# neuraloperator/graph-pde

Hardware: AMD Instinct MI355X
Metric: M-edges/s through fused NNConv fwd (width=64) (higher is better)
Workload: dtype f32 (hidden layer + aggregation: 2-term f16-split MFMA, f32 accumulate); 1 GPU; GKN Darcy-2D 241x241 radius graph r=0.1 N=58081 E=95539625; NNConv_old fwd width=64; kernel MLP 6-1024-1024-4096; aggr=mean root+bias; one sample per GPU; graph=g241

## Files before the change

### graph-pde_amd/_lib.py

```python
from __future__ import annotations

import ctypes
import os
import re
import threading

_PKG = os.path.dirname(os.path.abspath(__file__))
LIB_PATH = os.environ.get("GPDE_LIB", os.path.join(_PKG, "libgpde.so"))

GPDE_OK = 0
GPDE_VERSION, GPDE_VERSION_ABLATION, GPDE_VERSION_INSTRUMENTED = 101, 0x10000, 0x20000
GPDE_ACC_EDGE_WEIGHTS, GPDE_ACC_ROOT, GPDE_ACC_BIAS = 1, 2, 4
GPDE_AGGR_ADD, GPDE_AGGR_MEAN, GPDE_AGGR_MAX = 0, 1, 2
GPDE_WECONV_MAX_GROUP = 16
GPDE_WECONV_ANY_MAX_WIDTH = 256
GPDE_REASSOC_ANY_MAX_HIDDEN = 4096
GPDE_RADIUS_BATCHED_REC_BYTES = 96
GPDE_FWD_DEFAULT, GPDE_FWD_F16SPLIT = 0, 1
GPDE_FWD_F16SPLIT_8WAVE, GPDE_FWD_STATIC_RANGES, GPDE_FWD_AGG_F16, GPDE_FWD_AGG_F32, GPDE_FWD_NO_EDGE_PATH = 2, 4, 16, 32, 64
GPDE_WIDTH = 64
GPDE_BWD_ACCUMULATE_GRAD_HIDDEN = 1

class GpdeWeConvDesc(ctypes.Structure):
    _fields_ = [("x", ctypes.c_void_p), ("edge_weights", ctypes.c_void_p), ("rowptr", ctypes.c_void_p),
                ("src", ctypes.c_void_p), ("root", ctypes.c_void_p), ("bias", ctypes.c_void_p),
                ("residual", ctypes.c_void_p), ("out", ctypes.c_void_p), ("n_nodes", ctypes.c_int32),
                ("aggr", ctypes.c_int32), ("relu", ctypes.c_int32), ("reserved", ctypes.c_int32)]


class GpdeNodeAttr(ctypes.Structure):
    _fields_ = [("table", ctypes.c_void_p), ("stride", ctypes.c_int32), ("n_slots", ctypes.c_int32), ("sel", ctypes.c_int32 * 8)]


HEADER_PATH = os.environ.get("GPDE_HEADER", os.path.join(os.path.dirname(_PKG), "include", "gpde.h"))
_SCALARS = {"int": ctypes.c_int, "int32_t": ctypes.c_int32, "int64_t": ctypes.c_int64, "uint32_t": ctypes.c_uint32,
            "size_t": ctypes.c_size_t, "double": ctypes.c_double}


def header_prototypes(path: str = None) -> dict:
    src = open(path or HEADER_PATH).read()
    src = re.sub(r"/\*.*?\*/", "", src, flags=re.S)
    out = {}
    for m in re.finditer(r"GPDE_API\s+([\w \*]+?)\s*\b(gpde_[a-z0-9_]+)\s*\(([^;]*?)\)\s*;", src, flags=re.S):
        ret, name, args = m.group(1).strip(), m.group(2), " ".join(m.group(3).split())
        types = []
        if args not in ("", "void"):
            for a in args.split(","):
                a = a.strip()
                t = re.sub(r"\b\w+$", "", a).strip() if not a.endswith("*") else a
                types.append(t.replace(" *", "*"))
        out[name] = (ret.replace(" *", "*"), types)
    return out


def _ctype(t: str, is_return: bool = False):
    if t.endswith("*"):
        return ctypes.c_char_p if is_return and t == "const char*" else ctypes.c_void_p
    base = t.replace("const ", "").strip()
    if base not in _SCALARS:
        raise GpdeError(f"{HEADER_PATH}: C type {t!r} has no binding rule (graph-pde_amd/_lib.py:_ctype)")
    return _SCALARS[base]


def _signatures_from_header() -> dict:
    if not os.path.exists(HEADER_PATH):
        raise GpdeError(f"{HEADER_PATH} not found: the binding is generated from the header (GPDE_HEADER overrides the path)")
    return {name: (_ctype(ret, True), [_ctype(a) for a in args]) for name, (ret, args) in header_prototypes().items()}


PROF_KINDS = ("fused", "gemm3", "epilogue", "prep", "other")


def profile_begin():
    lib().gpde_profile_begin()


def profile_end():
    ms = (ctypes.c_double * len(PROF_KINDS))()
    n = (ctypes.c_int32 * len(PROF_KINDS))()
    check(lib().gpde_profile_end_kinds(ms, n), "gpde_profile_end_kinds")
    return {k: (float(ms[i]), int(n[i])) for i, k in enumerate(PROF_KINDS)}


BWD_TRACE_FIELDS = ("phase", "na", "nb", "e0", "rows", "edge_kernel", "z", "hlast", "h1", "call_amax", "du1", "dw2", "dw1",
                    "du_pre", "ordered", "grad_attr", "from_h")
BWD_TRACE_CODES = {
    "phase": ("full", "conv", "mlp", "light", "deferred"),
    "z": ("none", "kept", "zagg32", "zagg16"),
    "hlast": ("none", "given", "store", "layers"),
    "h1": ("none", "gemm", "first_layer", "on_the_fly"),
    "du1": ("none", "f16s", "f32"),
    "dw2": ("none", "tn_split", "tn_acc"),
    "dw1": ("none", "epilogue", "dw_first", "tn_acc"),
}
BWD_TRACE_CAPACITY = 4096


def bwd_trace_begin():
    check(lib().gpde_bwd_trace_begin(), "gpde_bwd_trace_begin")


def bwd_trace_end() -> list:
    nf = len(BWD_TRACE_FIELDS)
    buf = (ctypes.c_int32 * (nf * BWD_TRACE_CAPACITY))()
    n = ctypes.c_int32()
    check(lib().gpde_bwd_trace_end(buf, BWD_TRACE_CAPACITY, ctypes.byref(n)), "gpde_bwd_trace_end")
    if n.value > BWD_TRACE_CAPACITY:
        raise GpdeError(f"gpde_bwd_trace_end: {n.value} records, more than the {BWD_TRACE_CAPACITY} this binding reads")
    out = []
    for r in range(n.value):
        rec = dict(zip(BWD_TRACE_FIELDS, buf[r * nf:(r + 1) * nf]))
        for k, names in BWD_TRACE_CODES.items():
            rec[k] = names[rec[k]]
        out.append(rec)
    return out

_lib = None
_lock = threading.Lock()
n_native_calls = 0


class GpdeError(RuntimeError):
    pass


SIGNATURES = _signatures_from_header()


def lib() -> ctypes.CDLL:
    global _lib
    if _lib is None:
        with _lock:
            if _lib is None:
                if not os.path.exists(LIB_PATH):
                    raise GpdeError(
                        f"{LIB_PATH} not found - build it with `python graph-pde_amd/build.py` "
                        "(or __graft_entry__.build()); the NNConv hot path has no non-HIP fallback")
                l = ctypes.CDLL(LIB_PATH)
                for name, (res, args) in SIGNATURES.items():
                    fn = getattr(l, name)
                    fn.restype, fn.argtypes = res, args
                ver = int(l.gpde_version())
                m = re.search(r"#define\s+GPDE_VERSION\s+(\d+)", open(HEADER_PATH).read())
                if m is None or int(m.group(1)) != (ver & 0xffff):
                    raise GpdeError(f"{LIB_PATH} reports ABI version {ver & 0xffff}, {HEADER_PATH} declares "
                                    f"{m.group(1) if m else '?'}: header and library do not belong together (GPDE_LIB / GPDE_HEADER)")
                if ver & GPDE_VERSION_ABLATION and os.environ.get("GPDE_ALLOW_ABLATION") != "1":
                    raise GpdeError(
                        f"{LIB_PATH} is an ABLATION build (gpde_version() = {ver:#x}: arithmetic compiled out, results are "
                        "wrong; timing experiments only) - refused.  GPDE_ALLOW_ABLATION=1 loads it for such an experiment")
                _lib = l
    return _lib


def reload_switches() -> None:
    if _lib is not None:
        _lib.gpde_reload_switches()


def check(rc: int, what: str) -> None:
    if rc != GPDE_OK:
        msg = lib().gpde_last_error().decode("utf-8", "replace")
        if rc == -2:
            raise NotImplementedError(f"{what}: {msg}")
        raise GpdeError(f"{what} failed (code {rc}): {msg}")


def dims_array(dims):
    return (ctypes.c_int32 * len(dims))(*[int(d) for d in dims])
```

### graph-pde_amd/csrc/gpde_api.hip

```cpp
#include "gpde_common.h"
#include <stdarg.h>
#include <stdio.h>
#include <stdlib.h>
#include <vector>

static thread_local char g_err[512] = "";

void gpde_set_error(const char* fmt, ...) {
    va_list ap;
    va_start(ap, fmt);
    vsnprintf(g_err, sizeof(g_err), fmt, ap);
    va_end(ap);
}

namespace {
__global__ void k_zero_words(unsigned* __restrict__ p, size_t n) {
    const size_t stride = (size_t)gridDim.x * blockDim.x;
    for (size_t i = (size_t)blockIdx.x * blockDim.x + threadIdx.x; i < n; i += stride) p[i] = 0u;
}
__global__ void k_zero_vec4(uint4* __restrict__ p, size_t n) {
    const size_t stride = (size_t)gridDim.x * blockDim.x;
    for (size_t i = (size_t)blockIdx.x * blockDim.x + threadIdx.x; i < n; i += stride) p[i] = uint4{0u, 0u, 0u, 0u};
}
__global__ void k_zero2d_words(unsigned* __restrict__ p, size_t pitch_words, size_t width_words, size_t rows) {
    const size_t n = width_words * rows, stride = (size_t)gridDim.x * blockDim.x;
    for (size_t i = (size_t)blockIdx.x * blockDim.x + threadIdx.x; i < n; i += stride) p[(i / width_words) * pitch_words + i % width_words] = 0u;
}
__global__ void k_copy_words(unsigned* __restrict__ d, const unsigned* __restrict__ s_, size_t n) {
    const size_t stride = (size_t)gridDim.x * blockDim.x;
    for (size_t i = (size_t)blockIdx.x * blockDim.x + threadIdx.x; i < n; i += stride) d[i] = s_[i];
}
unsigned fill_blocks(size_t items) {
    size_t b = (items + 255) / 256;
    return (unsigned)(b < 1 ? 1 : (b > 8192 ? 8192 : b));
}
}

hipError_t gpde_zero_async(void* p, size_t bytes, hipStream_t st) {
    if (bytes == 0) return hipSuccess;
    if (bytes % 4 != 0 || ((uintptr_t)p & 3)) return hipErrorInvalidValue;
    if (bytes % 16 == 0 && ((uintptr_t)p & 15) == 0) hipLaunchKernelGGL(k_zero_vec4, dim3(fill_blocks(bytes / 16)), dim3(256), 0, st, (uint4*)p, bytes / 16);
    else hipLaunchKernelGGL(k_zero_words, dim3(fill_blocks(bytes / 4)), dim3(256), 0, st, (unsigned*)p, bytes / 4);
    return hipGetLastError();
}
hipError_t gpde_zero2d_async(void* p, size_t pitch_bytes, size_t width_bytes, size_t rows, hipStream_t st) {
    if (width_bytes == 0 || rows == 0) return hipSuccess;
    if (pitch_bytes % 4 != 0 || width_bytes % 4 != 0 || ((uintptr_t)p & 3)) return hipErrorInvalidValue;
    hipLaunchKernelGGL(k_zero2d_words, dim3(fill_blocks(width_bytes / 4 * rows)), dim3(256), 0, st, (unsigned*)p, pitch_bytes / 4, width_bytes / 4, rows);
    return hipGetLastError();
}
hipError_t gpde_copy_async(void* dst, const void* src, size_t bytes, hipStream_t st) {
    if (bytes == 0) return hipSuccess;
    if (bytes % 4 != 0 || ((uintptr_t)dst & 3) || ((uintptr_t)src & 3)) return hipErrorInvalidValue;
    hipLaunchKernelGGL(k_copy_words, dim3(fill_blocks(bytes / 4)), dim3(256), 0, st, (unsigned*)dst, (const unsigned*)src, bytes / 4);
    return hipGetLastError();
}

namespace {
GpdeSwitches load_switches() {
    auto on = [](const char* n) { return getenv(n) != nullptr; };
    auto num = [](const char* n) { const char* e = getenv(n); return e ? atoi(e) : 0; };
    GpdeSwitches s{};
    s.bwd_gemm_f32 = on("GPDE_BWD_GEMM_F32");
    s.bwd_dw2_f32 = on("GPDE_BWD_DW2_F32");
    s.bwd_h1_materialize = on("GPDE_BWD_H1_MATERIALIZE");
    s.nt_no_prefetch = on("GPDE_NT_NO_PREFETCH");
    s.tn_no_ks_xcd = on("GPDE_TN_NO_KS_XCD");
    s.edge_bwd = num("GPDE_EDGE_BWD");
    const int v = num("GPDE_DEBUG_SKEW_US");
    s.debug_skew_us = v > 0 ? (v < 100000 ? v : 100000) : 0;
    return s;
}
GpdeSwitches& switches_storage() {
    static GpdeSwitches s = load_switches();
    return s;
}
}

const GpdeSwitches& gpde_switches() { return switches_storage(); }

extern "C" int gpde_reload_switches(void) {
    switches_storage() = load_switches();
    return GPDE_OK;
}

#if defined(GPDE_ABL_2MFMA) || defined(GPDE_ABL_NOSTAGE) || defined(GPDE_ABL_NOBARRIER) || defined(GPDE_ABL_NOGEMM2) || defined(GPDE_ABL_NOWAIT) || defined(GPDE_BWABL)
#define GPDE_BUILD_FLAGS_ GPDE_VERSION_ABLATION
#elif defined(GPDE_V6_TIMING) || defined(GPDE_NT_TIMING) || defined(GPDE_EB2_TIMING) || defined(GPDE_V3_TIMING)
#define GPDE_BUILD_FLAGS_ GPDE_VERSION_INSTRUMENTED
#else
#define GPDE_BUILD_FLAGS_ 0
#endif
extern "C" int gpde_version(void) { return GPDE_VERSION | GPDE_BUILD_FLAGS_; }
extern "C" const char* gpde_last_error(void) { return g_err; }

namespace {

struct EvPair { hipEvent_t a, b; int kind; };
thread_local bool g_prof_on = false;
thread_local std::vector<EvPair> g_prof;

struct ProfScope {
    bool on; EvPair p; hipStream_t s;
    ProfScope(int kind, hipStream_t stream) : on(g_prof_on), s(stream) {
        if (!on) return;
        p.kind = kind;
        if (hipEventCreate(&p.a) != hipSuccess || hipEventCreate(&p.b) != hipSuccess) { on = false; return; }
        (void)hipEventRecord(p.a, s);
    }
    ~ProfScope() {
        if (!on) return;
        (void)hipEventRecord(p.b, s);
        g_prof.push_back(p);
    }
};

constexpr size_t kAlign = 256;
size_t align_up(size_t v) { return (v + kAlign - 1) / kAlign * kAlign; }

int num_cus_impl() {
    static std::atomic<int> cus[32];
    int dev = 0;
    if (hipGetDevice(&dev) != hipSuccess || dev < 0 || dev > 31) dev = 0;
    int v = cus[dev].load(std::memory_order_relaxed);
    if (v == 0) {
        if (hipDeviceGetAttribute(&v, hipDeviceAttributeMultiprocessorCount, dev) != hipSuccess || v <= 0) v = 256;
        cus[dev].store(v, std::memory_order_relaxed);
    }
    return v;
}

struct Plan {
    GpdePackLayout L;
    int64_t nodes_per_chunk;
    int n_chunks;
    int n_groups;
    size_t off_part, off_z, off_ha, off_hb, off_xs, off_scal, off_blk;
    int nblk_max;
    size_t h_floats;
};

int pick_splits(int64_t nn) {
    const int64_t tiles = (nn + 63) / 64;
    int s = 1;
    while (s < 64 && tiles * s < 1024) s *= 2;
    return s;
}

int make_plan(int64_t N, int64_t E, int n_layers, const int32_t* dims, size_t ws_bytes, bool sizing,
              Plan* P, size_t* needed, bool hidden_given = false) {
    int rc = gpde_pack_layout(n_layers, dims, &P->L);
    if (rc != GPDE_OK) return rc;
    const GpdePackLayout& L = P->L;
    const size_t zrow = (size_t)GP_W * L.K2P * sizeof(float);
    const size_t prow = (size_t)64 * GP_W * sizeof(float);
    size_t fixed = 0;
    P->h_floats = 0;
    const size_t xs_bytes = (L.mode == 1 || hidden_given || sizing) ? align_up((size_t)(N > 0 ? N : 1) * GP_W * 4) + kAlign : 0;
    if (L.mode == 2 && !hidden_given) {
        int kmax = 0;
        for (int l = 1; l <= n_layers - 1; ++l) kmax = kmax > L.frontKP[l] ? kmax : L.frontKP[l];
        P->h_floats = (size_t)(E > 0 ? E : 1) * kmax;
        fixed = 2 * align_up(P->h_floats * sizeof(float));
    }
    fixed += xs_bytes;
    P->nblk_max = (L.mode == 1 && E < ((int64_t)1 << 31) - GP_QBLOCK) ? (int)(E / GP_QBLOCK + E / 8 / (GP_QBLOCK / 8)) + 10 : 0;
    const size_t blk_bytes = P->nblk_max ? align_up(((size_t)P->nblk_max + 2 + 64) * 4) : 0;
    fixed += blk_bytes;
    int64_t npc;
    if (sizing) {
        int64_t cap = (int64_t)(((size_t)4 << 30) / zrow);
        if (cap < 64) cap = 64;
        npc = N < cap ? N : cap;
        if (npc < 1) npc = 1;
    } else {
        if (ws_bytes < fixed + 2 * kAlign) {
            gpde_set_error("gpde_nnconv_fwd: workspace %zu bytes cannot hold the %zu-byte hidden "
                           "activation buffers", ws_bytes, fixed);
            return GPDE_EWORKSPACE;
        }
        npc = (int64_t)((ws_bytes - fixed - 2 * kAlign) / (zrow + prow));
        if (N > 0 && align_up((size_t)N * prow) + align_up((size_t)N * zrow) + fixed <= ws_bytes) npc = N;
        if (npc > N) npc = N;
        const int64_t min_nodes = N < 64 ? N : 64;
        if (npc < min_nodes || (N > 0 && npc < 1)) {
            gpde_set_error("gpde_nnconv_fwd: workspace %zu bytes holds %lld destination nodes, need >= %lld "
                           "(%zu bytes per node)", ws_bytes, (long long)npc, (long long)min_nodes, zrow + prow);
            return GPDE_EWORKSPACE;
        }
        if (npc < N && npc > 64) npc = npc / 64 * 64;
    }
    if (npc < 1) npc = 1;
    P->nodes_per_chunk = npc;
    P->n_chunks = (int)((N + npc - 1) / npc);
    if (P->n_chunks < 1) P->n_chunks = 1;
    size_t off = 0;
    P->off_part = off; off += align_up((size_t)npc * prow);
    P->off_z = off;    off += align_up((size_t)npc * zrow);
    P->off_ha = off;   off += (L.mode == 2 && !hidden_given) ? align_up(P->h_floats * sizeof(float)) : 0;
    P->off_hb = off;   off += (L.mode == 2 && !hidden_given) ? align_up(P->h_floats * sizeof(float)) : 0;
    P->off_xs = off;   off += xs_bytes ? xs_bytes - kAlign : 0;
    P->off_scal = off; off += xs_bytes ? kAlign : 0;
    P->off_blk = off;  off += blk_bytes;
    if (needed) *needed = off;
    const int ns = L.K2P / GP_TN;
    int groups = num_cus_impl() / ns;
    if (groups < 1) groups = 1;
    const int64_t tiles_chunk = ((E + GP_TE - 1) / GP_TE + P->n_chunks - 1) / P->n_chunks;
    int64_t gcap = (tiles_chunk + GP_WAVES - 1) / GP_WAVES;
    const int64_t gcap_nodes = (npc + GP_WAVES - 1) / GP_WAVES;
    if (gcap < gcap_nodes) gcap = gcap_nodes;
    if (groups > gcap) groups = (int)(gcap < 1 ? 1 : gcap);
    P->n_groups = groups;
    return GPDE_OK;
}

enum FusedKind { FK_GENERIC = 0, FK_V3 = 1, FK_V6 = 2 };
struct FusedChoice { FusedKind kind; bool g2f16; };
FusedChoice choose_fused(const GpdePackLayout& L, int mode, uint32_t flags, int64_t n_edges, int kt) {
    FusedChoice c{FK_GENERIC, false};
    if (mode != 1 || !(flags & GPDE_FWD_F16SPLIT)) return c;
    GpdeFusedArgs probe = gpde_fused_probe(L);
    probe.kt = kt;
    if (!gpde_fused_f16v3_supported(probe)) return c;
    c.kind = FK_V3;
    c.g2f16 = !(flags & GPDE_FWD_AGG_F32) && n_edges > 0 && ((flags & GPDE_FWD_AGG_F16) || n_edges >= 32768);
    probe.xs = c.g2f16 ? (const unsigned*)(uintptr_t)8 : nullptr;
    if (c.g2f16 && !(flags & GPDE_FWD_F16SPLIT_8WAVE) && gpde_fused_f16v6_supported(probe)) c.kind = FK_V6;
    return c;
}

bool takes_edge_path(const Plan& P, uint32_t flags, int64_t n_nodes, int64_t n_edges, bool hidden, bool hidden_absmax,
                     bool mixed, int kt) {
    const GpdePackLayout& L = P.L;
    bool store_ok = false;
    if (L.mode == 1 && L.k0 + 1 <= 8) store_ok = gpde_fused_store_supported(gpde_fused_probe(L));
    return ((flags & GPDE_FWD_F16SPLIT) || (hidden && hidden_absmax)) && !mixed && !kt && L.has_w3s && P.n_chunks == 1 &&
           n_edges >= 4096 && n_edges <= 4 * n_nodes && n_edges < ((int64_t)1 << 24) &&
           !(flags & GPDE_FWD_NO_EDGE_PATH) &&
           (hidden || (L.mode == 1 && store_ok)) &&
           (size_t)(n_edges) * L.K2P + gpde_edge_messages_ws_floats(n_edges, GP_W * GP_W) <=
               (size_t)n_nodes * GP_W * L.K2P;
}

}

int gpde_num_cus() { return num_cus_impl(); }

extern "C" const char* gpde_nnconv_fwd_kernel(int64_t n_edges, int n_layers, const int32_t* dims, uint32_t flags) {
    GpdePackLayout L;
    if (!dims || gpde_pack_layout(n_layers, dims, &L) != GPDE_OK) return "";
    switch (choose_fused(L, L.mode, flags, n_edges, 0).kind) {
        case FK_V6: return "gpde_fused_f16v6_kernel";
        case FK_V3: return "gpde_fused_f16v3_kernel";
        default: return "gpde_fused_kernel";
    }
}

extern "C" int gpde_nnconv_fwd_edge_path(int64_t n_nodes, int64_t n_edges, int n_layers, const int32_t* dims, uint32_t flags,
                                         size_t ws_bytes) {
    Plan P;
    if (!dims || n_nodes < 0 || n_edges < 0) { gpde_set_error("gpde_nnconv_fwd_edge_path: null/negative argument"); return GPDE_EINVAL; }
    int rc = make_plan(n_nodes, n_edges, n_layers, dims, ws_bytes, false, &P, nullptr);
    if (rc != GPDE_OK) return rc;
    return takes_edge_path(P, flags, n_nodes, n_edges, false, false, false, 0) ? 1 : 0;
}

extern "C" size_t gpde_nnconv_fwd_workspace_bytes(int64_t n_nodes, int64_t n_edges, int n_layers,
                                                  const int32_t* dims) {
    Plan P;
    size_t need = 0;
    if (!dims || n_nodes < 0 || n_edges < 0) return 0;
    if (make_plan(n_nodes, n_edges, n_layers, dims, 0, true, &P, &need) != GPDE_OK) return 0;
    return need + 2 * kAlign;
}

extern "C" int gpde_nnconv_fwd_plan(int64_t n_nodes, int64_t n_edges, int n_layers,
                                    const int32_t* dims, size_t ws_bytes, int32_t* n_chunks,
                                    int64_t* nodes_per_chunk, int32_t* fused_workgroups,
                                    int32_t* mode) {
    Plan P;
    if (!dims) { gpde_set_error("gpde_nnconv_fwd_plan: dims is null"); return GPDE_EINVAL; }
    int rc = make_plan(n_nodes, n_edges, n_layers, dims, ws_bytes, false, &P, nullptr);
    if (rc != GPDE_OK) return rc;
    if (n_chunks) *n_chunks = P.n_chunks;
    if (nodes_per_chunk) *nodes_per_chunk = P.nodes_per_chunk;
    if (fused_workgroups) *fused_workgroups = P.n_groups * (P.L.K2P / GP_TN);
    if (mode) *mode = P.L.mode;
    return GPDE_OK;
}

namespace {

struct FwdArgs {
    const float* x = nullptr;
    int64_t n_nodes = 0, n_edges = 0;
    const int32_t *rowptr = nullptr, *src = nullptr, *dst = nullptr;
    int n_layers = 0;
    const int32_t* dims = nullptr;
    const void* packed = nullptr;
    const float *root = nullptr, *bias = nullptr;
    int aggr = 0;
    float* out = nullptr;
    void* ws = nullptr;
    size_t ws_bytes = 0;
    hipStream_t stream = nullptr;
    const float* edge_attr = nullptr;
    const int32_t* perm = nullptr;
    uint32_t flags = 0;
    const float *hidden = nullptr, *hidden_absmax = nullptr;
    int64_t hidden_nodes = -1;
    int kt = 0;
    const int* sel = nullptr;
    const float* residual = nullptr;
    int relu_out = 0;
    float* z_keep = nullptr;
};

FwdArgs fwd_common(const float* x, int64_t n_nodes, int64_t n_edges, const int32_t* rowptr, const int32_t* src, const int32_t* dst,
                   int n_layers, const int32_t* dims, const void* packed, const float* root, const float* bias, int aggr,
                   float* out, void* ws, size_t ws_bytes, void* stream) {
    FwdArgs a;
    a.x = x; a.n_nodes = n_nodes; a.n_edges = n_edges; a.rowptr = rowptr; a.src = src; a.dst = dst;
    a.n_layers = n_layers; a.dims = dims; a.packed = packed; a.root = root; a.bias = bias; a.aggr = aggr;
    a.out = out; a.ws = ws; a.ws_bytes = ws_bytes; a.stream = (hipStream_t)stream;
    return a;
}

int fwd_impl(const FwdArgs& a) {
    const bool mixed = a.hidden && a.hidden_nodes >= 0 && a.hidden_nodes < a.n_nodes;
    if (a.aggr != GPDE_AGGR_ADD && a.aggr != GPDE_AGGR_MEAN) {
        gpde_set_error("gpde_nnconv_fwd: aggr %d not implemented (add=0, mean=1)", a.aggr);
        return GPDE_EUNSUPPORTED;
    }
    if (a.n_nodes == 0) return GPDE_OK;
    if (!a.ws) { gpde_set_error("gpde_nnconv_fwd: workspace is null"); return GPDE_EWORKSPACE; }
    Plan P;
    int rc = make_plan(a.n_nodes, a.n_edges, a.n_layers, a.dims, a.ws_bytes, false, &P, nullptr, a.hidden != nullptr && !mixed);
    if (rc != GPDE_OK) return rc;
    const GpdePackLayout& L = P.L;
    const int mode = (a.hidden && !mixed) ? 2 : L.mode;
    if (mixed && L.mode != 1) { gpde_set_error("gpde_nnconv_fwd_mixed_keepz: built for 3-Linear kernel MLPs"); return GPDE_EUNSUPPORTED; }
    const float* pk = (const float*)a.packed;
    char* w = (char*)a.ws;
    w = (char*)(((uintptr_t)w + kAlign - 1) / kAlign * kAlign);
    float* part = (float*)(w + P.off_part);
    float* zbuf = (float*)(w + P.off_z);
    float* ha = (float*)(w + P.off_ha);
    float* hb = (float*)(w + P.off_hb);

    const float* hfinal = a.hidden;
    if (!a.hidden && L.mode == 2 && a.n_edges > 0) {
        const float* in = a.edge_attr;
        int ldx = L.k0, kin = L.k0;
        const int32_t* gather = a.perm;
        float* bufs[2] = {ha, hb};
        for (int l = 0; l < a.n_layers - 1; ++l) {
            GpdeDenseArgs d;
            d.X = in; d.ldx = ldx; d.kin = kin; d.gather = gather; d.row0 = 0;
            d.W = pk + L.off_front_w[l]; d.ldw = L.frontKP[l];
            d.b = pk + L.off_front_b[l];
            d.Y = bufs[l & 1]; d.KoutP = L.frontKP[l + 1];
            d.rows = (int)a.n_edges; d.relu = 1;
            rc = gpde_launch_dense(d, a.stream);
            if (rc != GPDE_OK) return rc;
            in = d.Y; ldx = kin = d.KoutP; gather = nullptr;
        }
        hfinal = in;
    }

    const bool edge_path = !a.z_keep && takes_edge_path(P, a.flags, a.n_nodes, a.n_edges, a.hidden != nullptr,
                                                        a.hidden_absmax != nullptr, mixed, a.kt);
    if (edge_path) {
        float* Hbuf = zbuf;
        float* ews = zbuf + (a.hidden ? 0 : (size_t)a.n_edges * L.K2P);
        const float* Hrows = a.hidden;
        if (!a.hidden) {
            ProfScope ps(GPDE_PROF_FUSED, a.stream);
            GpdeFusedArgs f{};
            f.attr = a.edge_attr; f.rowptr = a.rowptr; f.perm = a.perm;
            gpde_fused_set_pack(f, pk, L);
            f.hout = Hbuf; f.hmax_out = nullptr;
            f.nc0 = 0; f.nc1 = (int)a.n_nodes; f.e_chunk0 = 0;
            f.n_groups = gpde_fused_groups(L.K2P, gpde_group_cap_fwd(a.n_edges));
            if ((rc = gpde_launch_fused_store(f, a.stream)) != GPDE_OK) return rc;
            Hrows = Hbuf;
        }
        {
            ProfScope ps(GPDE_PROF_GEMM3, a.stream);
            rc = gpde_launch_edge_messages(Hrows, L.K2P, a.n_edges, pk + L.off_w3s, pk + L.off_ucol3, a.x, a.src, a.rowptr, a.n_nodes,
                                           ews, part, a.stream);
            if (rc != GPDE_OK) return rc;
        }
        GpdeEpilogueArgs e;
        e.part = part; e.x = a.x; e.rowptr = a.rowptr; e.src = a.src;
        e.b3 = pk + L.off_b3; e.root = a.root; e.bias = a.bias; e.out = a.out;
        e.nc0 = 0; e.nn = (int)a.n_nodes; e.splits = 1; e.aggr = a.aggr;
        e.residual = a.residual; e.relu_out = a.relu_out;
        ProfScope ps2(GPDE_PROF_EPILOGUE, a.stream);
        return gpde_launch_epilogue(e, a.stream);
    }

    const unsigned* xs = nullptr;
    const unsigned* scal = nullptr;
    const FusedChoice fc = choose_fused(L, mode, a.flags, a.n_edges, a.kt);
    if (a.kt && fc.kind == FK_GENERIC) {
        gpde_set_error("gpde_nnconv_fwd_mixed_keepz (node_attr): built for 3-Linear kernel MLPs on the f16-split kernel only");
        return GPDE_EUNSUPPORTED;
    }
    if ((!a.hidden || mixed) && fc.g2f16) {
        ProfScope psp(GPDE_PROF_PREP, a.stream);
        rc = gpde_launch_g2_prep(a.x, a.n_nodes, a.edge_attr, a.n_edges, L.k0, pk + L.off_w1 + (size_t)L.K1P * 8,
                                 (unsigned*)(w + P.off_scal), (unsigned*)(w + P.off_xs), a.stream, a.kt, a.sel, a.src, a.dst);
        if (rc != GPDE_OK) return rc;
        xs = (const unsigned*)(w + P.off_xs);
        scal = (const unsigned*)(w + P.off_scal);
    }

    if (a.hidden && !mixed && a.hidden_absmax && a.n_edges >= 32768 && !(a.flags & GPDE_FWD_AGG_F32)) {
        rc = gpde_launch_g2_prep(a.x, a.n_nodes, nullptr, 0, 0, nullptr, (unsigned*)(w + P.off_scal),
                                 (unsigned*)(w + P.off_xs), a.stream);
        if (rc != GPDE_OK) return rc;
        xs = (const unsigned*)(w + P.off_xs);
        scal = (const unsigned*)(w + P.off_scal);
    }

    const int64_t hn = mixed ? a.hidden_nodes : (a.hidden ? a.n_nodes : 0);
    for (int64_t nc0 = 0, nc1 = 0; nc0 < a.n_nodes; nc0 = nc1) {
        const int64_t lim = nc0 < hn ? hn : a.n_nodes;
        nc1 = (nc0 + P.nodes_per_chunk < lim) ? nc0 + P.nodes_per_chunk : lim;
        const bool from_h = nc0 < hn;
        const int nn = (int)(nc1 - nc0);
        const int splits = pick_splits(nn);
        if (a.n_edges > 0) {
            GpdeFusedArgs f{};
            f.x = a.x; f.attr = a.edge_attr; f.rowptr = a.rowptr; f.src = a.src; f.dst = a.dst; f.perm = a.perm;
            gpde_fused_set_pack(f, pk, L);
            float* zc = a.z_keep ? a.z_keep + (size_t)nc0 * GP_W * L.K2P : zbuf;
            f.hbuf = hfinal; f.zbuf = zc; f.xs = xs; f.scal = scal;
            f.kt = a.kt; f.hmax = (from_h && xs) ? (const unsigned*)a.hidden_absmax : nullptr;
            for (int d = 0; d < 8; ++d) f.sel[d] = (a.kt && a.sel) ? a.sel[d < L.k0 ? d : L.k0 - 1] : 0;
            f.nc0 = (int)nc0; f.nc1 = (int)nc1; f.e_chunk0 = 0; f.n_groups = P.n_groups;
            {
                ProfScope ps(GPDE_PROF_FUSED, a.stream);
                if (!from_h && fc.kind == FK_V6 && P.nblk_max && L.K2P / GP_TN <= 64 && !(a.flags & GPDE_FWD_STATIC_RANGES)) {
                    int32_t* blk = (int32_t*)(w + P.off_blk);
                    f.blk = blk; f.qn = blk + P.nblk_max + 1; f.qctr = (unsigned*)(blk + P.nblk_max + 2);
                    rc = gpde_launch_block_bounds(a.rowptr, (int)nc0, (int)nc1, P.nblk_max, blk, blk + P.nblk_max + 1,
                                                  (unsigned*)(blk + P.nblk_max + 2), L.K2P / GP_TN, a.stream);
                    if (rc != GPDE_OK) return rc;
                }
                if (from_h) rc = gpde_launch_zagg(f, a.stream);
                else if (fc.kind == FK_V6) rc = gpde_launch_fused_f16v6(f, a.stream);
                else if (fc.kind == FK_V3) rc = gpde_launch_fused_f16v3(f, a.stream);
                else rc = gpde_launch_fused(mode, (a.flags & GPDE_FWD_F16SPLIT) != 0 && mode == 1, f, a.stream);
            }
            if (rc != GPDE_OK) return rc;
            ProfScope ps1(GPDE_PROF_GEMM3, a.stream);
            GpdeGemm3Args g;
            g.zbuf = zc; g.w3q = pk + L.off_w3q; g.part = part; g.nn = nn; g.K2P = L.K2P;
            g.splits = splits; g.rowptr = a.rowptr; g.nc0 = (int)nc0;
            rc = gpde_launch_gemm3(g, a.stream);
            if (rc != GPDE_OK) return rc;
        }
        GpdeEpilogueArgs e;
        e.part = part; e.x = a.x; e.rowptr = a.rowptr; e.src = a.src;
        e.b3 = pk + L.off_b3; e.root = a.root; e.bias = a.bias; e.out = a.out;
        e.nc0 = (int)nc0; e.nn = nn; e.splits = splits; e.aggr = a.aggr;
        e.residual = a.residual; e.relu_out = a.relu_out;
        ProfScope ps2(GPDE_PROF_EPILOGUE, a.stream);
        rc = gpde_launch_epilogue(e, a.stream);
        if (rc != GPDE_OK) return rc;
    }
    return GPDE_OK;
}

}

extern "C" int gpde_nnconv_fwd(const float* x, int64_t n_nodes, const float* edge_attr,
                               int64_t n_edges, const int32_t* rowptr, const int32_t* src,
                               const int32_t* dst, const int32_t* perm, int n_layers,
                               const int32_t* dims, const void* packed, const float* root,
                               const float* bias, int aggr, uint32_t flags, float* out, void* ws,
                               size_t ws_bytes, void* stream_) {
    if (n_nodes < 0 || n_edges < 0 || !dims || !packed || !rowptr || (n_nodes > 0 && (!x || !out)) ||
        (n_edges > 0 && (!edge_attr || !src || !dst || !perm))) {
        gpde_set_error("gpde_nnconv_fwd: null/negative argument");
        return GPDE_EINVAL;
    }
    FwdArgs a = fwd_common(x, n_nodes, n_edges, rowptr, src, dst, n_layers, dims, packed, root, bias, aggr, out, ws, ws_bytes, stream_);
    a.edge_attr = edge_attr; a.perm = perm; a.flags = flags;
    return fwd_impl(a);
}

extern "C" int gpde_nnconv_fwd_mixed_keepz(const float* x, int64_t n_nodes, const float* edge_attr, const GpdeNodeAttr* node_attr,
                                           const float* hidden, const float* hidden_absmax, int64_t hidden_nodes, int64_t n_edges,
                                           const int32_t* rowptr, const int32_t* src, const int32_t* dst,
                                           const int32_t* perm, int n_layers, const int32_t* dims, const void* packed,
                                           const float* root, const float* bias, int aggr, uint32_t flags, float* z_keep,
                                           float* out, void* ws, size_t ws_bytes, void* stream_) {
    if (n_nodes < 0 || n_edges < 0 || !dims || !packed || !rowptr || (n_nodes > 0 && (!x || !out)) ||
        (n_edges > 0 && (!src || !dst || (!node_attr && (!edge_attr || !perm)))) || hidden_nodes < 0 || hidden_nodes > n_nodes ||
        (hidden_nodes > 0 && !hidden)) {
        gpde_set_error("gpde_nnconv_fwd_mixed_keepz: null/negative argument");
        return GPDE_EINVAL;
    }
    int kt = 0;
    int sel[8] = {0, 0, 0, 0, 0, 0, 0, 0};
    const float* attr = edge_attr;
    if (node_attr) {
        const GpdeNodeAttr* na = node_attr;
        if (!na->table || na->stride < 1 || na->n_slots != dims[0] || dims[0] < 1 || dims[0] > 7) {
            gpde_set_error("gpde_nnconv_fwd_mixed_keepz: GpdeNodeAttr must describe dims[0] = 1..7 slots of a node table");
            return GPDE_EINVAL;
        }
        for (int d = 0; d < 8; ++d) {
            sel[d] = na->sel[d < dims[0] ? d : dims[0] - 1];
            if ((sel[d] >> 8) < 0 || (sel[d] >> 8) > 1 || (sel[d] & 255) >= na->stride) {
                gpde_set_error("gpde_nnconv_fwd_mixed_keepz: GpdeNodeAttr.sel[%d] = 0x%x (endpoint << 8 | column, column < %d)", d, sel[d], na->stride);
                return GPDE_EINVAL;
            }
        }
        kt = na->stride;
        attr = na->table;
        perm = nullptr;
    }
    FwdArgs a = fwd_common(x, n_nodes, n_edges, rowptr, src, dst, n_layers, dims, packed, root, bias, aggr, out, ws, ws_bytes, stream_);
    a.edge_attr = attr; a.perm = perm; a.flags = flags; a.kt = kt; a.sel = kt ? sel : nullptr; a.z_keep = z_keep;
    if (hidden_nodes != 0) { a.hidden = hidden; a.hidden_absmax = hidden_absmax; a.hidden_nodes = hidden_nodes; }
    return fwd_impl(a);
}

extern "C" int gpde_nnconv_fwd_hidden(const float* x, int64_t n_nodes, const float* hidden,
                                      const float* hidden_absmax, int64_t n_edges, const int32_t* rowptr, const int32_t* src,
                                      const int32_t* dst, int n_layers, const int32_t* dims,
                                      const void* packed, const float* root, const float* bias,
                                      int aggr, float* out, void* ws, size_t ws_bytes, void* stream_) {
    if (n_nodes < 0 || n_edges < 0 || !dims || !packed || !rowptr || (n_nodes > 0 && (!x || !out)) ||
        (n_edges > 0 && (!hidden || !src || !dst))) {
        gpde_set_error("gpde_nnconv_fwd_hidden: null/negative argument");
        return GPDE_EINVAL;
    }
    FwdArgs a = fwd_common(x, n_nodes, n_edges, rowptr, src, dst, n_layers, dims, packed, root, bias, aggr, out, ws, ws_bytes, stream_);
    a.hidden = hidden; a.hidden_absmax = hidden_absmax;
    return fwd_impl(a);
}

extern "C" int gpde_nnconv_fwd_act(const float* x, int64_t n_nodes, const float* edge_attr, int64_t n_edges,
                                   const int32_t* rowptr, const int32_t* src, const int32_t* dst, const int32_t* perm,
                                   int n_layers, const int32_t* dims, const void* packed, const float* root,
                                   const float* bias, int aggr, uint32_t flags, const float* residual, int relu_out,
                                   float* out, void* ws, size_t ws_bytes, void* stream_) {
    if (n_nodes < 0 || n_edges < 0 || !dims || !packed || !rowptr || (n_nodes > 0 && (!x || !out)) ||
        (n_edges > 0 && (!edge_attr || !src || !dst || !perm)) || (residual && residual == out)) {
        gpde_set_error("gpde_nnconv_fwd_act: null/negative argument (or residual aliases out)");
        return GPDE_EINVAL;
    }
    FwdArgs a = fwd_common(x, n_nodes, n_edges, rowptr, src, dst, n_layers, dims, packed, root, bias, aggr, out, ws, ws_bytes, stream_);
    a.edge_attr = edge_attr; a.perm = perm; a.flags = flags; a.residual = residual; a.relu_out = relu_out;
    return fwd_impl(a);
}

extern "C" int gpde_nnconv_fwd_hidden_act(const float* x, int64_t n_nodes, const float* hidden, const float* hidden_absmax,
                                          int64_t n_edges, const int32_t* rowptr, const int32_t* src, const int32_t* dst,
                                          int n_layers, const int32_t* dims, const void* packed, const float* root,
                                          const float* bias, int aggr, const float* residual, int relu_out, float* out,
                                          void* ws, size_t ws_bytes, void* stream_) {
    if (n_nodes < 0 || n_edges < 0 || !dims || !packed || !rowptr || (n_nodes > 0 && (!x || !out)) ||
        (n_edges > 0 && (!hidden || !src || !dst)) || (residual && residual == out)) {
        gpde_set_error("gpde_nnconv_fwd_hidden_act: null/negative argument (or residual aliases out)");
        return GPDE_EINVAL;
    }
    FwdArgs a = fwd_common(x, n_nodes, n_edges, rowptr, src, dst, n_layers, dims, packed, root, bias, aggr, out, ws, ws_bytes, stream_);
    a.hidden = hidden; a.hidden_absmax = hidden_absmax; a.residual = residual; a.relu_out = relu_out;
    return fwd_impl(a);
}

extern "C" int gpde_nnconv_fwd_keepz(const float* x, int64_t n_nodes, const float* edge_attr, const float* hidden,
                                     const float* hidden_absmax, int64_t n_edges, const int32_t* rowptr, const int32_t* src,
                                     const int32_t* dst, const int32_t* perm, int n_layers, const int32_t* dims,
                                     const void* packed, const float* root, const float* bias, int aggr, uint32_t flags,
                                     float* z_keep, float* out, void* ws, size_t ws_bytes, void* stream_) {
    if (n_nodes < 0 || n_edges < 0 || !dims || !packed || !rowptr || (n_nodes > 0 && (!x || !out || !z_keep)) ||
        (n_edges > 0 && (!src || !dst || (!hidden && (!edge_attr || !perm))))) {
        gpde_set_error("gpde_nnconv_fwd_keepz: null/negative argument");
        return GPDE_EINVAL;
    }
    FwdArgs a = fwd_common(x, n_nodes, n_edges, rowptr, src, dst, n_layers, dims, packed, root, bias, aggr, out, ws, ws_bytes, stream_);
    a.z_keep = z_keep;
    if (hidden) { a.hidden = hidden; a.hidden_absmax = hidden_absmax; }
    else { a.edge_attr = edge_attr; a.perm = perm; a.flags = flags; }
    return fwd_impl(a);
}

extern "C" int gpde_profile_begin(void) {
// ... 27 lines not shown
```

### graph-pde_amd/csrc/gpde_common.h

```cpp
#pragma once
#include <hip/hip_runtime.h>
#include <stdint.h>
#include <stddef.h>
#include "gpde.h"
#include <atomic>

typedef float f32x4 __attribute__((ext_vector_type(4)));
typedef float f32x16 __attribute__((ext_vector_type(16)));

constexpr int GP_W = GPDE_WIDTH;
constexpr int GP_TE = 32;
constexpr int GP_TN = 128;
constexpr int GP_BK = 32;
constexpr int GP_WAVES = 4;
constexpr int GP_BS_STRIDE = 36;

static inline int gp_round_up(int v, int m) { return (v + m - 1) / m * m; }

static inline bool gp_overlap(const void* a, size_t na, const void* b, size_t nb) {
    if (!a || !b || !na || !nb) return false;
    const uintptr_t a0 = (uintptr_t)a, b0 = (uintptr_t)b;
    return a0 < b0 + nb && b0 < a0 + na;
}

struct GpdePackLayout {
    int mode;
    int n_layers;
    int k0;
    int k1, K1P;
    int k2, K2P;
    size_t off_w1;
    size_t off_w2t;
    size_t off_b2;
    size_t off_w2h;
    size_t off_ucol;
    size_t off_w1h;
    size_t off_fcol;
    size_t off_w3q;
    size_t off_b3;
    size_t off_front;
    int frontKP[GPDE_MAX_LAYERS + 1];
    size_t off_front_w[GPDE_MAX_LAYERS];
    size_t off_front_b[GPDE_MAX_LAYERS];
    size_t off_w3s;
    size_t off_ucol3;
    int has_w3s;
    size_t total_floats;
    int has_b3;
};

int gpde_pack_layout(int n_layers, const int32_t* dims, GpdePackLayout* L);

void gpde_set_error(const char* fmt, ...);

hipError_t gpde_zero_async(void* p, size_t bytes, hipStream_t st);
hipError_t gpde_zero2d_async(void* p, size_t pitch_bytes, size_t width_bytes, size_t rows, hipStream_t st);
hipError_t gpde_copy_async(void* dst, const void* src, size_t bytes, hipStream_t st);

struct GpdeSwitches {
    bool bwd_gemm_f32;
    bool bwd_dw2_f32;
    bool bwd_h1_materialize;
    bool nt_no_prefetch;
    bool tn_no_ks_xcd;
    int edge_bwd;
    int debug_skew_us;
};
const GpdeSwitches& gpde_switches();

#define GP_HIP_CHECK(expr)                                                              \
    do {                                                                                \
        hipError_t _e = (expr);                                                         \
        if (_e != hipSuccess) {                                                         \
            gpde_set_error("%s failed: %s (%s:%d)", #expr, hipGetErrorString(_e),       \
                           __FILE__, __LINE__);                                         \
            return GPDE_EHIP;                                                           \
        }                                                                               \
    } while (0)

#define GP_LAUNCH_CHECK(name)                                                           \
    do {                                                                                \
        hipError_t _e = hipGetLastError();                                              \
        if (_e != hipSuccess) {                                                         \
            gpde_set_error("launch of %s failed: %s", name, hipGetErrorString(_e));     \
            return GPDE_EHIP;                                                           \
        }                                                                               \
    } while (0)

struct GpdeLdsOnce {
    std::atomic<unsigned> done{0};
    template <typename... Fn>
    int ensure(Fn... fns) {
        int dev = 0;
        if (hipGetDevice(&dev) != hipSuccess || dev < 0 || dev > 31) dev = 0;
        if (done.load(std::memory_order_acquire) & (1u << dev)) return GPDE_OK;
        const void* fl[] = {(const void*)fns...};
        for (const void* f : fl) {
            hipError_t e = hipFuncSetAttribute(f, hipFuncAttributeMaxDynamicSharedMemorySize, 160 * 1024);
            if (e != hipSuccess) {
                gpde_set_error("hipFuncSetAttribute(MaxDynamicSharedMemorySize) failed: %s", hipGetErrorString(e));
                return GPDE_EHIP;
            }
        }
        done.fetch_or(1u << dev, std::memory_order_release);
        return GPDE_OK;
    }
};

struct GpdeFusedArgs {
    const float* x;
    const float* attr;
    const int32_t* rowptr;
    const int32_t* src;
    const int32_t* dst;
    const int32_t* perm;
    const float* w1;
    const float* w2t;
    const float* b2;
    const void* w2h;
    const float* ucol;
    const void* w1h;
    const float* fcol;
    const float* hbuf;
    float* zbuf;
    float* hout;
    const unsigned* xs;
    const unsigned* scal;
    const unsigned* hmax;
    unsigned* hmax_out;
    const int32_t* blk;
    const int32_t* qn;
    unsigned* qctr;
    int kt;
    int sel[8];
    int k0, K1P, K2P;
    int nc0, nc1;
    int e_chunk0;
    int n_groups;
    int kernarg_pad_;
};
int gpde_launch_fused(int mode, bool f16split, const GpdeFusedArgs& a, hipStream_t stream);
int gpde_launch_g2_prep(const float* x, int64_t n_nodes, const float* attr, int64_t n_edges, int k0,
                        const float* wmax8, unsigned* scal, unsigned* xs, hipStream_t stream,
                        int kt = 0, const int* sel = nullptr, const int32_t* src = nullptr,
                        const int32_t* dst = nullptr);
constexpr int GP_QBLOCK = 4096;
int gpde_launch_block_bounds(const int32_t* rowptr, int nc0, int nc1, int nblk_max, int32_t* blk, int32_t* qn,
                             unsigned* qctr, int n_slices, hipStream_t stream);
__host__ __device__ static inline float gpde_pow2_to_2p13(float v) {
    union { float f; unsigned u; } a; a.f = v;
    const int eb = (int)((a.u >> 23) & 0xff);
    if (eb < 20 || eb > 230) return 1.f;
    a.u = (unsigned)(267 - eb) << 23;
    return a.f;
}
int gpde_launch_zagg(const GpdeFusedArgs& a, hipStream_t stream);
bool gpde_fused_f16v3_supported(const GpdeFusedArgs& a);
int gpde_launch_fused_f16v3(const GpdeFusedArgs& a, hipStream_t stream);
bool gpde_fused_store_supported(GpdeFusedArgs probe);
int gpde_launch_fused_store(const GpdeFusedArgs& a, hipStream_t stream);
bool gpde_fused_f16v6_supported(const GpdeFusedArgs& a);
int gpde_launch_fused_f16v6(const GpdeFusedArgs& a, hipStream_t stream);
int gpde_num_cus();
static inline void gpde_fused_set_pack(GpdeFusedArgs& f, const float* pk, const GpdePackLayout& L) {
    f.w1 = pk + L.off_w1; f.w2t = pk + L.off_w2t; f.b2 = pk + L.off_b2;
    f.w2h = pk + L.off_w2h; f.ucol = pk + L.off_ucol; f.w1h = pk + L.off_w1h; f.fcol = pk + L.off_fcol;
    f.k0 = L.k0; f.K1P = L.K1P; f.K2P = L.K2P;
}
static inline GpdeFusedArgs gpde_fused_probe(const GpdePackLayout& L) {
    GpdeFusedArgs probe{};
    probe.k0 = L.k0; probe.K1P = L.K1P; probe.K2P = L.K2P;
    return probe;
}
static inline int64_t gpde_group_cap_fwd(int64_t n_edges) { return ((n_edges + GP_TE - 1) / GP_TE + GP_WAVES - 1) / GP_WAVES; }
static inline int64_t gpde_group_cap_bwd_chunk(int rows) { return (rows / GP_TE + GP_WAVES) / GP_WAVES; }
static inline int gpde_fused_groups(int K2P, int64_t cap) {
    int groups = gpde_num_cus() / (K2P / GP_TN);
    if (groups < 1) groups = 1;
    return groups > cap ? (int)cap : groups;
}

struct GpdeGemm3Args {
    const float* zbuf;
    const float* w3q;
    float* part;
    int nn, K2P, splits;
    const int32_t* rowptr;
    int nc0;
};
int gpde_launch_gemm3(const GpdeGemm3Args& a, hipStream_t stream);

struct GpdeEpilogueArgs {
    const float* part;
    const float* x;
    const int32_t* rowptr;
    const int32_t* src;
    const float* b3;
    const float* root;
    const float* bias;
    float* out;
    int nc0, nn, splits, aggr;
    const float* residual;
    int relu_out;
};
int gpde_launch_epilogue(const GpdeEpilogueArgs& a, hipStream_t stream);

struct GpdeDenseArgs {
    const float* X; int ldx; int kin;
    const int32_t* gather;
    int row0;
    const float* W; int ldw;
    const float* b;
    float* Y; int KoutP;
    int rows; int relu;
};
int gpde_launch_dense(const GpdeDenseArgs& a, hipStream_t stream);

struct GpdeGemmArgs {
    const float* A; const float* B; float* C;
    int M, N, K;
    int lda, ldb, ldc;
    int a_kcontig, b_kcontig;
    const float* bias;
    int relu;
    const float* mask; int ldmask;
    int accumulate;
    int batches; size_t strideA, strideB, strideC;
    int splits; size_t strideSplit;
    int skew_us;
};
int gpde_debug_skew_us();
__device__ __forceinline__ void gp_debug_skew(int us) {
    if (us > 0) {
        const unsigned long long t0 = wall_clock64();
        while (wall_clock64() - t0 < (unsigned long long)us * 100ull) __builtin_amdgcn_s_sleep(64);
    }
}
int gpde_launch_gemm(const GpdeGemmArgs& g, hipStream_t stream);
int gpde_launch_reduce_splits(const float* P, size_t n, int splits, size_t stride, float* C,
                              int accumulate, hipStream_t stream);
struct GpdeGemmF16sArgs {
    const float* A; int lda; int M;
    const void* bsplit; const float* ucol;
    const float* mask; int ldmask;
    const uint32_t* maskbits; int ldmb;
    float* C; int ldc;
    int K, N;
    const float* sc; const float* isc;
    int n_groups;
    int ksplits; size_t cstride;
    const float* xc_x; const int32_t* xc_src;
    int skew_us;
    int no_tile_prefetch;
    int no_ks_xcd;
    const int32_t* g_src;
    const int32_t* g_tile;
    int g_ntiles;
    size_t g_layer_stride;
    size_t g_bnode_bytes;
    const float* g_unscale;
    int fl_mode;
    const float* fl_attr; int fl_ld0;
    int fl_rows;
    const void* fl_wimg;
    const float* fl_alpha;
    float* fl_dw_part; float* fl_dw_out; int fl_dw_ld; float* fl_db_out; int fl_skip_store;
};
size_t gpde_gemm_f16s_dw_part_floats(int M, int N);
bool gpde_gemm_f16s_supported(int M, int N, int K, int lda);

struct GpdeEdgeBwd3Args {
    const float* x; const int32_t* src; const int32_t* dst;
    const float* dZ;
    const float* dz_unscale;
    const float* dS;
    const float* H;
    float* dU;
    float* dx;
    float* dxe;
    int e0, e1, n0, K2P;
    float* dUt; int ldt;
    float* row_sc; float* row_isc;
    float* csum_part; unsigned* cmax_part;
    int du_accumulate;
};
int gpde_launch_dz_split(float* dZ, int nn, int K2P, float* unscale, hipStream_t stream);
int gpde_launch_edge_bwd3(const GpdeEdgeBwd3Args& a, hipStream_t stream);
int gpde_launch_gemm_f16s_nt(const GpdeGemmF16sArgs& a, float* row_scale_ws , hipStream_t stream);
size_t gpde_edge_messages_ws_floats(int64_t n_edges, int n_out);
int gpde_launch_edge_messages(const float* H, int K2P, int64_t n_edges, const void* w3s, const float* ucol3,
                              const float* x, const int32_t* src, const int32_t* rowptr, int64_t n_nodes, float* ws,
                              float* part, hipStream_t stream);
size_t gpde_gemm_f16s_tn_ws_floats(int rows_max, int n_out, int n_in, int ksplits);
struct GpdeFirstLayerSpec {
    const float* H0; int ld0;
    const float* Wp; int ldw;
    const float* bp;
    uint32_t* maskbits;
    int k0;
    const unsigned* amax_bits;
};
bool gpde_first_layer_in_kernel(const GpdeFirstLayerSpec& f, int rows, int ksplits);
struct GpdeDuStats {
    float* db_accumulate;
    float* row_sc; float* row_isc;
    const float* tile_csum; const unsigned* tile_cmax;
};
float* gpde_gemm_f16s_tn_at(float* ws, int rows, int ksplits, int* ld);
int gpde_launch_gemm_f16s_tn(const float* dU, int ldu, int n_out, const float* H, int ldh, int n_in, int rows,
                             int ksplits, float* ws, float* part, hipStream_t stream,
                             const unsigned* du_absmax_bits = nullptr ,
                             const GpdeFirstLayerSpec* first_layer = nullptr ,
                             const GpdeDuStats* du_stats = nullptr);
int gpde_launch_gemm_f16s_gather(const float* xstack, size_t layer_stride, int Lp, const float* sc_src, const float* isc_src,
                                 const int32_t* src_rows, int rows, const int32_t* tiles, int ntiles, const void* bimg,
// ... 16 lines not shown
```

### graph-pde_amd/csrc/gpde_fused_f16v6.hip

```cpp
#include "gpde_common.h"
#include <cstdlib>
#include <type_traits>

namespace {

typedef _Float16 h8 __attribute__((ext_vector_type(8)));
typedef unsigned u4 __attribute__((ext_vector_type(4)));

__device__ __forceinline__ f32x4 mfma32k(h8 a, h8 b, f32x4 c) {
    return __builtin_amdgcn_mfma_f32_16x16x32_f16(a, b, c, 0, 0, 0);
}
#define GPDE_GLDS(g, l, off)                                                                       \
    __builtin_amdgcn_global_load_lds((const __attribute__((address_space(1))) void*)(g),         \
                                     (__attribute__((address_space(3))) void*)(l), 16, off, 0)

__device__ __forceinline__ int lower_bound_node(const int32_t* __restrict__ rowptr, int lo, int hi, long target) {
    while (lo < hi) {
        int mid = (lo + hi) >> 1;
        if ((long)rowptr[mid] < target) lo = mid + 1; else hi = mid;
    }
    return lo;
}

#ifdef GPDE_V6_TIMING
__device__ unsigned long long gpde_v6_tm[8];
#define TM_MARK(acc) do { const long long tm1_ = clock64(); acc += tm1_ - tm0_; tm0_ = tm1_; } while (0)
#else
#define TM_MARK(acc) do { } while (0)
#endif

constexpr int NS = 3;
constexpr int TILE_B = GP_TN * 128;
constexpr int TE = 64;
constexpr int NW = 4;

template <int MODE, bool NODEATTR = false>
__global__ __launch_bounds__(256) __attribute__((amdgpu_waves_per_eu(1, 1)))
void gpde_fused_f16v6_kernel(GpdeFusedArgs a) {
    constexpr bool WRITE_H = MODE == 1;
    extern __shared__ __attribute__((aligned(16))) char smem[];
    char* ring = smem;
    char* w1s = smem + NS * TILE_B;
    unsigned* Xs_all = (unsigned*)(w1s + (size_t)a.K1P * 32);
    float* Es_all = (float*)(Xs_all + NW * TE * GP_W);
    int* red = (int*)(Es_all + NW * TE);
    float* colc = (float*)(red + 16);

    const int tid = threadIdx.x;
    const int lane = tid & 63;
    const int wave = __builtin_amdgcn_readfirstlane(tid >> 6);
    const int l15 = lane & 15;
    const int g = lane >> 4;
    float* Es = Es_all + wave * TE;
    unsigned* Xs = Xs_all + wave * TE * GP_W;

    const int ns = a.K2P / GP_TN;
    const int slice = blockIdx.x % ns;
    const int group = blockIdx.x / ns;
    const int NKC = a.K1P / GP_BK;

    for (int i = tid; i < a.K1P * 2; i += 256) ((f32x4*)w1s)[i] = ((const f32x4*)a.w1h)[i];

    const int e_lo = a.rowptr[a.nc0], e_hi = a.rowptr[a.nc1];
    const bool queue = a.blk != nullptr;
    int blk_a = 0, blk_b = 0;
    const int nblk = queue ? *a.qn : 0;
    bool have;
    auto draw_block = [&](int& ba, int& bb) {
        for (;;) {
            int b = 0;
            if (lane == 0) b = (int)atomicAdd(a.qctr + slice, 1u);
            b = __builtin_amdgcn_readfirstlane(b);
            if (b >= nblk) return false;
            ba = a.blk[b];
            bb = a.blk[b + 1];
            if (bb > ba) return true;
        }
    };
    if (queue) {
        have = draw_block(blk_a, blk_b);
    } else {
        const long tot = (long)e_hi - e_lo;
        const int nranges = a.n_groups * NW;
        const int wg = group * NW + wave;
        const int na = lower_bound_node(a.rowptr, a.nc0, a.nc1, e_lo + tot * wg / nranges);
        const int nb_ = (wg == nranges - 1) ? a.nc1
                                            : lower_bound_node(a.rowptr, a.nc0, a.nc1, e_lo + tot * (wg + 1) / nranges);
        blk_a = a.rowptr[na];
        blk_b = a.rowptr[nb_];
        have = blk_b > blk_a;
    }
    if (lane == 0) { red[wave] = have ? 0 : 1; red[4 + wave] = 0; }
    __syncthreads();
    if (red[0] + red[1] + red[2] + red[3] == 4) return;

    const unsigned long long w2base = (unsigned long long)a.w2h + (size_t)slice * NKC * TILE_B + wave * 4096;
    const unsigned lane16 = lane * 16;
    auto w2_src = [&](int chunk) {
        unsigned long long gb = w2base + (size_t)chunk * TILE_B;
        asm volatile("" : "+s"(gb));
        return (const char*)(gb + lane16);
    };

    float z_unscale = 1.f;
    if constexpr (WRITE_H) {
        if (tid < GP_TN) {
            colc[tid] = a.b2[slice * GP_TN + tid];
            colc[GP_TN + tid] = a.ucol[slice * GP_TN + tid];
        }
    } else {
        const float sx = gpde_pow2_to_2p13(__uint_as_float(a.scal[0]));
        const float hb = a.fcol[8] + a.fcol[9] * __uint_as_float(a.scal[1]);
        const float sh = gpde_pow2_to_2p13(hb);
        if (tid < GP_TN) {
            colc[tid] = a.b2[slice * GP_TN + tid] * sh;
            colc[GP_TN + tid] = a.ucol[slice * GP_TN + tid] * sh;
        }
        z_unscale = (1.f / sx) * (1.f / sh);
    }
    float wmx8[8], fcol8[8];
#pragma unroll
    for (int d = 0; d < 8; ++d) {
        wmx8[d] = a.w1[(size_t)a.K1P * 8 + (d & 1) * 4 + (d >> 1)];
        fcol8[d] = a.fcol[d];
    }
    const int bo = l15 * 128 + ((g ^ ((l15 >> 1) & 7)) << 4);
    const int w1o = (16 * (l15 >> 3) + 4 * ((l15 >> 2) & 1) + (l15 & 3)) * 32 + (g == 2 ? 16 : 0);

    const int e_clamp = max(e_hi - 1, 0);
    int perm_n = 0;
    [[maybe_unused]] int dst_n = 0;
    int src_l = 0;
    float attr_n[8];
    auto load_perm = [&](int e0n) {
        if constexpr (NODEATTR) {
            perm_n = a.src[min(e0n + lane, e_clamp)];
            dst_n = a.dst[min(e0n + lane, e_clamp)];
        } else perm_n = a.perm[min(e0n + lane, e_clamp)];
    };
    auto load_attr_d = [&](int d) {
        if constexpr (NODEATTR) {
            const int sd = a.sel[d];
            attr_n[d] = a.attr[(size_t)((sd >> 8) ? dst_n : perm_n) * a.kt + (sd & 255)];
        } else {
            attr_n[d] = a.attr[(size_t)perm_n * a.k0 + min(d, a.k0 - 1)];
        }
    };
    auto load_attr = [&]() {
#pragma unroll
        for (int d = 0; d < 8; ++d) load_attr_d(d);
    };
    int xsidx[4];
    auto x_addr1 = [&](int i0, int i) { xsidx[i] = __builtin_amdgcn_ds_bpermute((4 * (i0 + i) + (lane >> 4)) * 4, src_l); };
    auto x_issue1 = [&](int i0, int i) {
        int unit = lane & 15;
        GPDE_GLDS(a.xs + (size_t)xsidx[i] * GP_W + unit * 4, Xs + (i0 + i) * 4 * GP_W, 0);
    };

    auto conv_a = [&](float v0, float v1, unsigned& ph, unsigned& t0_, unsigned& t1_) {
        asm("v_max_i32 %1, 0, %3\n\t"
            "v_max_i32 %2, 0, %4\n\t"
            "v_cvt_pkrtz_f16_f32 %0, %1, %2"
            : "=&v"(ph), "=&v"(t0_), "=&v"(t1_) : "v"(v0), "v"(v1));
    };
    auto conv_b = [&](unsigned ph, unsigned t0_, unsigned t1_, unsigned& pl) {
        asm("v_fma_mixlo_f16 %0, %1, 1.0, -%3 op_sel:[0,0,0] op_sel_hi:[0,0,1]\n\t"
            "v_fma_mixhi_f16 %0, %2, 1.0, -%3 op_sel:[0,0,1] op_sel_hi:[0,0,1]"
            : "=&v"(pl) : "v"(t0_), "v"(t1_), "v"(ph));
    };
    auto conv_pair = [&](float v0, float v1, unsigned& ph, unsigned& pl) {
        unsigned t0_, t1_;
        conv_a(v0, v1, ph, t0_, t1_);
        conv_b(ph, t0_, t1_, pl);
    };
    auto conv_step = [&](int step, float v0, float v1, unsigned& ph, unsigned& t0_, unsigned& t1_, unsigned& pl) {
        if (step == 0) asm("v_max_i32 %0, 0, %1" : "=v"(t0_) : "v"(v0));
        if (step == 1) asm("v_max_i32 %0, 0, %1" : "=v"(t1_) : "v"(v1));
        if (step == 2) asm("v_cvt_pkrtz_f16_f32 %0, %1, %2" : "=v"(ph) : "v"(t0_), "v"(t1_));
        if (step == 3) asm("v_fma_mixlo_f16 %0, %1, 1.0, -%2 op_sel:[0,0,0] op_sel_hi:[0,0,1]" : "=v"(pl) : "v"(t0_), "v"(ph));
        if (step == 4) asm("v_fma_mixhi_f16 %0, %1, 1.0, -%2 op_sel:[0,0,1] op_sel_hi:[0,0,1]" : "+v"(pl) : "v"(t1_), "v"(ph));
    };
    auto h1gen_half = [&](f32x4 (&dd)[4][2], int e0, h8 w1r0, h8 w1r1, const h8 (&at)[4]) {
        asm volatile("s_nop 4");
#pragma unroll
        for (int e = e0; e < e0 + 2; ++e) {
            asm volatile("v_mfma_f32_16x16x32_f16 %0, %1, %2, 0" : "=&v"(dd[e][0]) : "v"(w1r0), "v"(at[e]));
            asm volatile("v_mfma_f32_16x16x32_f16 %0, %1, %2, 0" : "=&v"(dd[e][1]) : "v"(w1r1), "v"(at[e]));
        }
    };
    auto h1gen = [&](f32x4 (&dd)[4][2], h8 w1r0, h8 w1r1, const h8 (&at)[4]) {
        h1gen_half(dd, 0, w1r0, w1r1, at);
        h1gen_half(dd, 2, w1r0, w1r1, at);
    };

    {
        const char* g0 = w2_src(0);
        char* l0 = ring + wave * 4096;
        GPDE_GLDS(g0, l0, 0); GPDE_GLDS(g0, l0, 1024); GPDE_GLDS(g0, l0, 2048); GPDE_GLDS(g0, l0, 3072);
        const char* g1 = w2_src(1);
        char* l1 = ring + TILE_B + wave * 4096;
        GPDE_GLDS(g1, l1, 0); GPDE_GLDS(g1, l1, 1024); GPDE_GLDS(g1, l1, 2048); GPDE_GLDS(g1, l1, 3072);
    }
    load_perm(have ? blk_a : e_hi);
    load_attr();
    asm volatile("s_waitcnt vmcnt(0)" ::: "memory");
    __syncthreads();

    f32x4 acc[4][8], Z[4][8];
#pragma unroll
    for (int e = 0; e < 4; ++e)
#pragma unroll
        for (int nb = 0; nb < 8; ++nb)
#pragma unroll
            for (int r = 0; r < 4; ++r) { acc[e][nb][r] = 0.f; Z[e][nb][r] = 0.f; }
    int cur = -1;
    [[maybe_unused]] float hmax_run = 0.f;

    auto flush = [&](int node) {
        float* zb = a.zbuf + ((size_t)(node - a.nc0) * GP_W) * a.K2P + slice * GP_TN;
        int zl = lane;
        asm volatile("" : "+v"(zl));
        const int z_loff = 4 * (zl >> 4) * a.K2P + (zl & 15);
#pragma unroll
        for (int cb = 0; cb < 4; ++cb)
#pragma unroll
            for (int nb = 0; nb < 8; ++nb) asm volatile("" : "+a"(Z[cb][nb]));
#pragma unroll
        for (int cb = 0; cb < 4; ++cb) {
#pragma unroll
            for (int r = 0; r < 4; ++r) {
                float* rp = zb + (size_t)(cb * 16 + r) * a.K2P;
#pragma unroll
                for (int nb = 0; nb < 8; ++nb) {
                    rp[z_loff + nb * 16] = Z[cb][nb][r] * z_unscale;
                    Z[cb][nb][r] = 0.f;
                }
                if ((r & 1) == 1) __builtin_amdgcn_sched_barrier(0);
            }
        }
#pragma unroll
        for (int cb = 0; cb < 4; ++cb)
#pragma unroll
            for (int nb = 0; nb < 8; ++nb) asm volatile("" : "+a"(Z[cb][nb]));
    };

    int slot = 0;

#ifdef GPDE_V6_TIMING
    long long tm_pro = 0, tm_loop = 0, tm_post = 0, tm_peel = 0, tm0_ = clock64();
#endif
    int e0 = have ? blk_a : e_hi;
    int n_rounds = 0;
    for (int t = 0;; ++t) {
        const int eb = have ? blk_b : e0;
        const int e_end = min(e0 + TE, eb);
        const bool last_in_blk = have && (e0 + TE >= blk_b);
        int na_ = 0, nb_ = 0;
        bool have_n = have && !last_in_blk;
        if (last_in_blk && queue) have_n = draw_block(na_, nb_);
        const int e0n = !have ? e_hi : (last_in_blk ? (have_n ? na_ : e_hi) : e0 + TE);
        if (t > 0) {
            if (lane == 0) red[(t & 1) * 4 + wave] = have ? 0 : 1;
            __syncthreads();
            const int* rf = red + (t & 1) * 4;
            if (rf[0] + rf[1] + rf[2] + rf[3] == 4) break;
        }
        ++n_rounds;

        h8 B1[4];
        {
#pragma unroll
            for (int b = 0; b < 4; ++b) {
                float av[8];
#pragma unroll
                for (int d = 0; d < 8; ++d)
                    av[d] = __int_as_float(__builtin_amdgcn_ds_bpermute((16 * b + l15) * 4, __float_as_int(attr_n[d])));
                const bool valid = (e0 + 16 * b + l15) < eb;
                float v[8];
                float bnd = 0.f;
#pragma unroll
                for (int d = 0; d < 8; ++d) {
                    float q = (valid && d < a.k0) ? av[d] : 0.f;
                    if (valid && d == a.k0) q = 1.f;
                    v[d] = q;
                    bnd = fmaf(wmx8[d], fabsf(q), bnd);
                }
                const int ebits = (__float_as_int(bnd) >> 23) & 0xff;
                const bool okb = (ebits >= 20) && (ebits <= 230);
                const float sc = okb ? __int_as_float((267 - ebits) << 23) : 1.f;
                const float isc = okb ? __int_as_float((ebits - 13) << 23) : 1.f;
                if (g == 0) Es[16 * b + l15] = isc;
#pragma unroll
                for (int d = 0; d < 8; ++d) {
                    const float s_ = v[d] * fcol8[d] * sc;
                    const _Float16 hi = (_Float16)s_;
                    const _Float16 lo = (_Float16)(s_ - (float)hi);
                    B1[b][d] = g == 1 ? lo : (g == 3 ? (_Float16)0.f : hi);
                }
            }
        }
        h8 bhi[2][2], blo[2][2];
#pragma unroll
        for (int nb = 0; nb < 2; ++nb) {
            bhi[0][nb] = *(const h8*)(ring + slot * TILE_B + nb * 2048 + bo);
            blo[0][nb] = *(const h8*)(ring + slot * TILE_B + nb * 2048 + (bo ^ 64));
        }
        f32x4 d[4][2];
        u4 ahi[4], alo[4];
        {
            const char* wp = w1s + w1o;
            const h8 A1 = *(const h8*)wp, A2 = *(const h8*)(wp + 256);
            h1gen(d, A1, A2, B1);
            asm volatile("s_nop 15\n\ts_nop 15" ::: "memory");
#pragma unroll
            for (int e = 0; e < 4; ++e)
#pragma unroll
                for (int jp = 0; jp < 4; ++jp) {
                    unsigned ph, pl;
                    conv_pair(d[e][jp >> 1][2 * (jp & 1)], d[e][jp >> 1][2 * (jp & 1) + 1], ph, pl);
                    ahi[e][jp] = ph;
                    alo[e][jp] = pl;
                }
        }
        int nf_v[2] = {0, 0}, nl_v[2] = {0, 0};
        unsigned cph = 0, ct0 = 0, ct1 = 0, cpl = 0;
        h8 A1, A2;

        TM_MARK(tm_pro);
        auto chunk = [&](auto ph_tag, int c) {
            constexpr int PH = decltype(ph_tag)::value;
            asm volatile("" : "+s"(c));
            const int slot1 = slot + 1 == NS ? 0 : slot + 1;
            const int slot2 = slot1 + 1 == NS ? 0 : slot1 + 1;
            int c2 = c + 2;
            if (c2 >= NKC) c2 -= NKC;
            const char* gsrc = w2_src(c2);
            char* ldst = ring + slot2 * TILE_B + wave * 4096;
            const char* rb0 = ring + slot * TILE_B;
            const char* rb1 = ring + slot1 * TILE_B;
            int c1 = c + 1;
            if (c1 >= NKC) c1 -= NKC;
            const char* w1n = w1s + (size_t)c1 * GP_BK * 32 + w1o;
#pragma unroll
            for (int g8 = 0; g8 < 8; ++g8) {
                const int hf = g8 >> 2, bt = g8 & 3, fs = g8 & 1;
                const char* rn = (g8 < 7) ? rb0 + (2 * ((bt + 1) & 3)) * 2048 : rb1;
#pragma unroll
                for (int q = 0; q < 12; ++q) {
                    const int e = 2 * hf + q / 6, j = q % 6;
                    const int tt = j >> 1, nb = j & 1;
                    const int cb = 2 * bt + nb;
                    const int n = g8 * 12 + q;
#ifdef GPDE_ABL_2MFMA
                    if (tt != 2)
#endif
                    acc[e][cb] = mfma32k(__builtin_bit_cast(h8, tt == 2 ? alo[e] : ahi[e]),
                                         tt == 0 ? blo[fs][nb] : bhi[fs][nb], acc[e][cb]);
                    asm volatile("" : "+a"(acc[e][cb]));
                    if (q != 5 && q != 11) {
                        const int v = q < 5 ? q : q - 1, pr = 2 * bt + v / 5, step = v % 5;
                        const int ce = 2 * (1 - hf) + (pr >> 2), jp = pr & 3;
                        conv_step(step, d[ce][jp >> 1][2 * (jp & 1)], d[ce][jp >> 1][2 * (jp & 1) + 1], cph, ct0, ct1, cpl);
                        if (step == 4) {
                            ahi[ce][jp] = cph;
                            alo[ce][jp] = cpl;
                        }
                    } else {
                        const int ce = 2 * (1 - hf) + (bt >> 1);
                        asm volatile("" ::"v"(ahi[ce]), "v"(alo[ce]));
                    }
                    if (q == 0) blo[fs ^ 1][0] = *(const h8*)(rn + (bo ^ 64));
                    if (q == 3) blo[fs ^ 1][1] = *(const h8*)(rn + 2048 + (bo ^ 64));
                    if (q == 6) bhi[fs ^ 1][0] = *(const h8*)(rn + bo);
                    if (q == 9) bhi[fs ^ 1][1] = *(const h8*)(rn + 2048 + bo);
                    if (n == 5) GPDE_GLDS(gsrc, ldst, 0);
                    if (n == 11) GPDE_GLDS(gsrc, ldst, 1024);
                    if (n == 17) GPDE_GLDS(gsrc, ldst, 2048);
                    if (n == 23) GPDE_GLDS(gsrc, ldst, 3072);
                    if (n == 25) A1 = *(const h8*)w1n;
                    if (n == 31) A2 = *(const h8*)(w1n + 256);
                    if constexpr (MODE == 0 && PH == 0) {
                        if (n == 53) load_perm(e0n);
                        if (n == 59) src_l = a.src[min(e0 + lane, e_clamp)];
                        if (n == 65) nf_v[0] = a.dst[min(e0, e_clamp)];
                        if (n == 71) nl_v[0] = a.dst[min(max(min(e0 + 32, eb) - 1, e0), e_clamp)];
                        if (n == 77) nf_v[1] = a.dst[min(e0 + 32, e_clamp)];
                        if (n == 83) nl_v[1] = a.dst[min(max(min(e0 + 64, eb) - 1, e0 + 32), e_clamp)];
                    } else if constexpr (WRITE_H && PH == 0) {
                        if (n == 53) load_perm(e0n);
                    }
                    if constexpr (PH == 2) {
                        if (n >= 29 && n < 77 && (n - 29) % 6 == 0) load_attr_d((n - 29) / 6);
                    }
                    if constexpr (!WRITE_H && PH >= 2 && PH <= 5) {
                        if (n == 1 || n == 7 || n == 13 || n == 19) x_addr1(4 * (PH - 2), (n - 1) / 6);
                        if constexpr (PH == 2) {
                            if (n == 77 || n == 83 || n == 89 || n == 95) x_issue1(0, (n - 77) / 6);
                        } else {
                            if (n == 53 || n == 65 || n == 77 || n == 89) x_issue1(4 * (PH - 2), (n - 53) / 12);
                        }
                    }
                    __builtin_amdgcn_sched_barrier(0);
                    if (n == 45 || n == 93) {
                        h1gen_half(d, n == 45 ? 0 : 2, A1, A2, B1);
                        __builtin_amdgcn_sched_barrier(0);
                    }
                }
            }
            if constexpr (WRITE_H && PH == 0 && NODEATTR) asm volatile("s_waitcnt vmcnt(2)" ::: "memory");
            else if constexpr (WRITE_H && PH == 0) asm volatile("s_waitcnt vmcnt(1)" ::: "memory");
            else if constexpr (WRITE_H && PH == 2) asm volatile("s_waitcnt vmcnt(8)" ::: "memory");
            else if constexpr (WRITE_H) asm volatile("s_waitcnt vmcnt(0)" ::: "memory");
            else if constexpr (PH == 0 && NODEATTR) asm volatile("s_waitcnt vmcnt(7)" ::: "memory");
            else if constexpr (PH == 0) asm volatile("s_waitcnt vmcnt(6)" ::: "memory");
            else if constexpr (PH == 2) asm volatile("s_waitcnt vmcnt(12)" ::: "memory");
            else if constexpr (PH >= 3 && PH <= 5) asm volatile("s_waitcnt vmcnt(4)" ::: "memory");
            else asm volatile("s_waitcnt vmcnt(0)" ::: "memory");
            __builtin_amdgcn_s_barrier();
            __builtin_amdgcn_sched_barrier(0);
            slot = slot1;
        };
        chunk(std::integral_constant<int, 0>{}, 0);
        chunk(std::integral_constant<int, 1>{}, 1);
        chunk(std::integral_constant<int, 2>{}, 2);
        chunk(std::integral_constant<int, 3>{}, 3);
        chunk(std::integral_constant<int, 4>{}, 4);
        chunk(std::integral_constant<int, 5>{}, 5);
#ifdef GPDE_V6_TIMING
        tm_peel += clock64() - tm0_;
#endif
        for (int c = 6; c < NKC; ++c) chunk(std::integral_constant<int, 6>{}, c);


        TM_MARK(tm_loop);
        if constexpr (WRITE_H) {
#pragma unroll
            for (int b = 0; b < 4; ++b) {
                const f32x4 ie = *(const f32x4*)&Es[16 * b + 4 * g];
                auto store_rows = [&](auto full_tag) {
                    constexpr bool FULL = decltype(full_tag)::value;
#pragma unroll
                    for (int r = 0; r < 4; ++r) {
                        const int e = e0 + 16 * b + 4 * g + r;
                        float* hp = a.hout + (size_t)(e - a.e_chunk0) * a.K2P + slice * GP_TN + l15;
#pragma unroll
                        for (int nb = 0; nb < 8; ++nb) {
                            const float y = fmaxf(fmaf(acc[b][nb][r], ie[r] * colc[GP_TN + nb * 16 + l15], colc[nb * 16 + l15]), 0.f);
                            acc[b][nb][r] = 0.f;
                            if (FULL || e < eb) { hp[nb * 16] = y; hmax_run = fmaxf(hmax_run, y); }
                        }
                    }
                };
                if (e0 + TE <= eb) store_rows(std::true_type{});
                else store_rows(std::false_type{});
            }
        } else
#pragma unroll
        for (int b = 0; b < 2; ++b) {
            u4 g2hi[8], g2lo[8];
            float ie[8];
#pragma unroll
            for (int q4 = 0; q4 < 2; ++q4) {
                const f32x4 t4 = *(const f32x4*)&Es[32 * b + 16 * q4 + 4 * g];
#pragma unroll
                for (int j = 0; j < 4; ++j) ie[4 * q4 + j] = t4[j];
            }
#pragma unroll
            for (int nb = 0; nb < 8; ++nb) {
                float y[8];
                const float b2v = colc[nb * 16 + l15], ucv = colc[GP_TN + nb * 16 + l15];
#pragma unroll
                for (int r = 0; r < 8; ++r) {
                    y[r] = fmaf(acc[2 * b + (r >> 2)][nb][r & 3], ie[r] * ucv, b2v);
                    acc[2 * b + (r >> 2)][nb][r & 3] = 0.f;
                }
#pragma unroll
                for (int p_ = 0; p_ < 4; ++p_) {
                    unsigned ph, pl;
                    conv_pair(y[2 * p_], y[2 * p_ + 1], ph, pl);
                    g2hi[nb][p_] = ph;
                    g2lo[nb][p_] = pl;
                }
                if (nb & 1) __builtin_amdgcn_sched_barrier(0);
            }
            const int s0 = e0 + 32 * b;
            const int s_end = min(s0 + 32, e_end);
            int e_seg = s0;
            const int n_last_b = __builtin_amdgcn_readfirstlane(nl_v[b]);
            int node = __builtin_amdgcn_readfirstlane(nf_v[b]);
            while (e_seg < s_end) {
                const int seg_end = (node == n_last_b) ? s_end : min(a.rowptr[node + 1], s_end);
                if (node != cur) {
                    if (cur >= 0) flush(cur);
                    cur = node;
                }
                const int lo = e_seg - s0 - 4 * g, hi = seg_end - s0 - 4 * g;
                const bool full = (e_seg == s0) && (seg_end == s0 + 32);
                const unsigned* xu = Xs + 32 * b * GP_W;
                unsigned wq[2][8];
                auto ldx = [&](int cb, unsigned (&w)[8]) {
#pragma unroll
                    for (int tq = 0; tq < 8; ++tq) {
                        const int er = 16 * (tq >> 2) + (tq & 3);
                        w[tq] = xu[(er + 4 * g) * GP_W + cb * 16 + l15];
                    }
                };
                ldx(0, wq[0]);
#pragma unroll
                for (int cb = 0; cb < 4; ++cb) {
                    unsigned (&w)[8] = wq[cb & 1];
                    if (cb + 1 < 4) ldx(cb + 1, wq[(cb + 1) & 1]);
                    asm volatile("" : "+v"(w[0]), "+v"(w[1]), "+v"(w[2]), "+v"(w[3]), "+v"(w[4]), "+v"(w[5]), "+v"(w[6]), "+v"(w[7]));
                    if (!full) {
#pragma unroll
                        for (int tq = 0; tq < 8; ++tq) {
                            const int er = 16 * (tq >> 2) + (tq & 3);
                            const unsigned keep = (er >= lo && er < hi) ? 0xffffffffu : 0u;
                            w[tq] &= keep;
                        }
                    }
                    u4 ah, al;
#pragma unroll
                    for (int jp = 0; jp < 4; ++jp) {
                        ah[jp] = __builtin_amdgcn_perm(w[2 * jp + 1], w[2 * jp], 0x05040100u);
                        al[jp] = __builtin_amdgcn_perm(w[2 * jp + 1], w[2 * jp], 0x07060302u);
                    }
                    const h8 xhi = __builtin_bit_cast(h8, ah), xlo = __builtin_bit_cast(h8, al);
#pragma unroll
                    for (int nb = 0; nb < 8; ++nb) {
                        const h8 gh = __builtin_bit_cast(h8, g2hi[nb]), gl = __builtin_bit_cast(h8, g2lo[nb]);
                        Z[cb][nb] = mfma32k(xhi, gh, Z[cb][nb]);
                        Z[cb][nb] = mfma32k(xhi, gl, Z[cb][nb]);
                        Z[cb][nb] = mfma32k(xlo, gh, Z[cb][nb]);
                        asm volatile("" : "+a"(Z[cb][nb]));
                    }
                }
                e_seg = seg_end;
                if (e_seg < s_end) node = a.dst[e_seg];
            }
        }
        if constexpr (MODE == 0)
#pragma unroll
        for (int cb = 0; cb < 4; ++cb)
#pragma unroll
            for (int nb = 0; nb < 8; ++nb) asm volatile("" : "+a"(Z[cb][nb]));
        TM_MARK(tm_post);
        if (last_in_blk) {
            have = have_n;
            blk_a = na_;
            blk_b = nb_;
            e0 = have ? blk_a : e_hi;
        } else if (have) {
            e0 += TE;
        }
    }
    if constexpr (WRITE_H) {
        if (a.hmax_out) {
#pragma unroll
            for (int o = 32; o > 0; o >>= 1) hmax_run = fmaxf(hmax_run, __shfl_xor(hmax_run, o));
            if (lane == 0 && hmax_run > 0.f) atomicMax(a.hmax_out, __float_as_uint(hmax_run));
        }
    } else if constexpr (MODE == 0) {
        if (cur >= 0) flush(cur);
    }
    asm volatile("s_waitcnt vmcnt(0)" ::: "memory");
#ifdef GPDE_V6_TIMING
    if (lane == 0) {
        atomicAdd(&gpde_v6_tm[0], (unsigned long long)tm_pro);
        atomicAdd(&gpde_v6_tm[1], (unsigned long long)tm_loop);
        atomicAdd(&gpde_v6_tm[2], (unsigned long long)tm_post);
        atomicAdd(&gpde_v6_tm[3], (unsigned long long)n_rounds);
        atomicAdd(&gpde_v6_tm[4], (unsigned long long)tm_peel);
    }
#endif
}

size_t v6_lds_bytes(int K1P) {
    return (size_t)NS * TILE_B + (size_t)K1P * 32 + (size_t)NW * TE * GP_W * 4 + (size_t)NW * TE * 4 + 64 +
           2 * GP_TN * 4;
}

}

#ifdef GPDE_V6_TIMING
extern "C" GPDE_API int gpde_debug_v6_timing(unsigned long long* out8, int reset) {
    if (hipMemcpyFromSymbol(out8, HIP_SYMBOL(gpde_v6_tm), 64) != hipSuccess) return -1;
    if (reset) {
        unsigned long long z[8] = {0, 0, 0, 0, 0, 0, 0, 0};
        if (hipMemcpyToSymbol(HIP_SYMBOL(gpde_v6_tm), z, 64) != hipSuccess) return -1;
    }
    return 0;
}
#endif

bool gpde_fused_f16v6_supported(const GpdeFusedArgs& a) {
    return a.K1P / GP_BK >= 8 && a.k0 + 1 <= 8 && v6_lds_bytes(a.K1P) <= 160 * 1024 &&
           (a.hout != nullptr || a.xs != nullptr);
}

int gpde_launch_fused_f16v6(const GpdeFusedArgs& a, hipStream_t stream) {
    const int ns = a.K2P / GP_TN;
    const dim3 grid(a.n_groups * ns), block(256);
    const size_t lds = v6_lds_bytes(a.K1P);
    static GpdeLdsOnce once;
    if (int rc = once.ensure(gpde_fused_f16v6_kernel<0, false>, gpde_fused_f16v6_kernel<1, false>, gpde_fused_f16v6_kernel<0, true>,
                             gpde_fused_f16v6_kernel<1, true>)) return rc;
    if (a.hout) {
        GpdeFusedArgs b = a;
        b.blk = nullptr; b.qn = nullptr; b.qctr = nullptr;
        if (a.kt) hipLaunchKernelGGL((gpde_fused_f16v6_kernel<1, true>), grid, block, lds, stream, b);
        else hipLaunchKernelGGL((gpde_fused_f16v6_kernel<1, false>), grid, block, lds, stream, b);
    } else if (a.kt) hipLaunchKernelGGL((gpde_fused_f16v6_kernel<0, true>), grid, block, lds, stream, a);
    else hipLaunchKernelGGL((gpde_fused_f16v6_kernel<0, false>), grid, block, lds, stream, a);
    GP_LAUNCH_CHECK("gpde_fused_f16v6_kernel");
    return GPDE_OK;
}

bool gpde_fused_store_supported(GpdeFusedArgs probe) {
    if (!probe.hout) probe.hout = (float*)(uintptr_t)8;
    return gpde_fused_f16v6_supported(probe) || gpde_fused_f16v3_supported(probe);
}

int gpde_launch_fused_store(const GpdeFusedArgs& f, hipStream_t stream) {
    if (!f.hout) { gpde_set_error("gpde_launch_fused_store: hout is null"); return GPDE_EINVAL; }
    if (gpde_fused_f16v6_supported(f)) return gpde_launch_fused_f16v6(f, stream);
    if (gpde_fused_f16v3_supported(f)) return gpde_launch_fused_f16v3(f, stream);
    gpde_set_error("fused store kernel: unsupported kernel MLP (K1P = %d, k0 = %d)", f.K1P, f.k0);
    return GPDE_EUNSUPPORTED;
}
```

### graph-pde_amd/csrc/gpde_prep.hip

```cpp
#include "gpde_common.h"

namespace {

__global__ void k_absmax_x(const float* __restrict__ x, size_t n, unsigned* __restrict__ scal) {
    unsigned m = 0;
    for (size_t i = (size_t)blockIdx.x * blockDim.x + threadIdx.x; i < n; i += (size_t)gridDim.x * blockDim.x)
        m = max(m, __float_as_uint(x[i]) & 0x7fffffffu);
#pragma unroll
    for (int o = 32; o > 0; o >>= 1) m = max(m, (unsigned)__shfl_xor((int)m, o));
    if ((threadIdx.x & 63) == 0 && m) atomicMax(scal, m);
}

__global__ void k_attr_bound(const float* __restrict__ attr, int64_t E, int k0, const float* __restrict__ wmax8,
                             unsigned* __restrict__ scal) {
    float w[8];
#pragma unroll
    for (int d = 0; d < 8; ++d) w[d] = wmax8[(d & 1) * 4 + (d >> 1)];
    float m = 0.f;
    for (int64_t e = (int64_t)blockIdx.x * blockDim.x + threadIdx.x; e < E; e += (int64_t)gridDim.x * blockDim.x) {
        float bnd = w[k0 < 8 ? k0 : 7];
        for (int d = 0; d < k0 && d < 8; ++d) bnd = fmaf(w[d], fabsf(attr[(size_t)e * k0 + d]), bnd);
        m = fmaxf(m, bnd);
    }
#pragma unroll
    for (int o = 32; o > 0; o >>= 1) m = fmaxf(m, __shfl_xor(m, o));
    if ((threadIdx.x & 63) == 0 && m > 0.f) atomicMax(scal + 1, __float_as_uint(m));
}

struct SelArr { int v[8]; };
__global__ void k_attr_bound_nodes(const float* __restrict__ table, int kt, SelArr sel, const int32_t* __restrict__ src,
                                   const int32_t* __restrict__ dst, int64_t E, int k0,
                                   const float* __restrict__ wmax8, unsigned* __restrict__ scal) {
    float w[8];
#pragma unroll
    for (int d = 0; d < 8; ++d) w[d] = wmax8[(d & 1) * 4 + (d >> 1)];
    float m = 0.f;
    for (int64_t e = (int64_t)blockIdx.x * blockDim.x + threadIdx.x; e < E; e += (int64_t)gridDim.x * blockDim.x) {
        const int s_ = src[e], t_ = dst[e];
        float bnd = w[k0 < 8 ? k0 : 7];
        for (int d = 0; d < k0 && d < 8; ++d)
            bnd = fmaf(w[d], fabsf(table[(size_t)((sel.v[d] >> 8) ? t_ : s_) * kt + (sel.v[d] & 255)]), bnd);
        m = fmaxf(m, bnd);
    }
#pragma unroll
    for (int o = 32; o > 0; o >>= 1) m = fmaxf(m, __shfl_xor(m, o));
    if ((threadIdx.x & 63) == 0 && m > 0.f) atomicMax(scal + 1, __float_as_uint(m));
}

__global__ void k_split_x(const float* __restrict__ x, size_t n, const unsigned* __restrict__ scal,
                          unsigned* __restrict__ xs) {
    const float sc = gpde_pow2_to_2p13(__uint_as_float(scal[0]));
    for (size_t i = (size_t)blockIdx.x * blockDim.x + threadIdx.x; i < n; i += (size_t)gridDim.x * blockDim.x) {
        const float y = x[i] * sc;
        const _Float16 hi = (_Float16)__builtin_amdgcn_cvt_pkrtz(y, 0.f)[0];
        const _Float16 lo = (_Float16)(y - (float)hi);
        xs[i] = ((unsigned)__builtin_bit_cast(unsigned short, lo) << 16) | __builtin_bit_cast(unsigned short, hi);
    }
}

__global__ void k_block_bounds(const int32_t* __restrict__ rowptr, int nc0, int nc1, int nblk_max, int32_t* __restrict__ blk,
                               int32_t* __restrict__ qn, unsigned* __restrict__ qctr, int n_slices) {
    const int b = blockIdx.x * blockDim.x + threadIdx.x;
    const int e_lo = rowptr[nc0], e_hi = rowptr[nc1];
    const long tot = (long)e_hi - e_lo;
    const int nbig = (int)(tot / 8 * 7 / GP_QBLOCK);
    const long rest = tot - (long)nbig * GP_QBLOCK;
    constexpr int SMALL = GP_QBLOCK / 8;
    const int nblk = min(nbig + (int)((rest + SMALL - 1) / SMALL), nblk_max);
    if (b == 0) *qn = nblk;
    if (b < n_slices) qctr[b] = 0u;
    if (b > nblk) return;
    if (b == nblk) { blk[b] = e_hi; return; }
    const long target = (long)e_lo + (b <= nbig ? (long)b * GP_QBLOCK : (long)nbig * GP_QBLOCK + (long)(b - nbig) * SMALL);
    int lo = nc0, hi = nc1;
    while (lo < hi) {
        const int mid = (lo + hi) >> 1;
        if ((long)rowptr[mid] < target) lo = mid + 1; else hi = mid;
    }
    blk[b] = rowptr[lo];
}

}

int gpde_launch_block_bounds(const int32_t* rowptr, int nc0, int nc1, int nblk_max, int32_t* blk, int32_t* qn,
                             unsigned* qctr, int n_slices, hipStream_t stream) {
    const int threads = nblk_max + 1 > n_slices ? nblk_max + 1 : n_slices;
    hipLaunchKernelGGL(k_block_bounds, dim3((threads + 255) / 256), dim3(256), 0, stream, rowptr, nc0, nc1, nblk_max, blk, qn,
                       qctr, n_slices);
    GP_LAUNCH_CHECK("k_block_bounds");
    return GPDE_OK;
}

int gpde_launch_g2_prep(const float* x, int64_t n_nodes, const float* attr, int64_t n_edges, int k0,
                        const float* wmax8, unsigned* scal, unsigned* xs, hipStream_t stream, int kt,
                        const int* sel, const int32_t* src, const int32_t* dst) {
    GP_HIP_CHECK(gpde_zero_async(scal, 8, stream));
    const size_t n = (size_t)n_nodes * GP_W;
    const unsigned gx = (unsigned)((n + 1023) / 1024 < 1024 ? (n + 1023) / 1024 : 1024);
    const unsigned ge = (unsigned)((n_edges + 1023) / 1024 < 2048 ? (n_edges + 1023) / 1024 : 2048);
    hipLaunchKernelGGL(k_absmax_x, dim3(gx ? gx : 1), dim3(256), 0, stream, x, n, scal);
    if (n_edges == 0 || !wmax8) {
    } else if (kt) {
        SelArr sa;
        for (int d = 0; d < 8; ++d) sa.v[d] = sel[d];
        hipLaunchKernelGGL(k_attr_bound_nodes, dim3(ge ? ge : 1), dim3(256), 0, stream, attr, kt, sa, src, dst,
                           n_edges, k0, wmax8, scal);
    } else {
        hipLaunchKernelGGL(k_attr_bound, dim3(ge ? ge : 1), dim3(256), 0, stream, attr, n_edges, k0, wmax8, scal);
    }
    hipLaunchKernelGGL(k_split_x, dim3(gx ? gx : 1), dim3(256), 0, stream, x, n, scal, xs);
    GP_LAUNCH_CHECK("gpde_g2_prep kernels");
    return GPDE_OK;
}
```

### graph-pde_amd/ops.py

```python
from __future__ import annotations

import ctypes
import os
import weakref
from dataclasses import dataclass
from typing import List, Optional, Sequence, Tuple

import torch

from . import _lib

WIDTH = _lib.GPDE_WIDTH


cross_stream_hits: "dict[str, int]" = {}


def _current_stream(dev):
    return torch.cuda.current_stream(dev)


def _capturing() -> bool:
    return torch.cuda.is_current_stream_capturing()

# ... 401 lines not shown
           tuple(edge_index.shape), tuple(edge_index.stride()), _ver(edge_index), n_nodes)
    if n_src is not None or flip:
        key = key + (None if n_src is None else int(n_src), bool(flip))
    hit = _csr_cache.pop(key, None)
    if hit is not None:
        _csr_cache[key] = hit
        csr = hit[2]
        if hit[3] is not None:
            order_hit(hit[3], "csr", (csr.rowptr, csr.src, csr.dst, csr.perm))
        return csr
    csr = build_csr(edge_index, n_nodes, n_src, flip)
    _csr_cache[key] = (storage, storage.nbytes(), csr, stream_tag(edge_index.device, synced=int(edge_index.size(1)) > 0))
    while len(_csr_cache) > _CSR_CACHE_MAX_ENTRIES or \
            (len(_csr_cache) > 1 and sum(v[1] for v in _csr_cache.values()) > _CSR_CACHE_MAX_BYTES):
        _csr_cache.pop(next(iter(_csr_cache)))
    return csr


_capture_watch: "list | None" = None


def watch(*tensors):
    if _capture_watch is not None:
        for t in tensors:
            if isinstance(t, torch.Tensor) and not t.is_inference():
                _capture_watch.append((t, t._version))


def cache_snapshot() -> list:
    pins = [v for v in _csr_cache.values()] + [v[1] for v in _pack_cache.values()] + [v for v in _stage_cache.values()]
    for v in _gcn_norm_cache.values():
        pins.append((v[2].csr, v[2].coef, v[2].self_coef, v[2]._reversed))
    for v in _csr_cache.values():
        srt = v[2]._attr_sorted
        if srt:
            pins.extend(srt.values())
    return pins


def clear_param_caches():
    _pack_cache.clear()
    _pack_by_ptr.clear()


def clear_caches():
    _csr_cache.clear()
    _pack_cache.clear()
    _pack_by_ptr.clear()
    _stage_cache.clear()
    _gcn_norm_cache.clear()
    cross_stream_hits.clear()


def mlp_linears(mlp: torch.nn.Module) -> List[torch.nn.Linear]:
    if hasattr(mlp, "layers") and isinstance(mlp.layers, torch.nn.ModuleList):
        layers = list(mlp.layers)
    elif isinstance(mlp, torch.nn.Sequential):
        layers = list(mlp)
    elif isinstance(mlp, torch.nn.Linear):
        layers = [mlp]
    else:
        raise NotImplementedError(
            f"kernel network of type {type(mlp).__name__} is not a Linear/ReLU chain; the fused "
            "MI355X operator implements the DenseNet kernels used by the reference scripts")
    lin: List[torch.nn.Linear] = []
    expect_linear = True
    for l in layers:
        if isinstance(l, torch.nn.Linear):
            if not expect_linear:
                raise NotImplementedError("two Linear layers without ReLU between them")
            lin.append(l)
            expect_linear = False
        elif isinstance(l, torch.nn.ReLU):
            if expect_linear:
                raise NotImplementedError("ReLU without a preceding Linear layer")
            expect_linear = True
        else:
            raise NotImplementedError(f"kernel network layer {type(l).__name__} is not supported "
                                      "(Linear/ReLU chains only)")
    if expect_linear or len(lin) < 2:
        raise NotImplementedError("kernel network must be Linear,(ReLU,Linear)+ ending in Linear")
    return lin


@dataclass
class PackedMlp:
    dims: Tuple[int, ...]
    packed: torch.Tensor
    dims_c: object
    tag: Optional[StreamTag] = None


_pack_cache: "dict[tuple, tuple]" = {}
_pack_by_ptr: "dict[tuple, tuple]" = {}
_PACK_CACHE_MAX_BYTES = 1 << 30


def pack_mlp(weights: Sequence[torch.Tensor], biases: Sequence[Optional[torch.Tensor]]) -> PackedMlp:
    lib = _lib.lib()
    n = len(weights)
    for w in weights:
        _require_cuda(w, "kernel-network weight")
        if w.dtype != torch.float32:
            raise NotImplementedError(f"kernel-network weights must be float32, got {w.dtype}")
    dims = tuple([int(weights[0].size(1))] + [int(w.size(0)) for w in weights])
    watch(*weights, *biases)
    ptrs = tuple(w.data_ptr() for w in weights) + tuple(0 if b is None else b.data_ptr() for b in biases) + (dims,)
    key = tuple((w.data_ptr(), _ver(w)) for w in weights) + \
        tuple((0, 0) if b is None else (b.data_ptr(), _ver(b)) for b in biases) + (dims,)
    hit = _pack_cache.pop(key, None)
    if hit is not None:
        refs, pm = hit
        if all(r() is t for r, t in zip(refs, list(weights) + [b for b in biases if b is not None])):
            _pack_cache[key] = hit
            order_hit(pm.tag, "pack_mlp", (pm.packed,))
            return pm
    dims_c = _lib.dims_array(dims)
    nbytes = int(lib.gpde_mlp_pack_bytes(n, dims_c))
    if nbytes == 0:
        _lib.check(-2, "gpde_mlp_pack_bytes")
    dev = weights[0].device
    packed = torch.empty(nbytes // 4, dtype=torch.float32, device=dev)
    w_shapes, b_shapes = _mlp_shapes(dims)
    ws = _operands([w.detach() for w in weights], "kernel-network weight", w_shapes, dev)
    bs = _operands([None if b is None else b.detach() for b in biases], "kernel-network bias", b_shapes, dev)
    wp = (ctypes.c_void_p * n)(*[w.data_ptr() for w in ws])
    bp = (ctypes.c_void_p * n)(*[None if b is None else b.data_ptr() for b in bs])
    with torch.cuda.device(dev):
        rc = lib.gpde_mlp_pack(n, dims_c, wp, bp, packed.data_ptr(), nbytes, _stream_ptr(dev))
    _lib.check(rc, "gpde_mlp_pack")
    pm = PackedMlp(dims, packed, dims_c, stream_tag(dev))
    old_key = _pack_by_ptr.get(ptrs)
    if old_key is not None:
        _pack_cache.pop(old_key, None)
    refs = [weakref.ref(t) for t in list(weights) + [b for b in biases if b is not None]]
    _pack_cache[key] = (refs, pm)
    _pack_by_ptr[ptrs] = key
    while len(_pack_cache) > 1 and sum(v[1].packed.numel() * 4 for v in _pack_cache.values()) > _PACK_CACHE_MAX_BYTES:
        k0 = next(iter(_pack_cache))
        _pack_cache.pop(k0)
    if len(_pack_by_ptr) > 4096:
        live = set(_pack_cache)
        for k in [k for k, v in _pack_by_ptr.items() if v not in live]:
            _pack_by_ptr.pop(k)
    return pm


_AGGR = {"add": _lib.GPDE_AGGR_ADD, "mean": _lib.GPDE_AGGR_MEAN}
_PRECISION = {"f32": _lib.GPDE_FWD_DEFAULT, "f16split": _lib.GPDE_FWD_F16SPLIT,
              "f16split_8wave": _lib.GPDE_FWD_F16SPLIT | _lib.GPDE_FWD_F16SPLIT_8WAVE,
              "f16split_static": _lib.GPDE_FWD_F16SPLIT | _lib.GPDE_FWD_STATIC_RANGES,
              "f16split_agg16": _lib.GPDE_FWD_F16SPLIT | _lib.GPDE_FWD_AGG_F16,
              "f16split_agg32": _lib.GPDE_FWD_F16SPLIT | _lib.GPDE_FWD_AGG_F32,
              "f16split_noedge": _lib.GPDE_FWD_F16SPLIT | _lib.GPDE_FWD_NO_EDGE_PATH}
DEFAULT_PRECISION = os.environ.get("GPDE_PRECISION", "f16split")
EDGE_PATH_MAX_IN_DEGREE = 64


def _fwd_flags(csr: "Csr", precision: Optional[str]) -> int:
    name = DEFAULT_PRECISION if precision is None else precision
    if name not in _PRECISION:
        raise ValueError(f"precision must be one of {sorted(_PRECISION)}, got {name!r}")
    flags = _PRECISION[name]
    if precision is None and (flags & _lib.GPDE_FWD_F16SPLIT) and csr.n_edges > 0 and csr.max_in_degree > EDGE_PATH_MAX_IN_DEGREE:
        flags |= _lib.GPDE_FWD_NO_EDGE_PATH
    return flags


def workspace_bytes(n_nodes: int, n_edges: int, pm: PackedMlp) -> int:
    return int(_lib.lib().gpde_nnconv_fwd_workspace_bytes(n_nodes, n_edges, len(pm.dims) - 1, pm.dims_c))


SAVE_Z_BYTES = int(float(os.environ.get("GPDE_SAVE_Z_GB", "16")) * (1 << 30))
SAVE_Z_RESERVE_BYTES = int(float(os.environ.get("GPDE_SAVE_Z_RESERVE_GB", "48")) * (1 << 30))
SAVE_H_BYTES = int(float(os.environ.get("GPDE_SAVE_H_GB", "32")) * (1 << 30))
SAVE_H_MIN_EDGES = 262144


BWD_WS_FRACTION = float(os.environ.get("GPDE_BWD_WS_FRACTION", "0"))


def bwd_workspace_bytes(lib, n: int, e: int, nl: int, dims_c, dev, h_given_bytes: int = 0) -> int:
    nbytes = int(lib.gpde_nnconv_bwd_workspace_bytes(n, e, nl, dims_c))
    if nbytes == 0:
        _lib.check(-2, "gpde_nnconv_bwd_workspace_bytes")
    if BWD_WS_FRACTION > 0:
        one = int(lib.gpde_nnconv_bwd_workspace_bytes_one_chunk(n, e, nl, dims_c)) - int(h_given_bytes)
        free, _ = device_free_bytes(dev)
        if nbytes < one <= int(BWD_WS_FRACTION * free):
            nbytes = one
    return nbytes


def bwd_plan(n_nodes: int, n_edges: int, dims: Sequence[int], ws_bytes: int, n_defer: int = 0, h_given: bool = False) -> dict:
    ec, nc = ctypes.c_int64(), ctypes.c_int64()
    rc = _lib.lib().gpde_nnconv_bwd_plan(int(n_nodes), int(n_edges), len(dims) - 1, _lib.dims_array(dims), int(ws_bytes),
                                         int(n_defer), int(bool(h_given)), ctypes.byref(ec), ctypes.byref(nc))
    _lib.check(rc, "gpde_nnconv_bwd_plan")
    return {"edges_per_chunk": ec.value, "nodes_per_chunk": nc.value}


def device_free_bytes(dev):
    free, total = torch.cuda.mem_get_info(dev)
    cached = torch.cuda.memory_reserved(dev) - torch.cuda.memory_allocated(dev)
    return free + max(0, cached), total


def alloc_bwd_ws(lib, n: int, e: int, nl: int, dims_c, dev, h_given_bytes: int = 0) -> torch.Tensor:
    nbytes = bwd_workspace_bytes(lib, n, e, nl, dims_c, dev, h_given_bytes)
    default = int(lib.gpde_nnconv_bwd_workspace_bytes(n, e, nl, dims_c))
    if nbytes > default:
        try:
            return torch.empty(nbytes, dtype=torch.uint8, device=dev)
        except torch.OutOfMemoryError:
            global n_bwd_ws_fallbacks
            n_bwd_ws_fallbacks += 1
    return _alloc_ws(default, dev)


n_grad_hidden_accumulated = 0
n_kept_hidden = 0
n_bwd_ws_fallbacks = 0


def _alloc_ws(nbytes: int, dev) -> torch.Tensor:
    try:
        return torch.empty(max(int(nbytes), 1), dtype=torch.uint8, device=dev)
    except torch.OutOfMemoryError:
        from . import hidden_cache
        if not hidden_cache.release_all():
            raise
        torch.cuda.empty_cache()
        return torch.empty(max(int(nbytes), 1), dtype=torch.uint8, device=dev)


def z_buffer(csr: Csr, dims: Sequence[int], device) -> Optional[torch.Tensor]:
    nbytes = csr.n_nodes * WIDTH * hidden_width(dims) * 4
    if SAVE_Z_BYTES <= 0 or nbytes > SAVE_Z_BYTES or csr.n_edges < 32 * csr.n_nodes:
        return None
    if nbytes > (1 << 30):
        free, _ = device_free_bytes(device)
        if free - nbytes < SAVE_Z_RESERVE_BYTES:
            return None
    try:
        return torch.zeros(csr.n_nodes, WIDTH * hidden_width(dims), dtype=torch.float32, device=device)
    except torch.OutOfMemoryError:
        return None


def keep_hidden(csr: Csr, dims: Sequence[int], device) -> bool:
    nbytes = csr.n_edges * hidden_width(dims) * 4
    if SAVE_H_BYTES <= 0 or nbytes > SAVE_H_BYTES or len(dims) != 4 or csr.n_edges < SAVE_H_MIN_EDGES or \
            DEFAULT_PRECISION != "f16split" or not 1 <= dims[0] <= 8 or (int(dims[1]) + 31) // 32 < 8 or \
            csr.n_edges < 32 * csr.n_nodes:
        return False
    free, _ = device_free_bytes(device)
    return free - nbytes >= SAVE_Z_RESERVE_BYTES


def _check_residual(residual, x, n):
    if residual is None:
        return None
    _require_cuda(residual, "residual")
    if residual.dtype != torch.float32 or tuple(residual.shape) != (n, WIDTH):
        raise ValueError(f"residual must be float32 [{n},{WIDTH}], got {residual.dtype} {tuple(residual.shape)}")
    return _operand(residual, "residual", (n, WIDTH), x.device)


def _root_bias(root, bias, dev):
    return (_operand(None if root is None else root.detach(), "root", (WIDTH, WIDTH), dev),
            _operand(None if bias is None else bias.detach(), "bias", (WIDTH,), dev))


def _out_ws(out, ws, n, dev):
    return (_operand(out, "out", (n, WIDTH), dev, writable=True),
            _operand(ws, "ws", (None,), dev, writable=True, dtype=torch.uint8))


def _attr_source(csr: "Csr", edge_attr, keep_rows: bool = False):
    if edge_attr is None:
        return None, None, None, None
    if isinstance(edge_attr, NodeAttr):
        nas = edge_attr.c_struct()
        return None, ctypes.byref(nas), None, (edge_attr, nas)
    if keep_rows:
        attr, perm = _dense16(edge_attr), csr.perm
    else:
        attr, perm = attr_in_slot_order(csr, _dense16(edge_attr))
    return attr.data_ptr(), None, perm.data_ptr(), (attr, perm)


def _forward64(label: str, x: torch.Tensor, csr: Csr, pm: PackedMlp, root, bias, aggr: str, flags: int, attr=None,
               hidden: Optional[torch.Tensor] = None, hmax: Optional[torch.Tensor] = None, hidden_nodes: Optional[int] = None,
               residual: Optional[torch.Tensor] = None, relu: bool = False, z_keep: Optional[torch.Tensor] = None,
               out: Optional[torch.Tensor] = None, ws: Optional[torch.Tensor] = None) -> torch.Tensor:
    lib = _lib.lib()
    _require_cuda(x, "x")
    if aggr not in _AGGR:
        raise NotImplementedError(f"aggr={aggr!r}: 'add' and 'mean' only")
    n, e, dev, k2p = csr.n_nodes, csr.n_edges, x.device, hidden_width(pm.dims)
    x = _operand(x, "x", (n, WIDTH), dev)
    if isinstance(attr, NodeAttr):
        _require_cuda(attr.table, "node table")
        if attr.table.size(0) != n or attr.k0 != pm.dims[0]:
            raise ValueError(f"node table must have {n} rows and {pm.dims[0]} slots")
    elif attr is not None:
        _require_cuda(attr, "edge_attr")
        if attr.dim() != 2 or attr.size(0) != e or attr.size(1) != pm.dims[0]:
            raise ValueError(f"edge_attr must be [{e},{pm.dims[0]}], got {tuple(attr.shape)}")
        if attr.device != dev:
            raise ValueError(f"edge_attr is on {attr.device}, x on {dev}")
        if attr.dtype != torch.float32:
            raise NotImplementedError(f"float32 only (got x {x.dtype}, edge_attr {attr.dtype})")
    general = hidden_nodes is not None or isinstance(attr, NodeAttr)
    if hidden_nodes is not None:
# ... 12 lines not shown
        raise ValueError("z_keep cannot be combined with the fused glue")
    if general and glue:
        raise NotImplementedError("the fused glue with node-table attributes or a partial H is not built")
    if out is None:
        out = torch.empty(n, WIDTH, dtype=torch.float32, device=dev)
    if ws is None:
        ws = _alloc_ws(workspace_bytes(n, e, pm), dev)
    head = (x.data_ptr(), n)
    graph = (csr.rowptr.data_ptr(), csr.src.data_ptr(), csr.dst.data_ptr())
    mlp = (len(pm.dims) - 1, pm.dims_c, pm.packed.data_ptr(), _ptr(root_c), _ptr(bias_c), _AGGR[aggr])
    tail = (out.data_ptr(), ws.data_ptr(), ws.numel(), _stream_ptr(dev))
    act = (_ptr(residual), 1 if relu else 0)
    with torch.cuda.device(dev):
        if general:
            rc = lib.gpde_nnconv_fwd_mixed_keepz(*head, attr_p, na_ref, _ptr(hidden), _ptr(hmax), hidden_nodes or 0, e, *graph, perm_p,
                                                 *mlp, flags, _ptr(z_keep), *tail)
        elif z_keep is not None:
            rc = lib.gpde_nnconv_fwd_keepz(*head, attr_p, _ptr(hidden), _ptr(hmax), e, *graph, perm_p, *mlp, flags, z_keep.data_ptr(), *tail)
        elif hidden is not None:
            rc = lib.gpde_nnconv_fwd_hidden_act(*head, hidden.data_ptr(), _ptr(hmax), e, *graph, *mlp, *act, *tail)
        elif glue:
            rc = lib.gpde_nnconv_fwd_act(*head, attr_p, e, *graph, perm_p, *mlp, flags, *act, *tail)
        else:
            rc = lib.gpde_nnconv_fwd(*head, attr_p, e, *graph, perm_p, *mlp, flags, *tail)
    _lib.check(rc, label)
    _lib.n_native_calls += 1
    return out


def nnconv_forward_raw(x: torch.Tensor, csr: Csr, edge_attr: torch.Tensor, pm: PackedMlp,
                       root: Optional[torch.Tensor], bias: Optional[torch.Tensor], aggr: str,
                       out: Optional[torch.Tensor] = None, ws: Optional[torch.Tensor] = None,
                       precision: Optional[str] = None, residual: Optional[torch.Tensor] = None,
                       relu: bool = False, z_keep: Optional[torch.Tensor] = None) -> torch.Tensor:
    if isinstance(edge_attr, NodeAttr):
        if residual is not None or relu:
            raise NotImplementedError("the fused glue with node-table attributes is not built")
        return nnconv_forward_mixed_raw(x, csr, edge_attr, None, None, 0, pm, root, bias, aggr, precision=precision, z_keep=z_keep,
                                        out=out, ws=ws)
    if aggr not in _AGGR:
        raise NotImplementedError(
            f"aggr={aggr!r}: the fused MI355X operator implements 'add' and 'mean' (every reference "
            "script uses 'mean'); 'max' cannot use the re-associated contraction")
    flags = _fwd_flags(csr, precision)
    if x.dtype != torch.float32 or edge_attr.dtype != torch.float32:
        raise NotImplementedError(f"float32 only (got x {x.dtype}, edge_attr {edge_attr.dtype})")
    if x.dim() != 2 or x.size(1) != WIDTH:
        raise NotImplementedError(f"node features must be [N,{WIDTH}] (in_channels = out_channels = "
                                  f"{WIDTH}), got {tuple(x.shape)}")
    if x.size(0) != csr.n_nodes:
        raise ValueError(f"x has {x.size(0)} rows, CSR was built for {csr.n_nodes} nodes")
    return _forward64("gpde_nnconv_fwd", x, csr, pm, root, bias, aggr, flags, attr=edge_attr, residual=residual, relu=relu,
                      z_keep=z_keep, out=out, ws=ws)


class NodeAttr:

    def __init__(self, table: torch.Tensor, sel: Sequence[Tuple[int, int]]):
        if table.dim() != 2 or table.dtype != torch.float32:
            raise ValueError("node table must be float32 [N, columns]")
        if not 1 <= len(sel) <= 7:
            raise NotImplementedError("1..7 attribute slots")
        for ep, col in sel:
            if ep not in (0, 1) or not 0 <= col < table.size(1) or col > 255:
                raise ValueError(f"slot ({ep}, {col}): endpoint 0 = source / 1 = target, column < {table.size(1)}")
        if table.requires_grad and torch.is_grad_enabled():
            dense = table.is_contiguous() and table.data_ptr() % 16 == 0
            self.table = table if dense else table.clone(memory_format=torch.contiguous_format)
        else:
            self.table = _dense16(table)
        self.sel = [(int(ep), int(col)) for ep, col in sel]

    @staticmethod
    def darcy(pos: torch.Tensor, a: torch.Tensor) -> "NodeAttr":
        d = pos.size(1)
        table = torch.cat([pos.float(), a.float().reshape(-1, 1)], dim=1)
        sel = [(0, c) for c in range(d)] + [(1, c) for c in range(d)] + [(0, d), (1, d)]
        return NodeAttr(table, sel)

    @property
    def k0(self) -> int:
        return len(self.sel)

    dtype = torch.float32
    requires_grad = False

    def dim(self) -> int:
        return 2

    def detach(self) -> "NodeAttr":
        return self

    def contiguous(self) -> "NodeAttr":
        return self

    @property
    def is_cuda(self) -> bool:
        return self.table.is_cuda

    @property
    def device(self):
        return self.table.device

    def c_struct(self):
        na = _lib.GpdeNodeAttr()
        na.table, na.stride, na.n_slots = self.table.data_ptr(), int(self.table.size(1)), self.k0
        for d in range(8):
            ep, col = self.sel[min(d, self.k0 - 1)]
            na.sel[d] = (ep << 8) | col
        return na

    def materialize(self, edge_index: torch.Tensor) -> torch.Tensor:
        cols = [self.table[edge_index[ep].long(), col] for ep, col in self.sel]
        return torch.stack(cols, dim=1)


def nnconv_forward_nodeattr_raw(x: torch.Tensor, csr: Csr, na: NodeAttr, pm: PackedMlp,
                                root: Optional[torch.Tensor], bias: Optional[torch.Tensor], aggr: str,
                                out: Optional[torch.Tensor] = None, ws: Optional[torch.Tensor] = None,
                                precision: Optional[str] = None) -> torch.Tensor:
    if na.table.size(0) != csr.n_nodes or na.k0 != pm.dims[0]:
        raise ValueError(f"node table must have {csr.n_nodes} rows and {pm.dims[0]} slots, got {na.table.size(0)} / {na.k0}")
    return nnconv_forward_mixed_raw(x, csr, na, None, None, 0, pm, root, bias, aggr, precision=precision, out=out, ws=ws)


PER_EDGE_MAX_EDGES = 1 << 17


def per_edge_association(csr: Csr, dims: Sequence[int], aggr: str) -> bool:
    return aggr in ("add", "mean") and 0 < csr.n_edges <= PER_EDGE_MAX_EDGES and csr.max_in_degree > csr.n_nodes


def nnconv_forward_per_edge_raw(x: torch.Tensor, csr: Csr, edge_attr: torch.Tensor, pm: PackedMlp,
                                weights: Sequence[torch.Tensor], biases: Sequence[Optional[torch.Tensor]],
                                root: Optional[torch.Tensor], bias: Optional[torch.Tensor], aggr: str) -> torch.Tensor:
    hidden, _ = hidden_forward_raw(csr, edge_attr.detach().contiguous(), pm, list(weights[:-1]) + [None],
                                   list(biases[:-1]) + [None], "f32")
    we = edge_weights_raw(hidden, pm, weights[-1], biases[-1])
    del hidden
    return nnconv_forward_edgeweights_raw(x.detach().contiguous(), csr, we, root, bias, aggr)


def forward_route(csr: Csr, pm: PackedMlp, aggr: str = "mean", precision: Optional[str] = None,
                  ws_bytes: Optional[int] = None) -> dict:
    if per_edge_association(csr, pm.dims, aggr):
        return {"association": "per_edge"}
    flags = _fwd_flags(csr, precision)
    precision = DEFAULT_PRECISION if precision is None else precision
    n, e = csr.n_nodes, csr.n_edges
    ws_bytes = workspace_bytes(n, e, pm) if ws_bytes is None else int(ws_bytes)
    rc = _lib.lib().gpde_nnconv_fwd_edge_path(n, e, len(pm.dims) - 1, pm.dims_c, flags, ws_bytes)
    if rc < 0:
        _lib.check(rc, "gpde_nnconv_fwd_edge_path")
    return {"association": "node", "kernel": fused_kernel_name(n, e, pm, precision), "edge_path": rc == 1,
            "n_chunks": launch_plan(n, e, pm, ws_bytes)["n_chunks"]}


def launch_plan(n_nodes: int, n_edges: int, pm: PackedMlp, ws_bytes: int):
    lib = _lib.lib()
    nch, npc, wgs, mode = ctypes.c_int32(), ctypes.c_int64(), ctypes.c_int32(), ctypes.c_int32()
    rc = lib.gpde_nnconv_fwd_plan(n_nodes, n_edges, len(pm.dims) - 1, pm.dims_c, ws_bytes,
                                  ctypes.byref(nch), ctypes.byref(npc), ctypes.byref(wgs),
                                  ctypes.byref(mode))
    _lib.check(rc, "gpde_nnconv_fwd_plan")
    return {"n_chunks": nch.value, "nodes_per_chunk": npc.value, "fused_workgroups": wgs.value,
            "mode": mode.value}


def fused_kernel_name(n_nodes: int, n_edges: int, pm: PackedMlp, precision: Optional[str] = None) -> str:
    precision = DEFAULT_PRECISION if precision is None else precision
    return _lib.lib().gpde_nnconv_fwd_kernel(n_edges, len(pm.dims) - 1, pm.dims_c, _PRECISION[precision]).decode()


def nnconv_backward_raw(x: torch.Tensor, csr: Csr, edge_attr: torch.Tensor,
                        weights: Sequence[torch.Tensor], biases: Sequence[Optional[torch.Tensor]],
                        root: Optional[torch.Tensor], aggr: str, grad_out: torch.Tensor,
                        need_root: bool = True, need_bias: bool = True,
                        ws: Optional[torch.Tensor] = None, z_saved: Optional[torch.Tensor] = None, need_attr: bool = False,
                        hidden_saved: Optional[torch.Tensor] = None):
    lib = _lib.lib()
    for t, nm in ((x, "x"), (edge_attr, "edge_attr"), (grad_out, "grad_out")):
        _require_cuda(t, nm)
    if aggr not in _AGGR:
        raise NotImplementedError(f"aggr={aggr!r}")
    n, e, dev = csr.n_nodes, csr.n_edges, x.device
    x = _operand(x.detach(), "x", (n, WIDTH), dev)
    dims, dims_c, ws_, bs_ = _mlp_operands(weights, biases, dev)
    nl, k2p = len(ws_), hidden_width(dims)
    if need_attr and (isinstance(edge_attr, NodeAttr) or dims[0] > 8):
        raise NotImplementedError("the edge-attribute gradient is built for attribute tensors of <= 8 slots")
    attr_p, na_ref, perm_p, _alive = _attr_source(csr, edge_attr.detach(), keep_rows=need_attr)
    grad_out = _operand(grad_out.detach().float(), "grad_out", (n, WIDTH), dev)
    root_c, _ = _root_bias(root, None, dev)
    ws = _operand(ws, "ws", (None,), dev, writable=True, dtype=torch.uint8)
    z_saved = _operand(z_saved, "z_saved", (n, WIDTH * k2p), dev)
    gx = torch.empty(n, WIDTH, dtype=torch.float32, device=dev)
    gW = [torch.empty_like(w) for w in ws_]
    gb = [None if b is None else torch.empty_like(b) for b in bs_]
    groot, gbias = _update_grads(root, need_root, need_bias, dev)
    ga = torch.zeros(e, dims[0], dtype=torch.float32, device=dev) if need_attr else None
    if n == 0:
        for t in gW + gb + [groot, gbias]:
            if t is not None:
                t.zero_()
        return (gx, gW, gb, groot, gbias, ga) if need_attr else (gx, gW, gb, groot, gbias)
    if ws is None:
        ws = alloc_bwd_ws(lib, n, e, nl, dims_c, dev, 0 if hidden_saved is None else e * k2p * 4)
    srp, ssl = csr.src_order
    if hidden_saved is not None and (need_attr or hidden_saved.dtype != torch.float32 or tuple(hidden_saved.shape) != (e, k2p)):
        raise ValueError(f"hidden_saved must be float32 [{e},{k2p}] (and excludes need_attr)")
    hidden_saved = _operand(hidden_saved, "hidden_saved", (e, k2p), dev)
    with torch.cuda.device(dev):
        rc = lib.gpde_nnconv_bwd(x.data_ptr(), n, attr_p, na_ref, _ptr(hidden_saved), e, csr.rowptr.data_ptr(), csr.src.data_ptr(),
                                 csr.dst.data_ptr(), perm_p, csr.rowptr_host.data_ptr(), _ptr(srp), _ptr(ssl), nl, dims_c,
                                 _ptr_array(ws_), _ptr_array(bs_), _ptr(root_c), _AGGR[aggr], grad_out.data_ptr(), _ptr(z_saved),
                                 gx.data_ptr(), None, _ptr(ga), _ptr_array(gW), _ptr_array(gb), _ptr(groot), _ptr(gbias), 0,
                                 ws.data_ptr(), ws.numel(), _stream_ptr(dev))
    _lib.check(rc, "gpde_nnconv_bwd")
    _lib.n_native_calls += 1
    return (gx, gW, gb, groot, gbias, ga) if need_attr else (gx, gW, gb, groot, gbias)


def deferred_supported(dims: Sequence[int]) -> bool:
    return bool(_lib.lib().gpde_nnconv_bwd_deferred_supported(len(dims) - 1, _lib.dims_array(dims)))


def nodeattr_train_supported(dims: Sequence[int]) -> bool:
    return len(dims) == 4 and 1 <= dims[0] <= 7 and (int(dims[1]) + 31) // 32 >= 8 and deferred_supported(dims) and \
        DEFAULT_PRECISION == "f16split"


def deferred_layers_padded(n_defer: int) -> int:
    return max(4, (n_defer + 1) // 2 * 2)


def nnconv_backward_light_raw(x: torch.Tensor, csr: Csr, edge_attr: torch.Tensor,
                              weights: Sequence[torch.Tensor], biases: Sequence[Optional[torch.Tensor]],
                              root: Optional[torch.Tensor], aggr: str, grad_out: torch.Tensor,
                              need_root: bool = True, need_bias: bool = True, z_saved: Optional[torch.Tensor] = None,
                              hidden_part: Optional[torch.Tensor] = None, hidden_nodes: int = 0):
    lib = _lib.lib()
    for t, nm in ((x, "x"), (edge_attr, "edge_attr"), (grad_out, "grad_out")):
        _require_cuda(t, nm)
    if aggr not in _AGGR:
        raise NotImplementedError(f"aggr={aggr!r}")
    n, e, dev = csr.n_nodes, csr.n_edges, x.device
    x = _operand(x.detach(), "x", (n, WIDTH), dev)
    attr_p, na_ref, perm_p, _alive = _attr_source(csr, edge_attr.detach())
    grad_out = _operand(grad_out.detach().float(), "grad_out", (n, WIDTH), dev)
    dims, dims_c, ws_, bs_ = _mlp_operands(weights, biases, dev)
    nl, k2p = len(ws_), hidden_width(dims)
    root_c, _ = _root_bias(root, None, dev)
    z_saved = _operand(z_saved, "z_saved", (n, WIDTH * k2p), dev)
    hidden_part = _operand(hidden_part, "hidden_part", (None, k2p), dev)
    gx = torch.empty(n, WIDTH, dtype=torch.float32, device=dev)
    gw = torch.empty_like(ws_[-1])
    gb = None if bs_[-1] is None else torch.empty_like(bs_[-1])
    groot, gbias = _update_grads(root, need_root, need_bias, dev)
    ws = _queried_ws("gpde_nnconv_bwd_workspace_bytes", dev, n, e, nl, dims_c)
    srp, ssl = csr.src_order
    with torch.cuda.device(dev):
        rc = lib.gpde_nnconv_bwd_light(x.data_ptr(), n, attr_p, na_ref, e, csr.rowptr.data_ptr(), csr.src.data_ptr(), csr.dst.data_ptr(),
                                       perm_p, csr.rowptr_host.data_ptr(), _ptr(srp), _ptr(ssl), nl, dims_c,
                                       _ptr_array(ws_), _ptr_array(bs_), _ptr(root_c), _AGGR[aggr], grad_out.data_ptr(), _ptr(z_saved),
                                       _ptr(hidden_part) if hidden_nodes > 0 else None, int(hidden_nodes) if hidden_part is not None else 0,
                                       gx.data_ptr(), gw.data_ptr(), _ptr(gb), _ptr(groot), _ptr(gbias), ws.data_ptr(), ws.numel(),
                                       _stream_ptr(dev))
    _lib.check(rc, "gpde_nnconv_bwd_light")
    _lib.n_native_calls += 1
    return gx, gw, gb, groot, gbias


def nnconv_backward_deferred_raw(xs: Sequence[torch.Tensor], gs: Sequence[torch.Tensor], csr: Csr, edge_attr: torch.Tensor,
                                 weights: Sequence[torch.Tensor], biases: Sequence[Optional[torch.Tensor]], aggr: str,
                                 hidden_part: Optional[torch.Tensor] = None, hidden_nodes: int = 0):
    lib = _lib.lib()
    L = len(xs)
    if L < 1 or len(gs) != L:
        raise ValueError("one (input, output gradient) pair per deferred application")
    n, e, dev = csr.n_nodes, csr.n_edges, edge_attr.device
    Lp = deferred_layers_padded(L)
    x_stack = torch.zeros(Lp, n, WIDTH, dtype=torch.float32, device=dev)
    g_stack = torch.empty(L, n, WIDTH, dtype=torch.float32, device=dev)
    for l in range(L):
        x_stack[l].copy_(_operand(xs[l].detach(), f"xs[{l}]", (n, WIDTH), dev))
        g_stack[l].copy_(_operand(gs[l].detach().float(), f"gs[{l}]", (n, WIDTH), dev))
    attr_p, na_ref, perm_p, _alive = _attr_source(csr, edge_attr.detach())
    dims, dims_c, ws_, bs_ = _mlp_operands(weights, biases, dev)
    nl = len(ws_)
    hidden_part = _operand(hidden_part, "hidden_part", (None, hidden_width(dims)), dev)
    gW = [torch.empty_like(w) for w in ws_[:-1]] + [None]
    gb = [None if b is None else torch.empty_like(b) for b in bs_[:-1]] + [None]
    ws = _queried_ws("gpde_nnconv_bwd_deferred_workspace_bytes", dev, n, e, nl, dims_c, L)
    with torch.cuda.device(dev):
        rc = lib.gpde_nnconv_bwd_deferred(x_stack.data_ptr(), g_stack.data_ptr(), L, n, attr_p, na_ref, e, csr.rowptr.data_ptr(),
                                          csr.src.data_ptr(), csr.dst.data_ptr(), perm_p, csr.rowptr_host.data_ptr(), nl, dims_c,
                                          _ptr_array(ws_), _ptr_array(bs_), _AGGR[aggr],
                                          _ptr(hidden_part) if hidden_nodes > 0 else None,
                                          int(hidden_nodes) if hidden_part is not None else 0,
                                          _ptr_array(gW), _ptr_array(gb), ws.data_ptr(), ws.numel(), _stream_ptr(dev))
    _lib.check(rc, "gpde_nnconv_bwd_deferred")
    _lib.n_native_calls += 1
    return gW[:-1], gb[:-1]


def hidden_width(dims: Sequence[int]) -> int:
    return (int(dims[-2]) + 127) // 128 * 128


def hidden_forward_raw(csr: Csr, edge_attr: torch.Tensor, pm: PackedMlp,
                       weights: Sequence[torch.Tensor], biases: Sequence[Optional[torch.Tensor]],
                       precision: Optional[str] = None, n_nodes_limit: Optional[int] = None) -> torch.Tensor:
    lib = _lib.lib()
    _require_cuda(edge_attr, "edge_attr")
    precision = DEFAULT_PRECISION if precision is None else precision
    if precision not in _PRECISION:
        raise ValueError(f"precision must be one of {sorted(_PRECISION)}, got {precision!r}")
    e, dev, nl, flags = csr.n_edges, edge_attr.device, len(pm.dims) - 1, _PRECISION[precision]
    is_na = isinstance(edge_attr, NodeAttr)
    if not is_na and (edge_attr.dtype != torch.float32 or edge_attr.dim() != 2 or edge_attr.size(0) != e or
                      edge_attr.size(1) != pm.dims[0]):
        raise ValueError(f"edge_attr must be float32 [{e},{pm.dims[0]}], got {edge_attr.dtype} {tuple(edge_attr.shape)}")
    attr_p, na_ref, perm_p, _alive = _attr_source(csr, edge_attr.detach())
    n_lim = csr.n_nodes
    if n_nodes_limit is not None:
        n_lim = int(n_nodes_limit)
        e = int(csr.rowptr_host[n_lim])
    hidden = torch.empty(e, hidden_width(pm.dims), dtype=torch.float32, device=dev)
    if is_na:
        fast, ends, wa, ba, ws = True, (csr.src.data_ptr(), csr.dst.data_ptr()), None, None, None
    else:
        _, _, ws_, bs_ = _mlp_operands(weights, biases, dev, pm.dims)
        ends, wa, ba = (None, None), _ptr_array(ws_), _ptr_array(bs_)
        nbytes = int(lib.gpde_hidden_workspace_bytes(e, nl, pm.dims_c))
        fast = (flags & _lib.GPDE_FWD_F16SPLIT) and nl == 3
        ws = torch.empty(1 if fast else max(nbytes, 1), dtype=torch.uint8, device=dev)
    hmax = torch.zeros(1, dtype=torch.float32, device=dev) if fast else None

    def call(hmax, ws):
        return lib.gpde_hidden_fwd(attr_p, na_ref, e, csr.rowptr.data_ptr(), n_lim, perm_p, *ends, nl, pm.dims_c, pm.packed.data_ptr(),
                                   wa, ba, flags, hidden.data_ptr(), _ptr(hmax), _ptr(ws), 0 if ws is None else ws.numel(),
                                   _stream_ptr(dev))
    with torch.cuda.device(dev):
        rc = call(hmax, ws)
        if rc in (-1, -3) and fast and not is_na:
            hmax = None
            rc = call(hmax, _alloc_ws(nbytes, dev))
    _lib.check(rc, "gpde_hidden_fwd (node table)" if is_na else "gpde_hidden_fwd")
    _lib.n_native_calls += 1
    return hidden, hmax


def nnconv_forward_hidden_raw(x: torch.Tensor, csr: Csr, hidden: torch.Tensor, pm: PackedMlp,
                              root: Optional[torch.Tensor], bias: Optional[torch.Tensor], aggr: str,
                              out: Optional[torch.Tensor] = None, ws: Optional[torch.Tensor] = None,
                              hmax: Optional[torch.Tensor] = None, residual: Optional[torch.Tensor] = None,
                              relu: bool = False, z_keep: Optional[torch.Tensor] = None) -> torch.Tensor:
    n = csr.n_nodes
    if x.dtype != torch.float32 or x.dim() != 2 or x.size(1) != WIDTH or x.size(0) != n:
        raise ValueError(f"x must be float32 [{n},{WIDTH}], got {x.dtype} {tuple(x.shape)}")
    return _forward64("gpde_nnconv_fwd_hidden" if z_keep is None else "gpde_nnconv_fwd_keepz", x, csr, pm, root, bias, aggr, 0,
                      hidden=hidden, hmax=hmax, residual=residual, relu=relu, z_keep=z_keep, out=out, ws=ws)


EDGE_WEIGHT_BYTES = WIDTH * WIDTH * 4


def edge_weights_raw(hidden: torch.Tensor, pm: PackedMlp, w_last: torch.Tensor, b_last: Optional[torch.Tensor]) -> torch.Tensor:
    lib = _lib.lib()
    _require_cuda(hidden, "hidden")
    e, dev = int(hidden.size(0)), hidden.device
    if hidden.dim() != 2:
        raise ValueError(f"hidden must be float32 [E,{hidden_width(pm.dims)}]")
    hidden = _operand(hidden.detach(), "hidden", (e, hidden_width(pm.dims)), dev)
    w_c = _operand(w_last.detach(), "w_last", (WIDTH * WIDTH, pm.dims[-2]), dev)
    b_c = _operand(None if b_last is None else b_last.detach(), "b_last", (WIDTH * WIDTH,), dev)
    we = torch.empty(e, WIDTH * WIDTH, dtype=torch.float32, device=dev)
    nl = len(pm.dims) - 1
    ws = torch.empty(max(int(lib.gpde_edge_weights_workspace_bytes(e, nl, pm.dims_c)), 1), dtype=torch.uint8, device=dev)
    with torch.cuda.device(dev):
        rc = lib.gpde_edge_weights_fwd(hidden.data_ptr(), e, nl, pm.dims_c, pm.packed.data_ptr(), w_c.data_ptr(),
                                       None if b_c is None else b_c.data_ptr(), we.data_ptr(), ws.data_ptr(), ws.numel(),
                                       _stream_ptr(dev))
    _lib.check(rc, "gpde_edge_weights_fwd")
    _lib.n_native_calls += 1
    return we


_AGGR_WE = {"add": _lib.GPDE_AGGR_ADD, "mean": _lib.GPDE_AGGR_MEAN, "max": _lib.GPDE_AGGR_MAX}


def nnconv_forward_edgeweights_group(calls: Sequence[dict]) -> List[torch.Tensor]:
    lib = _lib.lib()
    if not calls:
        return []
    dev = calls[0]["x"].device
    descs = (_lib.GpdeWeConvDesc * len(calls))()
    outs, keep = [], []
    for k, c in enumerate(calls):
        x, csr, we = c["x"], c["csr"], c["edge_weights"]
        _require_cuda(x, "x")
        n, e = csr.n_nodes, csr.n_edges
        if x.device != dev:
            raise ValueError("all calls of a group must live on one device")
        if x.dtype != torch.float32 or x.dim() != 2 or tuple(x.shape) != (n, WIDTH):
            raise ValueError(f"x must be float32 [{n},{WIDTH}], got {x.dtype} {tuple(x.shape)}")
        we = _operand(we.detach(), "edge_weights", (e, WIDTH * WIDTH), dev)
        aggr = c.get("aggr", "mean")
        if aggr not in _AGGR_WE:
            raise NotImplementedError(f"aggr={aggr!r}")
        x_c = _operand(x.detach(), "x", (n, WIDTH), dev)
        root_c, bias_c = _root_bias(c.get("root"), c.get("bias"), dev)
        res = _check_residual(c.get("residual"), x_c, n)
        out = _operand(c.get("out"), "out", (n, WIDTH), dev, writable=True)
        if out is None:
            out = torch.empty(n, WIDTH, dtype=torch.float32, device=dev)
        keep.append((x_c, root_c, bias_c, res, we, csr))
        outs.append(out)
        d = descs[k]
        d.x, d.edge_weights, d.rowptr, d.src = x_c.data_ptr(), we.data_ptr(), csr.rowptr.data_ptr(), csr.src.data_ptr()
        d.root = None if root_c is None else root_c.data_ptr()
        d.bias = None if bias_c is None else bias_c.data_ptr()
        d.residual = None if res is None else res.data_ptr()
        d.out, d.n_nodes, d.aggr, d.relu, d.reserved = out.data_ptr(), n, _AGGR_WE[aggr], 1 if c.get("relu") else 0, 0
    with torch.cuda.device(dev):
        rc = lib.gpde_nnconv_fwd_edgeweights_group(descs, len(calls), _stream_ptr(dev))
    _lib.check(rc, "gpde_nnconv_fwd_edgeweights_group")
    _lib.n_native_calls += len(calls)
    return outs


def nnconv_forward_edgeweights_raw(x, csr, edge_weights, root, bias, aggr, residual=None, relu=False, out=None):
    return nnconv_forward_edgeweights_group([dict(x=x, csr=csr, edge_weights=edge_weights, root=root, bias=bias, aggr=aggr,
                                                  residual=residual, relu=relu, out=out)])[0]


def nnconv_backward_edgeweights_raw(x: torch.Tensor, csr: Csr, edge_weights: torch.Tensor, root: Optional[torch.Tensor], aggr: str,
                                    grad_out: torch.Tensor, need_root: bool = True, need_bias: bool = True, acc=None):
    lib = _lib.lib()
    for t, nm in ((x, "x"), (edge_weights, "edge_weights"), (grad_out, "grad_out")):
        _require_cuda(t, nm)
    if aggr not in _AGGR:
        raise NotImplementedError(f"aggr={aggr!r}: the gradient of the per-edge weight operator is built for 'add' and 'mean'")
    n, e, dev = csr.n_nodes, csr.n_edges, x.device
    x = _operand(x.detach(), "x", (n, WIDTH), dev)
    grad_out = _operand(grad_out.detach().float(), "grad_out", (n, WIDTH), dev)
    we = _operand(edge_weights.detach(), "edge_weights", (e, WIDTH * WIDTH), dev)
    root_c, _ = _root_bias(root, None, dev)
    gx = torch.empty(n, WIDTH, dtype=torch.float32, device=dev)
    want_root = need_root and root is not None
    bits = 0
    if acc is not None:
        gwe, groot, gbias = acc
        if (groot is not None) != want_root or (gbias is not None) != bool(need_bias):
            raise ValueError("acc: (grad_edge_weights [E,4096], grad_root, grad_bias) of an application of the same module expected")
        gwe = _operand(gwe, "acc[0] (grad_edge_weights)", (e, WIDTH * WIDTH), dev, writable=True)
        groot = _operand(groot, "acc[1] (grad_root)", (WIDTH, WIDTH), dev, writable=True)
        gbias = _operand(gbias, "acc[2] (grad_bias)", (WIDTH,), dev, writable=True)
        bits = _lib.GPDE_ACC_EDGE_WEIGHTS | (_lib.GPDE_ACC_ROOT if want_root else 0) | (_lib.GPDE_ACC_BIAS if need_bias else 0)
    else:
        gwe = torch.empty(e, WIDTH * WIDTH, dtype=torch.float32, device=dev)
        groot = torch.empty(WIDTH, WIDTH, dtype=torch.float32, device=dev) if want_root else None
        gbias = torch.empty(WIDTH, dtype=torch.float32, device=dev) if need_bias else None
    ws = _alloc_ws(int(lib.gpde_nnconv_bwd_edgeweights_workspace_bytes(n, e)), dev)
    srp, ssl = csr.src_order
    with torch.cuda.device(dev):
        rc = lib.gpde_nnconv_bwd_edgeweights_acc(x.data_ptr(), n, we.data_ptr(), e, csr.rowptr.data_ptr(), csr.src.data_ptr(), _ptr(srp), _ptr(ssl),
                                                 _ptr(root_c), _AGGR[aggr], grad_out.data_ptr(), gx.data_ptr(), gwe.data_ptr(), _ptr(groot), _ptr(gbias),
                                                 bits, ws.data_ptr(), ws.numel(), _stream_ptr(dev))
    _lib.check(rc, "gpde_nnconv_bwd_edgeweights_acc")
# ... 1170 lines not shown
```

### include/gpde.h

```cpp
#ifndef GPDE_H
#define GPDE_H

#include <stddef.h>
#include <stdint.h>

#ifdef __cplusplus
extern "C" {
#endif

#define GPDE_VERSION 101
#define GPDE_VERSION_ABLATION 0x10000
#define GPDE_VERSION_INSTRUMENTED 0x20000

#define GPDE_API __attribute__((visibility("default")))

enum {
    GPDE_OK = 0,
    GPDE_EINVAL = -1,
    GPDE_EUNSUPPORTED = -2,
    GPDE_EWORKSPACE = -3,
    GPDE_EHIP = -4
};

enum { GPDE_AGGR_ADD = 0, GPDE_AGGR_MEAN = 1,
       GPDE_AGGR_MAX = 2  };

enum {
    GPDE_FWD_DEFAULT = 0,
    GPDE_FWD_F16SPLIT = 1,
    GPDE_FWD_F16SPLIT_8WAVE = 2,
    GPDE_FWD_STATIC_RANGES = 4,
    GPDE_FWD_AGG_F16 = 16,
    GPDE_FWD_AGG_F32 = 32,
    GPDE_FWD_NO_EDGE_PATH = 64
};

#define GPDE_MAX_LAYERS 8
#define GPDE_WIDTH 64

typedef struct GpdeNodeAttr {
    const float* table;
    int32_t stride;
    int32_t n_slots;
    int32_t sel[8];
} GpdeNodeAttr;

GPDE_API int gpde_version(void);
GPDE_API const char* gpde_last_error(void);
GPDE_API int gpde_reload_switches(void);

GPDE_API size_t gpde_csr_workspace_bytes(int64_t n_edges, int64_t n_nodes);
GPDE_API int gpde_csr_from_coo(const int64_t* edge_index, int64_t stride_row, int64_t stride_col,
                      int64_t n_edges, int64_t n_nodes, int32_t* rowptr, int32_t* src,
                      int32_t* dst, int32_t* perm, int32_t* n_bad, void* ws, size_t ws_bytes,
                      void* stream);
GPDE_API int gpde_csr_from_coo2(const int64_t* edge_index, int64_t stride_row, int64_t stride_col, int64_t n_edges,
                       int64_t n_src, int64_t n_dst, int32_t* rowptr, int32_t* src, int32_t* dst, int32_t* perm,
                       int32_t* n_bad, void* ws, size_t ws_bytes, void* stream);
GPDE_API int gpde_gather_rows(const float* rows, int k, const int32_t* perm, int64_t n, float* out, void* stream);

GPDE_API size_t gpde_mlp_pack_bytes(int n_layers, const int32_t* dims);
GPDE_API int gpde_mlp_pack(int n_layers, const int32_t* dims, const float* const* W,
                  const float* const* b, void* packed, size_t packed_bytes, void* stream);

GPDE_API size_t gpde_nnconv_fwd_workspace_bytes(int64_t n_nodes, int64_t n_edges, int n_layers,
                                       const int32_t* dims);
GPDE_API int gpde_nnconv_fwd(const float* x, int64_t n_nodes, const float* edge_attr, int64_t n_edges,
                    const int32_t* rowptr, const int32_t* src, const int32_t* dst,
                    const int32_t* perm, int n_layers, const int32_t* dims, const void* packed,
                    const float* root, const float* bias, int aggr, uint32_t flags, float* out,
                    void* ws, size_t ws_bytes, void* stream);

GPDE_API int gpde_nnconv_fwd_act(const float* x, int64_t n_nodes, const float* edge_attr, int64_t n_edges,
                        const int32_t* rowptr, const int32_t* src, const int32_t* dst, const int32_t* perm,
                        int n_layers, const int32_t* dims, const void* packed, const float* root,
                        const float* bias, int aggr, uint32_t flags, const float* residual, int relu_out,
                        float* out, void* ws, size_t ws_bytes, void* stream);
GPDE_API int gpde_nnconv_fwd_hidden_act(const float* x, int64_t n_nodes, const float* hidden, const float* hidden_absmax,
                               int64_t n_edges, const int32_t* rowptr, const int32_t* src, const int32_t* dst,
                               int n_layers, const int32_t* dims, const void* packed, const float* root,
                               const float* bias, int aggr, const float* residual, int relu_out, float* out,
                               void* ws, size_t ws_bytes, void* stream);

GPDE_API int gpde_nnconv_fwd_plan(int64_t n_nodes, int64_t n_edges, int n_layers, const int32_t* dims,
                         size_t ws_bytes, int32_t* n_chunks, int64_t* nodes_per_chunk,
                         int32_t* fused_workgroups, int32_t* mode);

GPDE_API const char* gpde_nnconv_fwd_kernel(int64_t n_edges, int n_layers, const int32_t* dims, uint32_t flags);

GPDE_API int gpde_nnconv_fwd_edge_path(int64_t n_nodes, int64_t n_edges, int n_layers, const int32_t* dims, uint32_t flags,
                                       size_t ws_bytes);

GPDE_API size_t gpde_nnconv_bwd_workspace_bytes(int64_t n_nodes, int64_t n_edges, int n_layers,
                                       const int32_t* dims);
GPDE_API size_t gpde_nnconv_bwd_workspace_bytes_one_chunk(int64_t n_nodes, int64_t n_edges, int n_layers,
                                                 const int32_t* dims);
GPDE_API int gpde_nnconv_bwd_plan(int64_t n_nodes, int64_t n_edges, int n_layers, const int32_t* dims, size_t ws_bytes,
                                  int n_defer, int h_given, int64_t* edges_per_chunk, int64_t* nodes_per_chunk);
enum { GPDE_BWD_ACCUMULATE_GRAD_HIDDEN = 1  };
GPDE_API int gpde_nnconv_bwd(const float* x, int64_t n_nodes, const float* edge_attr, const GpdeNodeAttr* node_attr,
                    const float* hidden, int64_t n_edges, const int32_t* rowptr, const int32_t* src, const int32_t* dst,
                    const int32_t* perm, const int32_t* rowptr_host, const int32_t* src_rowptr, const int32_t* src_slots,
                    int n_layers, const int32_t* dims, const float* const* W, const float* const* b, const float* root,
                    int aggr, const float* grad_out, const float* z_saved, float* grad_x, float* grad_hidden,
                    float* grad_edge_attr, float* const* grad_W, float* const* grad_b, float* grad_root,
                    float* grad_bias, uint32_t flags, void* ws, size_t ws_bytes, void* stream);
GPDE_API int gpde_csr_source_order(const int32_t* src, int64_t n_edges, int64_t n_nodes, int32_t* src_rowptr,
                          int32_t* src_slots, void* ws, size_t ws_bytes, void* stream);

GPDE_API size_t gpde_hidden_workspace_bytes(int64_t n_edges, int n_layers, const int32_t* dims);
GPDE_API int gpde_hidden_fwd(const float* edge_attr, const GpdeNodeAttr* node_attr, int64_t n_edges, const int32_t* rowptr,
                    int64_t n_nodes, const int32_t* perm, const int32_t* src, const int32_t* dst, int n_layers,
                    const int32_t* dims, const void* packed, const float* const* W, const float* const* b, uint32_t flags,
                    float* hidden, float* hidden_absmax, void* ws, size_t ws_bytes, void* stream);
GPDE_API int gpde_nnconv_fwd_hidden(const float* x, int64_t n_nodes, const float* hidden,
                           const float* hidden_absmax, int64_t n_edges,
                           const int32_t* rowptr, const int32_t* src, const int32_t* dst,
                           int n_layers, const int32_t* dims, const void* packed, const float* root,
                           const float* bias, int aggr, float* out, void* ws, size_t ws_bytes,
                           void* stream);
GPDE_API int gpde_hidden_bwd(const float* edge_attr, const GpdeNodeAttr* node_attr, int64_t n_edges, const int32_t* perm,
                    const int32_t* src, const int32_t* dst, int n_layers,
                    const int32_t* dims, const float* const* W, const float* const* b,
                    const float* grad_hidden, float* const* grad_W, float* const* grad_b, void* ws,
                    size_t ws_bytes, void* stream);

GPDE_API int gpde_nnconv_fwd_keepz(const float* x, int64_t n_nodes, const float* edge_attr, const float* hidden,
                          const float* hidden_absmax, int64_t n_edges, const int32_t* rowptr, const int32_t* src,
                          const int32_t* dst, const int32_t* perm, int n_layers, const int32_t* dims, const void* packed,
                          const float* root, const float* bias, int aggr, uint32_t flags, float* z_keep, float* out,
                          void* ws, size_t ws_bytes, void* stream);

GPDE_API int gpde_nnconv_bwd_deferred_supported(int n_layers, const int32_t* dims);
GPDE_API size_t gpde_nnconv_bwd_deferred_workspace_bytes(int64_t n_nodes, int64_t n_edges, int n_layers, const int32_t* dims,
                                                int n_defer);
GPDE_API int gpde_nnconv_bwd_light(const float* x, int64_t n_nodes, const float* edge_attr, const GpdeNodeAttr* node_attr,
                          int64_t n_edges, const int32_t* rowptr,
                          const int32_t* src, const int32_t* dst, const int32_t* perm, const int32_t* rowptr_host,
                          const int32_t* src_rowptr, const int32_t* src_slots, int n_layers, const int32_t* dims,
                          const float* const* W, const float* const* b, const float* root, int aggr, const float* grad_out,
                          const float* z_saved, const float* hidden_part, int64_t hidden_nodes, float* grad_x,
                          float* grad_w_last, float* grad_b_last, float* grad_root,
                          float* grad_bias, void* ws, size_t ws_bytes, void* stream);
GPDE_API int gpde_nnconv_bwd_deferred(const float* x_stack, const float* grad_out_stack, int n_defer, int64_t n_nodes,
                             const float* edge_attr, const GpdeNodeAttr* node_attr, int64_t n_edges, const int32_t* rowptr,
                             const int32_t* src, const int32_t* dst, const int32_t* perm, const int32_t* rowptr_host,
                             int n_layers, const int32_t* dims, const float* const* W, const float* const* b, int aggr,
                             const float* hidden_part, int64_t hidden_nodes,
                             float* const* grad_W, float* const* grad_b, void* ws, size_t ws_bytes, void* stream);
GPDE_API int gpde_nnconv_fwd_mixed_keepz(const float* x, int64_t n_nodes, const float* edge_attr, const GpdeNodeAttr* node_attr,
                                const float* hidden, const float* hidden_absmax, int64_t hidden_nodes, int64_t n_edges,
                                const int32_t* rowptr, const int32_t* src, const int32_t* dst,
                                const int32_t* perm, int n_layers, const int32_t* dims, const void* packed,
                                const float* root, const float* bias, int aggr, uint32_t flags, float* z_keep, float* out,
                                void* ws, size_t ws_bytes, void* stream);

GPDE_API size_t gpde_edge_weights_workspace_bytes(int64_t n_edges, int n_layers, const int32_t* dims);
GPDE_API int gpde_edge_weights_fwd(const float* hidden , int64_t n_edges, int n_layers,
                          const int32_t* dims, const void* packed ,
                          const float* w_last , const float* b_last ,
                          float* edge_weights , void* ws, size_t ws_bytes, void* stream);
#define GPDE_WECONV_MAX_GROUP 16
typedef struct GpdeWeConvDesc {
    const float* x;
    const float* edge_weights;
    const int32_t* rowptr;
    const int32_t* src;
    const float* root;
    const float* bias;
    const float* residual;
    float* out;
    int32_t n_nodes;
    int32_t aggr;
    int32_t relu;
    int32_t reserved;
} GpdeWeConvDesc;
GPDE_API int gpde_nnconv_fwd_edgeweights_group(const GpdeWeConvDesc* descs , int n_descs, void* stream);

GPDE_API size_t gpde_nnconv_bwd_edgeweights_workspace_bytes(int64_t n_nodes, int64_t n_edges);
GPDE_API int gpde_nnconv_bwd_edgeweights(const float* x, int64_t n_nodes, const float* edge_weights, int64_t n_edges,
                                const int32_t* rowptr, const int32_t* src, const int32_t* src_rowptr,
                                const int32_t* src_slots, const float* root, int aggr, const float* grad_out,
                                float* grad_x, float* grad_edge_weights, float* grad_root, float* grad_bias, void* ws,
                                size_t ws_bytes, void* stream);
enum {
    GPDE_ACC_EDGE_WEIGHTS = 1,
    GPDE_ACC_ROOT = 2,
    GPDE_ACC_BIAS = 4
};
GPDE_API int gpde_nnconv_bwd_edgeweights_acc(const float* x, int64_t n_nodes, const float* edge_weights, int64_t n_edges,
                                    const int32_t* rowptr, const int32_t* src, const int32_t* src_rowptr,
                                    const int32_t* src_slots, const float* root, int aggr, const float* grad_out,
                                    float* grad_x, float* grad_edge_weights, float* grad_root, float* grad_bias,
                                    int accumulate, void* ws, size_t ws_bytes, void* stream);
GPDE_API size_t gpde_edge_weights_bwd_workspace_bytes(int64_t n_edges, int n_layers, const int32_t* dims);
GPDE_API int gpde_edge_weights_bwd(const float* grad_edge_weights, const float* hidden, int64_t n_edges, int n_layers,
                          const int32_t* dims, const float* w_last, float* grad_hidden, float* grad_w_last,
                          float* grad_b_last, void* ws, size_t ws_bytes, void* stream);

#define GPDE_WECONV_ANY_MAX_WIDTH 256
GPDE_API int gpde_nnconv_fwd_edgeweights_any(const float* x, int64_t n_nodes, const float* edge_weights, int64_t n_edges,
                                    const int32_t* rowptr, const int32_t* src, const float* root, const float* bias,
                                    const float* residual, int relu, int aggr, int in_channels, int out_channels,
                                    float* out, void* stream);
GPDE_API size_t gpde_nnconv_bwd_edgeweights_any_workspace_bytes(int64_t n_nodes, int64_t n_edges, int in_channels,
                                                       int out_channels);
GPDE_API int gpde_nnconv_edgeweights_any_plan(int in_channels, int out_channels, int vec4, int aggr, int32_t* out);
GPDE_API int gpde_nnconv_bwd_edgeweights_any(const float* x, int64_t n_nodes, const float* edge_weights, int64_t n_edges,
                                    const int32_t* rowptr, const int32_t* src, const int32_t* src_rowptr,
                                    const int32_t* src_slots, const float* root, int aggr, int in_channels,
                                    int out_channels, const float* grad_out, float* grad_x, float* grad_edge_weights,
                                    float* grad_root, float* grad_bias, void* ws, size_t ws_bytes, void* stream);

#define GPDE_REASSOC_ANY_MAX_HIDDEN 4096
GPDE_API size_t gpde_nnconv_fwd_hidden_any_workspace_bytes(int64_t n_nodes, int64_t n_edges, int in_channels, int out_channels,
                                                  int k_hidden);
GPDE_API int gpde_nnconv_fwd_hidden_any(const float* x, int64_t n_nodes, const float* hidden, int64_t n_edges, int k_hidden,
                               const int32_t* rowptr, const int32_t* src, const float* w_last, const float* b_last,
                               const float* root, const float* bias, int aggr, int in_channels, int out_channels, float* out,
                               void* ws, size_t ws_bytes, void* stream);
GPDE_API size_t gpde_nnconv_bwd_hidden_any_workspace_bytes(int64_t n_nodes, int64_t n_edges, int in_channels, int out_channels,
                                                  int k_hidden);
GPDE_API int gpde_nnconv_bwd_hidden_any(const float* x, int64_t n_nodes, const float* hidden, int64_t n_edges, int k_hidden,
                               const int32_t* rowptr, const int32_t* src, const float* w_last, const float* b_last,
                               const float* root, int aggr, int in_channels, int out_channels, const float* grad_out,
                               float* grad_x, float* grad_hidden, float* grad_w_last, float* grad_b_last, float* grad_root,
                               float* grad_bias, const int32_t* src_rowptr, const int32_t* src_slots, void* ws, size_t ws_bytes,
                               void* stream);

GPDE_API int gpde_nnconv_fwd_edgeweights_bip(const float* x_src, int64_t n_src, const float* x_dst, int64_t n_dst,
                                    const float* edge_weights, int64_t n_edges, const int32_t* rowptr, const int32_t* src,
                                    const float* root, const float* bias, const float* residual, int relu, int aggr,
                                    int in_src, int in_dst, int out_channels, float* out, void* stream);
GPDE_API size_t gpde_nnconv_bwd_edgeweights_bip_workspace_bytes(int64_t n_src, int64_t n_dst, int64_t n_edges, int in_src,
                                                       int in_dst, int out_channels);
GPDE_API int gpde_nnconv_bwd_edgeweights_bip(const float* x_src, int64_t n_src, const float* x_dst, int64_t n_dst,
                                    const float* edge_weights, int64_t n_edges, const int32_t* rowptr, const int32_t* src,
                                    const int32_t* src_rowptr, const int32_t* src_slots, const float* root, int aggr,
                                    int in_src, int in_dst, int out_channels, const float* grad_out, float* grad_x_src,
                                    float* grad_x_dst, float* grad_edge_weights, float* grad_root, float* grad_bias,
                                    void* ws, size_t ws_bytes, void* stream);
GPDE_API size_t gpde_nnconv_fwd_hidden_bip_workspace_bytes(int64_t n_dst, int64_t n_edges, int in_src, int out_channels,
                                                  int k_hidden);
GPDE_API int gpde_nnconv_fwd_hidden_bip(const float* x_src, int64_t n_src, const float* x_dst, int64_t n_dst,
// ... 139 lines not shown
```

Before: 204.7 M-edges/s.

## Precompute per-edge f16-split attribute image before fused NNConv kernel

Adds a pre-pass kernel that gathers edge attributes through the permutation, computes the per-edge scale, and writes f16 hi/lo planes plus an inverse scale in sorted edge order. The fused f16v6 kernel then streams these with contiguous global-to-LDS loads instead of permuted gathers and in-loop conversion, and its first-layer operands are formed ahead of the loop. This costs an extra kernel pass and about 36 bytes per edge of workspace, which can shrink the node chunk size. A flag is added to turn the path off.

```diff
diff --git a/graph-pde_amd/_lib.py b/graph-pde_amd/_lib.py
--- a/graph-pde_amd/_lib.py
+++ b/graph-pde_amd/_lib.py
@@ -18,6 +18,7 @@
 GPDE_RADIUS_BATCHED_REC_BYTES = 96
 GPDE_FWD_DEFAULT, GPDE_FWD_F16SPLIT = 0, 1
 GPDE_FWD_F16SPLIT_8WAVE, GPDE_FWD_STATIC_RANGES, GPDE_FWD_AGG_F16, GPDE_FWD_AGG_F32, GPDE_FWD_NO_EDGE_PATH = 2, 4, 16, 32, 64
+GPDE_FWD_NO_ATTR_IMAGE = 128
 GPDE_WIDTH = 64
 GPDE_BWD_ACCUMULATE_GRAD_HIDDEN = 1
 
diff --git a/graph-pde_amd/csrc/gpde_api.hip b/graph-pde_amd/csrc/gpde_api.hip
--- a/graph-pde_amd/csrc/gpde_api.hip
+++ b/graph-pde_amd/csrc/gpde_api.hip
@@ -135,7 +135,8 @@
     int64_t nodes_per_chunk;
     int n_chunks;
     int n_groups;
-    size_t off_part, off_z, off_ha, off_hb, off_xs, off_scal, off_blk;
+    size_t off_part, off_z, off_ha, off_hb, off_xs, off_scal, off_blk, off_img;
+    bool attr_image;
     int nblk_max;
     size_t h_floats;
 };
@@ -147,8 +148,11 @@
     return s;
 }
 
+bool attr_image_eligible(const GpdePackLayout& L, uint32_t flags, int64_t n_edges, int kt);
+
 int make_plan(int64_t N, int64_t E, int n_layers, const int32_t* dims, size_t ws_bytes, bool sizing,
-              Plan* P, size_t* needed, bool hidden_given = false) {
+              Plan* P, size_t* needed, bool hidden_given = false, uint32_t flags = GPDE_FWD_F16SPLIT, int kt = 0,
+              bool attr_given = true) {
     int rc = gpde_pack_layout(n_layers, dims, &P->L);
     if (rc != GPDE_OK) return rc;
     const GpdePackLayout& L = P->L;
@@ -167,28 +171,43 @@
     P->nblk_max = (L.mode == 1 && E < ((int64_t)1 << 31) - GP_QBLOCK) ? (int)(E / GP_QBLOCK + E / 8 / (GP_QBLOCK / 8)) + 10 : 0;
     const size_t blk_bytes = P->nblk_max ? align_up(((size_t)P->nblk_max + 2 + 64) * 4) : 0;
     fixed += blk_bytes;
+    const size_t img_bytes = (attr_given && !hidden_given && attr_image_eligible(L, flags, E, kt)) ? gpde_attr_image_bytes(E) : 0;
+    int64_t npc_rec = (int64_t)(((size_t)4 << 30) / zrow);
+    if (npc_rec < 64) npc_rec = 64;
+    if (npc_rec > N) npc_rec = N;
+    if (npc_rec < 1) npc_rec = 1;
+    auto nodes_for = [&](size_t fx, bool quiet, int64_t* out) {
+        if (ws_bytes < fx + 2 * kAlign) {
+            if (!quiet) gpde_set_error("gpde_nnconv_fwd: workspace %zu bytes cannot hold the %zu-byte hidden "
+                                       "activation buffers", ws_bytes, fx);
+            return GPDE_EWORKSPACE;
+        }
+        int64_t n_ = (int64_t)((ws_bytes - fx - 2 * kAlign) / (zrow + prow));
+        if (N > 0 && align_up((size_t)N * prow) + align_up((size_t)N * zrow) + fx <= ws_bytes) n_ = N;
+        if (n_ > N) n_ = N;
+        const int64_t min_nodes = N < 64 ? N : 64;
+        if (n_ < min_nodes || (N > 0 && n_ < 1)) {
+            if (!quiet) gpde_set_error("gpde_nnconv_fwd: workspace %zu bytes holds %lld destination nodes, need >= %lld "
+                                       "(%zu bytes per node)", ws_bytes, (long long)n_, (long long)min_nodes, zrow + prow);
+            return GPDE_EWORKSPACE;
+        }
+        if (n_ < N && n_ > 64) n_ = n_ / 64 * 64;
+        *out = n_;
+        return GPDE_OK;
+    };
     int64_t npc;
+    P->attr_image = false;
     if (sizing) {
-        int64_t cap = (int64_t)(((size_t)4 << 30) / zrow);
-        if (cap < 64) cap = 64;
-        npc = N < cap ? N : cap;
-        if (npc < 1) npc = 1;
+        npc = npc_rec;
+        P->attr_image = img_bytes != 0;
     } else {
-        if (ws_bytes < fixed + 2 * kAlign) {
-            gpde_set_error("gpde_nnconv_fwd: workspace %zu bytes cannot hold the %zu-byte hidden "
-                           "activation buffers", ws_bytes, fixed);
-            return GPDE_EWORKSPACE;
-        }
-        npc = (int64_t)((ws_bytes - fixed - 2 * kAlign) / (zrow + prow));
-        if (N > 0 && align_up((size_t)N * prow) + align_up((size_t)N * zrow) + fixed <= ws_bytes) npc = N;
-        if (npc > N) npc = N;
-        const int64_t min_nodes = N < 64 ? N : 64;
-        if (npc < min_nodes || (N > 0 && npc < 1)) {
-            gpde_set_error("gpde_nnconv_fwd: workspace %zu bytes holds %lld destination nodes, need >= %lld "
-                           "(%zu bytes per node)", ws_bytes, (long long)npc, (long long)min_nodes, zrow + prow);
-            return GPDE_EWORKSPACE;
-        }
-        if (npc < N && npc > 64) npc = npc / 64 * 64;
+        int64_t npc_img = 0;
+        if (img_bytes && nodes_for(fixed + img_bytes, true, &npc_img) == GPDE_OK && npc_img >= npc_rec) {
+            npc = npc_img;
+            P->attr_image = true;
+        } else if ((rc = nodes_for(fixed, false, &npc)) != GPDE_OK) {
+            return rc;
+        }
     }
     if (npc < 1) npc = 1;
     P->nodes_per_chunk = npc;
@@ -202,6 +221,7 @@
     P->off_xs = off;   off += xs_bytes ? xs_bytes - kAlign : 0;
     P->off_scal = off; off += xs_bytes ? kAlign : 0;
     P->off_blk = off;  off += blk_bytes;
+    P->off_img = off;  off += P->attr_image ? img_bytes : 0;
     if (needed) *needed = off;
     const int ns = L.K2P / GP_TN;
     int groups = num_cus_impl() / ns;
@@ -230,6 +250,12 @@
     return c;
 }
 
+bool attr_image_eligible(const GpdePackLayout& L, uint32_t flags, int64_t n_edges, int kt) {
+    if ((flags & GPDE_FWD_NO_ATTR_IMAGE) || n_edges >= ((int64_t)1 << 31) - GP_QBLOCK) return false;
+    if (choose_fused(L, L.mode, flags, n_edges, kt).kind != FK_V6) return false;
+    return gpde_fused_f16v6_image_supported(gpde_fused_probe(L));
+}
+
 bool takes_edge_path(const Plan& P, uint32_t flags, int64_t n_nodes, int64_t n_edges, bool hidden, bool hidden_absmax,
                      bool mixed, int kt) {
     const GpdePackLayout& L = P.L;
@@ -261,9 +287,19 @@
                                          size_t ws_bytes) {
     Plan P;
     if (!dims || n_nodes < 0 || n_edges < 0) { gpde_set_error("gpde_nnconv_fwd_edge_path: null/negative argument"); return GPDE_EINVAL; }
-    int rc = make_plan(n_nodes, n_edges, n_layers, dims, ws_bytes, false, &P, nullptr);
+    int rc = make_plan(n_nodes, n_edges, n_layers, dims, ws_bytes, false, &P, nullptr, false, flags);
     if (rc != GPDE_OK) return rc;
     return takes_edge_path(P, flags, n_nodes, n_edges, false, false, false, 0) ? 1 : 0;
+}
+
+extern "C" int gpde_nnconv_fwd_attr_image(int64_t n_nodes, int64_t n_edges, int n_layers, const int32_t* dims, uint32_t flags,
+                                          size_t ws_bytes, int32_t* n_chunks) {
+    Plan P;
+    if (!dims || n_nodes < 0 || n_edges < 0) { gpde_set_error("gpde_nnconv_fwd_attr_image: null/negative argument"); return GPDE_EINVAL; }
+    int rc = make_plan(n_nodes, n_edges, n_layers, dims, ws_bytes, false, &P, nullptr, false, flags);
+    if (rc != GPDE_OK) return rc;
+    if (n_chunks) *n_chunks = P.n_chunks;
+    return (P.attr_image && !takes_edge_path(P, flags, n_nodes, n_edges, false, false, false, 0)) ? 1 : 0;
 }
 
 extern "C" size_t gpde_nnconv_fwd_workspace_bytes(int64_t n_nodes, int64_t n_edges, int n_layers,
@@ -336,7 +372,8 @@
     if (a.n_nodes == 0) return GPDE_OK;
     if (!a.ws) { gpde_set_error("gpde_nnconv_fwd: workspace is null"); return GPDE_EWORKSPACE; }
     Plan P;
-    int rc = make_plan(a.n_nodes, a.n_edges, a.n_layers, a.dims, a.ws_bytes, false, &P, nullptr, a.hidden != nullptr && !mixed);
+    int rc = make_plan(a.n_nodes, a.n_edges, a.n_layers, a.dims, a.ws_bytes, false, &P, nullptr, a.hidden != nullptr && !mixed,
+                       a.flags, a.kt, a.hidden == nullptr);
     if (rc != GPDE_OK) return rc;
     const GpdePackLayout& L = P.L;
     const int mode = (a.hidden && !mixed) ? 2 : L.mode;
@@ -403,6 +440,7 @@
 
     const unsigned* xs = nullptr;
     const unsigned* scal = nullptr;
+    GpdeAttrImage img{nullptr, nullptr, nullptr, nullptr};
     const FusedChoice fc = choose_fused(L, mode, a.flags, a.n_edges, a.kt);
     if (a.kt && fc.kind == FK_GENERIC) {
         gpde_set_error("gpde_nnconv_fwd_mixed_keepz (node_attr): built for 3-Linear kernel MLPs on the f16-split kernel only");
@@ -415,6 +453,12 @@
         if (rc != GPDE_OK) return rc;
         xs = (const unsigned*)(w + P.off_xs);
         scal = (const unsigned*)(w + P.off_scal);
+        if (P.attr_image && fc.kind == FK_V6) {
+            img = gpde_attr_image_at(w + P.off_img, a.n_edges);
+            rc = gpde_launch_attr_image(a.edge_attr, a.perm, a.n_edges, L.k0, pk + L.off_w1 + (size_t)L.K1P * 8, pk + L.off_fcol,
+                                        img, a.stream, a.kt, a.sel, a.src, a.dst);
+            if (rc != GPDE_OK) return rc;
+        }
     }
 
     if (a.hidden && !mixed && a.hidden_absmax && a.n_edges >= 32768 && !(a.flags & GPDE_FWD_AGG_F32)) {
@@ -441,6 +485,7 @@
             f.kt = a.kt; f.hmax = (from_h && xs) ? (const unsigned*)a.hidden_absmax : nullptr;
             for (int d = 0; d < 8; ++d) f.sel[d] = (a.kt && a.sel) ? a.sel[d < L.k0 ? d : L.k0 - 1] : 0;
             f.nc0 = (int)nc0; f.nc1 = (int)nc1; f.e_chunk0 = 0; f.n_groups = P.n_groups;
+            f.img_rec = img.rec; f.img_hi = img.hi; f.img_lo = img.lo; f.img_isc = img.isc;
             {
                 ProfScope ps(GPDE_PROF_FUSED, a.stream);
                 if (!from_h && fc.kind == FK_V6 && P.nblk_max && L.K2P / GP_TN <= 64 && !(a.flags & GPDE_FWD_STATIC_RANGES)) {
diff --git a/graph-pde_amd/csrc/gpde_common.h b/graph-pde_amd/csrc/gpde_common.h
--- a/graph-pde_amd/csrc/gpde_common.h
+++ b/graph-pde_amd/csrc/gpde_common.h
@@ -138,12 +138,29 @@
     int e_chunk0;
     int n_groups;
     int kernarg_pad_;
+    const void* img_hi;
+    const void* img_lo;
+    const float* img_isc;
+    const void* img_rec;
 };
 int gpde_launch_fused(int mode, bool f16split, const GpdeFusedArgs& a, hipStream_t stream);
 int gpde_launch_g2_prep(const float* x, int64_t n_nodes, const float* attr, int64_t n_edges, int k0,
                         const float* wmax8, unsigned* scal, unsigned* xs, hipStream_t stream,
                         int kt = 0, const int* sel = nullptr, const int32_t* src = nullptr,
                         const int32_t* dst = nullptr);
+struct GpdeAttrImage { void* rec; void* hi; void* lo; float* isc; };
+static inline size_t gpde_attr_image_bytes(int64_t n_edges) {
+    const size_t e = (size_t)(n_edges > 0 ? n_edges : 0);
+    return 256 + 2 * ((e * 16 + 255) / 256 * 256) + (e * 4 + 255) / 256 * 256;
+}
+static inline GpdeAttrImage gpde_attr_image_at(void* base, int64_t n_edges) {
+    const size_t e = (size_t)(n_edges > 0 ? n_edges : 0), plane = (e * 16 + 255) / 256 * 256;
+    char* b = (char*)base;
+    return GpdeAttrImage{b, b + 256, b + 256 + plane, (float*)(b + 256 + 2 * plane)};
+}
+int gpde_launch_attr_image(const float* attr, const int32_t* perm, int64_t n_edges, int k0, const float* wmax8,
+                           const float* fcol, const GpdeAttrImage& img, hipStream_t stream, int kt = 0,
+                           const int* sel = nullptr, const int32_t* src = nullptr, const int32_t* dst = nullptr);
 constexpr int GP_QBLOCK = 4096;
 int gpde_launch_block_bounds(const int32_t* rowptr, int nc0, int nc1, int nblk_max, int32_t* blk, int32_t* qn,
                              unsigned* qctr, int n_slices, hipStream_t stream);
@@ -161,6 +178,7 @@
 int gpde_launch_fused_store(const GpdeFusedArgs& a, hipStream_t stream);
 bool gpde_fused_f16v6_supported(const GpdeFusedArgs& a);
 int gpde_launch_fused_f16v6(const GpdeFusedArgs& a, hipStream_t stream);
+bool gpde_fused_f16v6_image_supported(const GpdeFusedArgs& a);
 int gpde_num_cus();
 static inline void gpde_fused_set_pack(GpdeFusedArgs& f, const float* pk, const GpdePackLayout& L) {
     f.w1 = pk + L.off_w1; f.w2t = pk + L.off_w2t; f.b2 = pk + L.off_b2;
diff --git a/graph-pde_amd/csrc/gpde_fused_f16v6.hip b/graph-pde_amd/csrc/gpde_fused_f16v6.hip
--- a/graph-pde_amd/csrc/gpde_fused_f16v6.hip
+++ b/graph-pde_amd/csrc/gpde_fused_f16v6.hip
@@ -34,10 +34,13 @@
 constexpr int TE = 64;
 constexpr int NW = 4;
 
-template <int MODE, bool NODEATTR = false>
+enum { ASRC_TENSOR = 0, ASRC_NODES = 1, ASRC_IMAGE = 2 };
+template <int MODE, int ASRC = ASRC_TENSOR>
 __global__ __launch_bounds__(256) __attribute__((amdgpu_waves_per_eu(1, 1)))
 void gpde_fused_f16v6_kernel(GpdeFusedArgs a) {
     constexpr bool WRITE_H = MODE == 1;
+    constexpr bool NODEATTR = ASRC == ASRC_NODES, IMAGE = ASRC == ASRC_IMAGE;
+    static_assert(!(IMAGE && WRITE_H), "the store variant forms its attribute operands itself");
     extern __shared__ __attribute__((aligned(16))) char smem[];
     char* ring = smem;
     char* w1s = smem + NS * TILE_B;
@@ -53,6 +56,12 @@
     const int g = lane >> 4;
     float* Es = Es_all + wave * TE;
     unsigned* Xs = Xs_all + wave * TE * GP_W;
+    char* stage = nullptr;
+    float* Es_n = nullptr;
+    if constexpr (IMAGE) {
+        stage = (char*)(colc + 2 * GP_TN) + wave * 2048;
+        Es_n = (float*)((char*)(colc + 2 * GP_TN) + NW * 2048) + wave * TE;
+    }
 
     const int ns = a.K2P / GP_TN;
     const int slice = blockIdx.x % ns;
@@ -91,6 +100,9 @@
         have = blk_b > blk_a;
     }
     if (lane == 0) { red[wave] = have ? 0 : 1; red[4 + wave] = 0; }
+    if constexpr (IMAGE) {
+        if (tid < 4) red[8 + tid] = 0;
+    }
     __syncthreads();
     if (red[0] + red[1] + red[2] + red[3] == 4) return;
 
@@ -150,6 +162,27 @@
 #pragma unroll
         for (int d = 0; d < 8; ++d) load_attr_d(d);
     };
+    [[maybe_unused]] auto img_issue = [&](int which, int e0t, int ebt, float* es_to) {
+        const int e = e0t + lane;
+        const bool ok = e < ebt;
+        if (which == 0) {
+            const char* p = ok ? (const char*)a.img_hi + (size_t)e * 16 : (const char*)a.img_rec;
+            GPDE_GLDS(p, stage, 0);
+        } else if (which == 1) {
+            const char* p = ok ? (const char*)a.img_lo + (size_t)e * 16 : (const char*)a.img_rec;
+            GPDE_GLDS(p, stage + 1024, 0);
+        } else {
+            const char* p = ok ? (const char*)(a.img_isc + e) : (const char*)a.img_rec + 16;
+            __builtin_amdgcn_global_load_lds((const __attribute__((address_space(1))) void*)p,
+                                             (__attribute__((address_space(3))) void*)es_to, 4, 0, 0);
+        }
+    };
+    const char* b1p = nullptr;
+    int b1s = 0;
+    if constexpr (IMAGE) {
+        b1p = g == 3 ? (const char*)(red + 8) : stage + l15 * 16 + (g == 1 ? 1024 : 0);
+        b1s = g == 3 ? 0 : 256;
+    }
     int xsidx[4];
     auto x_addr1 = [&](int i0, int i) { xsidx[i] = __builtin_amdgcn_ds_bpermute((4 * (i0 + i) + (lane >> 4)) * 4, src_l); };
     auto x_issue1 = [&](int i0, int i) {
@@ -201,8 +234,13 @@
         char* l1 = ring + TILE_B + wave * 4096;
         GPDE_GLDS(g1, l1, 0); GPDE_GLDS(g1, l1, 1024); GPDE_GLDS(g1, l1, 2048); GPDE_GLDS(g1, l1, 3072);
     }
-    load_perm(have ? blk_a : e_hi);
-    load_attr();
+    if constexpr (IMAGE) {
+#pragma unroll
+        for (int i = 0; i < 3; ++i) img_issue(i, have ? blk_a : e_hi, have ? blk_b : 0, Es);
+    } else {
+        load_perm(have ? blk_a : e_hi);
+        load_attr();
+    }
     asm volatile("s_waitcnt vmcnt(0)" ::: "memory");
     __syncthreads();
 
@@ -251,6 +289,26 @@
 #endif
     int e0 = have ? blk_a : e_hi;
     int n_rounds = 0;
+    h8 B1[4];
+    f32x4 d[4][2];
+    u4 ahi[4], alo[4];
+    if constexpr (IMAGE) {
+#pragma unroll
+        for (int b = 0; b < 4; ++b) B1[b] = *(const h8*)(b1p + b * b1s);
+        const char* wp = w1s + w1o;
+        const h8 A1 = *(const h8*)wp, A2 = *(const h8*)(wp + 256);
+        h1gen(d, A1, A2, B1);
+        asm volatile("s_nop 15\n\ts_nop 15" ::: "memory");
+#pragma unroll
+        for (int e = 0; e < 2; ++e)
+#pragma unroll
+            for (int jp = 0; jp < 4; ++jp) {
+                unsigned ph, pl;
+                conv_pair(d[e][jp >> 1][2 * (jp & 1)], d[e][jp >> 1][2 * (jp & 1) + 1], ph, pl);
+                ahi[e][jp] = ph;
+                alo[e][jp] = pl;
+            }
+    }
     for (int t = 0;; ++t) {
         const int eb = have ? blk_b : e0;
         const int e_end = min(e0 + TE, eb);
@@ -259,6 +317,7 @@
         bool have_n = have && !last_in_blk;
         if (last_in_blk && queue) have_n = draw_block(na_, nb_);
         const int e0n = !have ? e_hi : (last_in_blk ? (have_n ? na_ : e_hi) : e0 + TE);
+        [[maybe_unused]] const int ebn = !have ? 0 : (last_in_blk ? (have_n ? nb_ : 0) : blk_b);
         if (t > 0) {
             if (lane == 0) red[(t & 1) * 4 + wave] = have ? 0 : 1;
             __syncthreads();
@@ -267,8 +326,7 @@
         }
         ++n_rounds;
 
-        h8 B1[4];
-        {
+        if constexpr (!IMAGE) {
 #pragma unroll
             for (int b = 0; b < 4; ++b) {
                 float av[8];
@@ -305,9 +363,7 @@
             bhi[0][nb] = *(const h8*)(ring + slot * TILE_B + nb * 2048 + bo);
             blo[0][nb] = *(const h8*)(ring + slot * TILE_B + nb * 2048 + (bo ^ 64));
         }
-        f32x4 d[4][2];
-        u4 ahi[4], alo[4];
-        {
+        if constexpr (!IMAGE) {
             const char* wp = w1s + w1o;
             const h8 A1 = *(const h8*)wp, A2 = *(const h8*)(wp + 256);
             h1gen(d, A1, A2, B1);
@@ -380,7 +436,9 @@
                     if (n == 25) A1 = *(const h8*)w1n;
                     if (n == 31) A2 = *(const h8*)(w1n + 256);
                     if constexpr (MODE == 0 && PH == 0) {
-                        if (n == 53) load_perm(e0n);
+                        if constexpr (!IMAGE) {
+                            if (n == 53) load_perm(e0n);
+                        }
                         if (n == 59) src_l = a.src[min(e0 + lane, e_clamp)];
                         if (n == 65) nf_v[0] = a.dst[min(e0, e_clamp)];
                         if (n == 71) nl_v[0] = a.dst[min(max(min(e0 + 32, eb) - 1, e0), e_clamp)];
@@ -389,8 +447,16 @@
                     } else if constexpr (WRITE_H && PH == 0) {
                         if (n == 53) load_perm(e0n);
                     }
-                    if constexpr (PH == 2) {
+                    if constexpr (PH == 2 && IMAGE) {
+                        if (n == 29 || n == 35 || n == 41) img_issue((n - 29) / 6, e0n, ebn, Es_n);
+                    } else if constexpr (PH == 2) {
                         if (n >= 29 && n < 77 && (n - 29) % 6 == 0) load_attr_d((n - 29) / 6);
+                    }
+                    if constexpr (PH == 7) {
+                        if (n == 1) B1[0] = *(const h8*)b1p;
+                        if (n == 2) B1[1] = *(const h8*)(b1p + b1s);
+                        if (n == 4) B1[2] = *(const h8*)(b1p + 2 * b1s);
+                        if (n == 7) B1[3] = *(const h8*)(b1p + 3 * b1s);
                     }
                     if constexpr (!WRITE_H && PH >= 2 && PH <= 5) {
                         if (n == 1 || n == 7 || n == 13 || n == 19) x_addr1(4 * (PH - 2), (n - 1) / 6);
@@ -412,7 +478,9 @@
             else if constexpr (WRITE_H && PH == 2) asm volatile("s_waitcnt vmcnt(8)" ::: "memory");
             else if constexpr (WRITE_H) asm volatile("s_waitcnt vmcnt(0)" ::: "memory");
             else if constexpr (PH == 0 && NODEATTR) asm volatile("s_waitcnt vmcnt(7)" ::: "memory");
+            else if constexpr (PH == 0 && IMAGE) asm volatile("s_waitcnt vmcnt(5)" ::: "memory");
             else if constexpr (PH == 0) asm volatile("s_waitcnt vmcnt(6)" ::: "memory");
+            else if constexpr (PH == 2 && IMAGE) asm volatile("s_waitcnt vmcnt(7)" ::: "memory");
             else if constexpr (PH == 2) asm volatile("s_waitcnt vmcnt(12)" ::: "memory");
             else if constexpr (PH >= 3 && PH <= 5) asm volatile("s_waitcnt vmcnt(4)" ::: "memory");
             else asm volatile("s_waitcnt vmcnt(0)" ::: "memory");
@@ -429,8 +497,8 @@
 #ifdef GPDE_V6_TIMING
         tm_peel += clock64() - tm0_;
 #endif
-        for (int c = 6; c < NKC; ++c) chunk(std::integral_constant<int, 6>{}, c);
-
+        for (int c = 6; c < (IMAGE ? NKC - 1 : NKC); ++c) chunk(std::integral_constant<int, 6>{}, c);
+        if constexpr (IMAGE) chunk(std::integral_constant<int, 7>{}, NKC - 1);
 
         TM_MARK(tm_loop);
         if constexpr (WRITE_H) {
@@ -545,6 +613,11 @@
 #pragma unroll
             for (int nb = 0; nb < 8; ++nb) asm volatile("" : "+a"(Z[cb][nb]));
         TM_MARK(tm_post);
+        if constexpr (IMAGE) {
+            float* es_t = Es;
+            Es = Es_n;
+            Es_n = es_t;
+        }
         if (last_in_blk) {
             have = have_n;
             blk_a = na_;
@@ -579,6 +652,7 @@
     return (size_t)NS * TILE_B + (size_t)K1P * 32 + (size_t)NW * TE * GP_W * 4 + (size_t)NW * TE * 4 + 64 +
            2 * GP_TN * 4;
 }
+size_t v6_image_lds_bytes(int K1P) { return v6_lds_bytes(K1P) + (size_t)NW * 2048 + (size_t)NW * TE * 4; }
 
 }
 
@@ -598,20 +672,34 @@
            (a.hout != nullptr || a.xs != nullptr);
 }
 
+bool gpde_fused_f16v6_image_supported(const GpdeFusedArgs& a) {
+    GpdeFusedArgs p = a;
+    if (!p.xs) p.xs = (const unsigned*)(uintptr_t)8;
+    p.hout = nullptr;
+    return gpde_fused_f16v6_supported(p) && v6_image_lds_bytes(a.K1P) <= 160 * 1024;
+}
+
 int gpde_launch_fused_f16v6(const GpdeFusedArgs& a, hipStream_t stream) {
     const int ns = a.K2P / GP_TN;
     const dim3 grid(a.n_groups * ns), block(256);
     const size_t lds = v6_lds_bytes(a.K1P);
     static GpdeLdsOnce once;
-    if (int rc = once.ensure(gpde_fused_f16v6_kernel<0, false>, gpde_fused_f16v6_kernel<1, false>, gpde_fused_f16v6_kernel<0, true>,
-                             gpde_fused_f16v6_kernel<1, true>)) return rc;
+    if (int rc = once.ensure(gpde_fused_f16v6_kernel<0, ASRC_TENSOR>, gpde_fused_f16v6_kernel<1, ASRC_TENSOR>,
+                             gpde_fused_f16v6_kernel<0, ASRC_NODES>, gpde_fused_f16v6_kernel<1, ASRC_NODES>,
+                             gpde_fused_f16v6_kernel<0, ASRC_IMAGE>)) return rc;
     if (a.hout) {
         GpdeFusedArgs b = a;
         b.blk = nullptr; b.qn = nullptr; b.qctr = nullptr;
-        if (a.kt) hipLaunchKernelGGL((gpde_fused_f16v6_kernel<1, true>), grid, block, lds, stream, b);
-        else hipLaunchKernelGGL((gpde_fused_f16v6_kernel<1, false>), grid, block, lds, stream, b);
-    } else if (a.kt) hipLaunchKernelGGL((gpde_fused_f16v6_kernel<0, true>), grid, block, lds, stream, a);
-    else hipLaunchKernelGGL((gpde_fused_f16v6_kernel<0, false>), grid, block, lds, stream, a);
+        if (a.kt) hipLaunchKernelGGL((gpde_fused_f16v6_kernel<1, ASRC_NODES>), grid, block, lds, stream, b);
+        else hipLaunchKernelGGL((gpde_fused_f16v6_kernel<1, ASRC_TENSOR>), grid, block, lds, stream, b);
+    } else if (a.img_hi) {
+        if (!a.img_lo || !a.img_isc || !a.img_rec || !gpde_fused_f16v6_image_supported(a)) {
+            gpde_set_error("gpde_fused_f16v6_kernel: attribute image incomplete or K1P = %d beyond the image variant", a.K1P);
+            return GPDE_EINVAL;
+        }
+        hipLaunchKernelGGL((gpde_fused_f16v6_kernel<0, ASRC_IMAGE>), grid, block, v6_image_lds_bytes(a.K1P), stream, a);
+    } else if (a.kt) hipLaunchKernelGGL((gpde_fused_f16v6_kernel<0, ASRC_NODES>), grid, block, lds, stream, a);
+    else hipLaunchKernelGGL((gpde_fused_f16v6_kernel<0, ASRC_TENSOR>), grid, block, lds, stream, a);
     GP_LAUNCH_CHECK("gpde_fused_f16v6_kernel");
     return GPDE_OK;
 }
diff --git a/graph-pde_amd/csrc/gpde_prep.hip b/graph-pde_amd/csrc/gpde_prep.hip
--- a/graph-pde_amd/csrc/gpde_prep.hip
+++ b/graph-pde_amd/csrc/gpde_prep.hip
@@ -47,6 +47,55 @@
     if ((threadIdx.x & 63) == 0 && m > 0.f) atomicMax(scal + 1, __float_as_uint(m));
 }
 
+typedef _Float16 h8v __attribute__((ext_vector_type(8)));
+template <bool NODES>
+__global__ void k_attr_image(const float* __restrict__ attr, const int32_t* __restrict__ perm, int kt, SelArr sel,
+                             const int32_t* __restrict__ src, const int32_t* __restrict__ dst, int64_t E, int k0,
+                             const float* __restrict__ wmax8, const float* __restrict__ fcol, h8v* __restrict__ hi8,
+                             h8v* __restrict__ lo8, float* __restrict__ isc_out, unsigned* __restrict__ rec) {
+    float wmx8[8], fcol8[8];
+#pragma unroll
+    for (int d = 0; d < 8; ++d) {
+        wmx8[d] = wmax8[(d & 1) * 4 + (d >> 1)];
+        fcol8[d] = fcol[d];
+    }
+    if (blockIdx.x == 0 && threadIdx.x < 5) rec[threadIdx.x] = threadIdx.x == 4 ? __float_as_uint(1.f) : 0u;
+    for (int64_t e = (int64_t)blockIdx.x * blockDim.x + threadIdx.x; e < E; e += (int64_t)gridDim.x * blockDim.x) {
+        float v[8];
+        if constexpr (NODES) {
+            const int s_ = src[e], t_ = dst[e];
+#pragma unroll
+            for (int d = 0; d < 8; ++d)
+                v[d] = d < k0 ? attr[(size_t)((sel.v[d] >> 8) ? t_ : s_) * kt + (sel.v[d] & 255)] : 0.f;
+        } else {
+            const size_t row = (size_t)perm[e] * k0;
+#pragma unroll
+            for (int d = 0; d < 8; ++d) v[d] = d < k0 ? attr[row + d] : 0.f;
+        }
+        float bnd = 0.f;
+#pragma unroll
+        for (int d = 0; d < 8; ++d) {
+            if (d == k0) v[d] = 1.f;
+            bnd = fmaf(wmx8[d], fabsf(v[d]), bnd);
+        }
+        const int ebits = (__float_as_int(bnd) >> 23) & 0xff;
+        const bool okb = (ebits >= 20) && (ebits <= 230);
+        const float sc = okb ? __int_as_float((267 - ebits) << 23) : 1.f;
+        const float isc = okb ? __int_as_float((ebits - 13) << 23) : 1.f;
+        h8v hi, lo;
+#pragma unroll
+        for (int d = 0; d < 8; ++d) {
+            const float s_ = v[d] * fcol8[d] * sc;
+            const _Float16 h = (_Float16)s_;
+            hi[d] = h;
+            lo[d] = (_Float16)(s_ - (float)h);
+        }
+        hi8[e] = hi;
+        lo8[e] = lo;
+        isc_out[e] = isc;
+    }
+}
+
 __global__ void k_split_x(const float* __restrict__ x, size_t n, const unsigned* __restrict__ scal,
                           unsigned* __restrict__ xs) {
     const float sc = gpde_pow2_to_2p13(__uint_as_float(scal[0]));
@@ -91,6 +140,24 @@
     return GPDE_OK;
 }
 
+int gpde_launch_attr_image(const float* attr, const int32_t* perm, int64_t n_edges, int k0, const float* wmax8,
+                           const float* fcol, const GpdeAttrImage& img, hipStream_t stream, int kt, const int* sel,
+                           const int32_t* src, const int32_t* dst) {
+    if (k0 < 1 || k0 > 7 || (kt ? (!sel || !src || !dst) : !perm)) {
+        gpde_set_error("gpde_launch_attr_image: k0 = %d (1..7) or a missing attribute source", k0);
+        return GPDE_EINVAL;
+    }
+    const unsigned ge = (unsigned)((n_edges + 255) / 256 < 8192 ? (n_edges + 255) / 256 : 8192);
+    SelArr sa;
+    for (int d = 0; d < 8; ++d) sa.v[d] = kt ? sel[d] : 0;
+    if (kt) hipLaunchKernelGGL(k_attr_image<true>, dim3(ge ? ge : 1), dim3(256), 0, stream, attr, perm, kt, sa, src, dst, n_edges,
+                               k0, wmax8, fcol, (h8v*)img.hi, (h8v*)img.lo, img.isc, (unsigned*)img.rec);
+    else hipLaunchKernelGGL(k_attr_image<false>, dim3(ge ? ge : 1), dim3(256), 0, stream, attr, perm, kt, sa, src, dst, n_edges,
+                            k0, wmax8, fcol, (h8v*)img.hi, (h8v*)img.lo, img.isc, (unsigned*)img.rec);
+    GP_LAUNCH_CHECK("k_attr_image");
+    return GPDE_OK;
+}
+
 int gpde_launch_g2_prep(const float* x, int64_t n_nodes, const float* attr, int64_t n_edges, int k0,
                         const float* wmax8, unsigned* scal, unsigned* xs, hipStream_t stream, int kt,
                         const int* sel, const int32_t* src, const int32_t* dst) {
diff --git a/graph-pde_amd/ops.py b/graph-pde_amd/ops.py
--- a/graph-pde_amd/ops.py
+++ b/graph-pde_amd/ops.py
@@ -577,15 +577,21 @@
               "f16split_static": _lib.GPDE_FWD_F16SPLIT | _lib.GPDE_FWD_STATIC_RANGES,
               "f16split_agg16": _lib.GPDE_FWD_F16SPLIT | _lib.GPDE_FWD_AGG_F16,
               "f16split_agg32": _lib.GPDE_FWD_F16SPLIT | _lib.GPDE_FWD_AGG_F32,
-              "f16split_noedge": _lib.GPDE_FWD_F16SPLIT | _lib.GPDE_FWD_NO_EDGE_PATH}
+              "f16split_noedge": _lib.GPDE_FWD_F16SPLIT | _lib.GPDE_FWD_NO_EDGE_PATH,
+              "f16split_noimage": _lib.GPDE_FWD_F16SPLIT | _lib.GPDE_FWD_NO_ATTR_IMAGE}
+_SAME_BYTES_SWITCHES = ("f16split_noimage",)
 DEFAULT_PRECISION = os.environ.get("GPDE_PRECISION", "f16split")
+
+
+def _precision_choices() -> list:
+    return sorted(k for k in _PRECISION if k not in _SAME_BYTES_SWITCHES)
 EDGE_PATH_MAX_IN_DEGREE = 64
 
 
 def _fwd_flags(csr: "Csr", precision: Optional[str]) -> int:
     name = DEFAULT_PRECISION if precision is None else precision
     if name not in _PRECISION:
-        raise ValueError(f"precision must be one of {sorted(_PRECISION)}, got {name!r}")
+        raise ValueError(f"precision must be one of {_precision_choices()}, got {name!r}")
     flags = _PRECISION[name]
     if precision is None and (flags & _lib.GPDE_FWD_F16SPLIT) and csr.n_edges > 0 and csr.max_in_degree > EDGE_PATH_MAX_IN_DEGREE:
         flags |= _lib.GPDE_FWD_NO_EDGE_PATH
@@ -904,8 +910,12 @@
     rc = _lib.lib().gpde_nnconv_fwd_edge_path(n, e, len(pm.dims) - 1, pm.dims_c, flags, ws_bytes)
     if rc < 0:
         _lib.check(rc, "gpde_nnconv_fwd_edge_path")
+    nch = ctypes.c_int32()
+    img = _lib.lib().gpde_nnconv_fwd_attr_image(n, e, len(pm.dims) - 1, pm.dims_c, flags, ws_bytes, ctypes.byref(nch))
+    if img < 0:
+        _lib.check(img, "gpde_nnconv_fwd_attr_image")
     return {"association": "node", "kernel": fused_kernel_name(n, e, pm, precision), "edge_path": rc == 1,
-            "n_chunks": launch_plan(n, e, pm, ws_bytes)["n_chunks"]}
+            "n_chunks": nch.value, "attr_image": img == 1}
 
 
 def launch_plan(n_nodes: int, n_edges: int, pm: PackedMlp, ws_bytes: int):
@@ -915,8 +925,9 @@
                                   ctypes.byref(nch), ctypes.byref(npc), ctypes.byref(wgs),
                                   ctypes.byref(mode))
     _lib.check(rc, "gpde_nnconv_fwd_plan")
+    img = lib.gpde_nnconv_fwd_attr_image(n_nodes, n_edges, len(pm.dims) - 1, pm.dims_c, _PRECISION[DEFAULT_PRECISION], ws_bytes, None)
     return {"n_chunks": nch.value, "nodes_per_chunk": npc.value, "fused_workgroups": wgs.value,
-            "mode": mode.value}
+            "mode": mode.value, "attr_image": img == 1}
 
 
 def fused_kernel_name(n_nodes: int, n_edges: int, pm: PackedMlp, precision: Optional[str] = None) -> str:
@@ -1067,7 +1078,7 @@
     _require_cuda(edge_attr, "edge_attr")
     precision = DEFAULT_PRECISION if precision is None else precision
     if precision not in _PRECISION:
-        raise ValueError(f"precision must be one of {sorted(_PRECISION)}, got {precision!r}")
+        raise ValueError(f"precision must be one of {_precision_choices()}, got {precision!r}")
     e, dev, nl, flags = csr.n_edges, edge_attr.device, len(pm.dims) - 1, _PRECISION[precision]
     is_na = isinstance(edge_attr, NodeAttr)
     if not is_na and (edge_attr.dtype != torch.float32 or edge_attr.dim() != 2 or edge_attr.size(0) != e or
diff --git a/include/gpde.h b/include/gpde.h
--- a/include/gpde.h
+++ b/include/gpde.h
@@ -32,7 +32,8 @@
     GPDE_FWD_STATIC_RANGES = 4,
     GPDE_FWD_AGG_F16 = 16,
     GPDE_FWD_AGG_F32 = 32,
-    GPDE_FWD_NO_EDGE_PATH = 64
+    GPDE_FWD_NO_EDGE_PATH = 64,
+    GPDE_FWD_NO_ATTR_IMAGE = 128
 };
 
 #define GPDE_MAX_LAYERS 8
@@ -90,6 +91,9 @@
 
 GPDE_API int gpde_nnconv_fwd_edge_path(int64_t n_nodes, int64_t n_edges, int n_layers, const int32_t* dims, uint32_t flags,
                                        size_t ws_bytes);
+
+GPDE_API int gpde_nnconv_fwd_attr_image(int64_t n_nodes, int64_t n_edges, int n_layers, const int32_t* dims, uint32_t flags,
+                                        size_t ws_bytes, int32_t* n_chunks);
 
 GPDE_API size_t gpde_nnconv_bwd_workspace_bytes(int64_t n_nodes, int64_t n_edges, int n_layers,
                                        const int32_t* dims);
```

Result: faster. 209.6 M-edges/s (median of 6 runs) (+2.4%).
